# tejank10/AlphaGo.jl

Hardware: AMD Instinct MI355X
Metric: self-play positions/sec (9x9, tower=10, 400 readouts) (higher is better)
Workload: dtype f32

## Files before the change

### alphago.jl_amd/_lib.py

```python
import ctypes as C
import os

HERE = os.path.dirname(os.path.abspath(__file__))
LIB_PATH = os.path.join(HERE, "libagz.so")

OK, ILLEGAL_MOVE, ASSERT_DONE_NODE, HISTORY_INCOMPLETE, BAD_SHAPE, ASSERT_SOFTPICK = range(6)
BAD_ARGUMENT, HIP_ERROR, POOL_EXHAUSTED, RCCL_ERROR, NOT_READY = 6, 7, 8, 9, 10

L_VALUE_CONV, L_POLICY_CONV, L_VALUE_FC1, L_VALUE_FC2, L_POLICY_FC = -1, -2, -3, -4, -5
K_WEIGHT, K_BIAS, K_BN_BETA, K_BN_GAMMA, K_BN_MEAN, K_BN_VAR, K_BN_EPS = range(7)
F_CHILD_N, F_CHILD_W, F_CHILD_PRIOR = 0, 1, 2


class AgzError(RuntimeError):
    def __init__(self, status, message):
        super().__init__(f"agz status {status}: {message}")
        self.status = status


class IllegalMove(AgzError):
    """IllegalMove, src/AlphaGo.jl:8"""


class Config(C.Structure):
    _fields_ = [
        ("board_size", C.c_int32), ("tower_height", C.c_int32), ("games", C.c_int32),
        ("num_readouts", C.c_int32), ("parallel_readouts", C.c_int32), ("two_player_mode", C.c_int32),
        ("komi", C.c_float), ("reserved0", C.c_float),
        ("c_puct", C.c_double), ("dirichlet_noise_weight", C.c_double), ("resign_threshold", C.c_double),
        ("resign_disable_fraction", C.c_double),
        ("seed", C.c_uint64), ("game_id_base", C.c_uint64), ("game_id_stride", C.c_uint64),
        ("max_nodes_per_game", C.c_int32), ("device", C.c_int32), ("external_network", C.c_int32),
        ("pool_policy", C.c_int32), ("record_capacity_games", C.c_int32), ("arena_mode", C.c_int32),
    ]


class Stats(C.Structure):
    _fields_ = [(n, C.c_int64) for n in (
        "steps", "positions", "games_started", "games_finished", "evals", "duplicate_evals",
        "terminal_visits", "root_visits", "nodes_in_use", "pool_exhausted", "resigned_games", "live_games",
        "records_dropped", "pool_short_searches", "peak_nodes_per_game", "stalled_games", "node_capacity",
        "abandoned_games")]

    def as_dict(self):
        return {n: getattr(self, n) for n, _ in self._fields_}


class GameHeader(C.Structure):
    _fields_ = [("game_id", C.c_uint64), ("num_moves", C.c_int32), ("result", C.c_int32),
                ("was_resign", C.c_int32), ("resign_disabled", C.c_int32), ("final_score", C.c_float),
                ("short_searches", C.c_int32)]


class PositionInfo(C.Structure):
    _fields_ = [("n", C.c_int32), ("to_play", C.c_int32), ("ko", C.c_int32), ("caps_black", C.c_int32),
                ("caps_white", C.c_int32), ("last_move", C.c_int32), ("prev_move", C.c_int32),
                ("history_len", C.c_int32), ("komi", C.c_float)]


class NodeInfo(C.Structure):
    _fields_ = [("N", C.c_float), ("W", C.c_float), ("Q", C.c_float), ("parent", C.c_int32),
                ("fmove", C.c_int32), ("is_expanded", C.c_int32), ("losses_applied", C.c_int32),
                ("done", C.c_int32), ("pos", PositionInfo)]


class Analysis(C.Structure):
    _fields_ = [("move", C.c_int32), ("status", C.c_int32), ("N", C.c_float), ("W", C.c_float), ("Q", C.c_float),
                ("nodes_used", C.c_int32)]


class Line(C.Structure):
    _fields_ = [("move", C.c_int32), ("pv_len", C.c_int32), ("N", C.c_float), ("W", C.c_float), ("prior", C.c_float),
                ("end_W", C.c_float)]


_lib = None


def _share_hip_runtime_with_torch():
    import importlib.util
    import sys
    if "torch" in sys.modules or os.environ.get("AGZ_SYSTEM_HIP") == "1":
        return
    try:
        spec = importlib.util.find_spec("torch")
        path = os.path.join(os.path.dirname(spec.origin), "lib", "libamdhip64.so") if spec and spec.origin else None
        if path and os.path.exists(path):
            C.CDLL(path, mode=C.RTLD_GLOBAL)
    except Exception:
        pass


def load():
    global _lib
    if _lib is not None:
        return _lib
    _share_hip_runtime_with_torch()
    if not os.path.exists(LIB_PATH):
        raise ImportError(
            f"{LIB_PATH} is missing: build it with `python -c 'import __graft_entry__ as g; g.build()'` "
            "(hipcc --offload-arch=gfx950).  There is no CPU fallback.")
    L = C.CDLL(LIB_PATH)
    E = C.c_void_p
    P = C.POINTER
    i32, i64, u32, u64, f32, f64 = C.c_int32, C.c_int64, C.c_uint32, C.c_uint64, C.c_float, C.c_double
    i8p, i16p, i32p, f32p, f64p = P(C.c_int8), P(C.c_int16), P(i32), P(f32), P(f64)
    sig = {
        "agz_version": (i32, []),
        "agz_config_default": (None, [P(Config)]),
        "agz_engine_create": (i32, [P(Config), P(E)]),
        "agz_engine_destroy": (None, [E]),
        "agz_last_error": (C.c_char_p, [E]),
        "agz_engine_sync": (i32, [E]),
        "agz_net_set_weights": (i32, [E, i32, i32, f32p, i64]),
        "agz_net_param_count": (i64, [E, i32, i32]),
        "agz_net_get_weights": (i32, [E, i32, i32, f32p, i64]),
        "agz_net_init_synthetic": (i32, [E, u64]),
        "agz_net_forward": (i32, [E, i8p, i8p, i32p, i8p, i32, f32p, f32p]),
        "agz_net_forward_features": (i32, [E, f32p, i32, f32p, f32p]),
        "agz_net_forward_features_sym": (i32, [E, f32p, i32p, i32, f32p, f32p]),
        "agz_features": (i32, [E, i8p, i8p, i32p, i8p, i32, f32p]),
        "agz_net_time_forward": (i32, [E, i32, i32, f32p]),
        "agz_net_time_conv": (i32, [E, i32, i32, f32p]),
        "agz_net_set_winograd": (i32, [E, i32]),
        "agz_net_set_tower_persistent": (i32, [E, i32]),
        "agz_net_set_tower_streams": (i32, [E, i32]),
        "agz_net_set_precision": (i32, [E, i32]),
        "agz_profile_conv_enable": (i32, [E, i32]),
        "agz_profile_conv_read": (i32, [E, f64p, f64p, P(i64)]),
        "agz_profile_search_enable": (i32, [E, i32]),
        "agz_profile_search_read": (i32, [E, f64p, P(i64)]),
        "agz_go_play": (i32, [E, i8p, i8p, i32p, i32p, i32, i8p, i32p, i32p, i32p]),
        "agz_go_legal": (i32, [E, i8p, i8p, i32p, i32, i8p]),
        "agz_go_score": (i32, [E, i8p, f32p, i32, f32p]),
        "agz_selfplay_start": (i32, [E, i64]),
        "agz_selfplay_step": (i32, [E, i32]),
        "agz_selfplay_set_symmetry": (i32, [E, i32]),
        "agz_selfplay_set_hold": (i32, [E, i32]),
        "agz_selfplay_release": (i32, [E]),
        "agz_selfplay_set_starts": (i32, [E, i8p, P(PositionInfo), i8p, i64]),
        "agz_selfplay_starts_count": (i64, [E]),
        "agz_selfplay_set_playout_cap": (i32, [E, i32, C.c_double]),
        "agz_selfplay_playout_cap_counts": (i32, [E, P(i64)]),
        "agz_replay_set_targets_only": (i32, [E, i32]),
        "agz_replay_set_value_target": (i32, [E, C.c_double, C.c_double]),
        "agz_records_value_targets": (i32, [E, i64, C.c_double, C.c_double, f32p]),
        "agz_value_targets": (i32, [f32p, i32, i32, C.c_double, C.c_double, f32p]),
        "agz_selfplay_set_forced_playouts": (i32, [E, C.c_double, i32]),
        "agz_selfplay_forced_counts": (i32, [E, P(i64)]),
        "agz_tree_pruned_pi": (i32, [E, i32, i32, C.c_double, f32p]),
        "agz_selfplay_set_gumbel": (i32, [E, i32, C.c_double, C.c_double]),
        "agz_selfplay_gumbel_counts": (i32, [E, P(i64)]),
        "agz_tree_gumbel_pi": (i32, [E, i32, i32, C.c_double, C.c_double, f32p]),
        "agz_analyze_start": (i32, [E, i8p, P(PositionInfo), i8p, i64, u64]),
        "agz_review_start": (i32, [E, P(C.c_int16), P(i64), i8p, P(PositionInfo), i8p, i64, u64]),
        "agz_replay_reanalyze_start": (i32, [E, i64, i64, u64]),
        "agz_replay_reanalyze_commit": (i32, [E, P(i64)]),
        "agz_analyze_progress": (i32, [E, P(i64)]),
        "agz_analyze_results": (i32, [E, P(Analysis), f32p, f32p, f32p]),
        "agz_analyze_set_lines": (i32, [E, i32, i32, i32]),
        "agz_analyze_lines": (i32, [E, P(Line), i16p, f32p]),
        "agz_tree_lines": (i32, [E, i32, i32, i32, i32, i32, P(Line), i16p, f32p]),
        "agz_engine_stats": (i32, [E, P(Stats)]),
        "agz_selfplay_select": (i32, [E, i32p]),
        "agz_selfplay_leaf_features": (i32, [E, f32p]),
        "agz_selfplay_incorporate": (i32, [E, f32p, f32p]),
        "agz_records_count": (i64, [E]),
        "agz_records_header": (i32, [E, i64, P(GameHeader)]),
        "agz_records_game": (i32, [E, i64, i16p, f32p, f32p]),
        "agz_records_packed_size": (i32, [E, P(i64)]),
        "agz_records_export_packed": (i32, [E, C.c_void_p, i64, i32]),
        "agz_records_clear": (i32, [E]),
        "agz_slot_status": (i32, [E, i32p, i32p, i32p]),
        "agz_slot_abandon": (i32, [E, i32]),
        "agz_arena_counts": (i32, [E, i32p]),
        "agz_net_select": (i32, [E, i32]),
        "agz_records_features": (i32, [E, i64, f32p]),
        "agz_replay_features": (i32, [E, i16p, i64, i32p, i32p, i32, C.c_void_p, i32]),
        "agz_replay_features_starts": (i32, [E, i16p, i64, i32p, i32p, i32p, i32, C.c_void_p, i32]),
        "agz_replay_ingest_packed": (i32, [E, C.c_void_p, i64, i32, P(i64)]),
        "agz_replay_ingest_gathered": (i32, [E, C.c_void_p, i32, i32, i64, P(i64), P(i64)]),
        "agz_replay_count": (i64, [E]),
        "agz_replay_positions": (i64, [E]),
        "agz_replay_header": (i32, [E, i64, P(GameHeader)]),
        "agz_replay_game": (i32, [E, i64, i16p, f32p, f32p]),
        "agz_replay_trim": (i32, [E, i64]),
        "agz_replay_clear": (i32, [E]),
        "agz_replay_batch": (i32, [E, P(i64), i32p, i32, C.c_void_p, C.c_void_p, C.c_void_p, i32]),
        "agz_replay_batch_sym": (i32, [E, P(i64), i32p, i32p, i32, C.c_void_p, C.c_void_p, C.c_void_p, i32]),
        "agz_replay_ingest_records": (i32, [E, i64, i64, P(i64)]),
        "agz_replay_set_window": (i32, [E, i64]),
        "agz_replay_live_positions": (i64, [E]),
        "agz_device_alloc": (i32, [E, i64, P(C.c_void_p)]),
        "agz_device_free": (i32, [E, C.c_void_p]),
        "agz_replay_sample": (i32, [E, i32, u64, i32, C.c_void_p, C.c_void_p, C.c_void_p, C.c_void_p, C.c_void_p]),
        "agz_train_step": (i32, [E, C.c_void_p, C.c_void_p, C.c_void_p, i32, i32, f32, f32, f32p]),
        "agz_train_reset": (i32, [E]),
        "agz_comm_unique_id": (i32, [P(C.c_uint8)]),
        "agz_comm_create": (i32, [E, i32, i32, P(C.c_uint8), P(E)]),
        "agz_comm_destroy": (None, [E]),
        "agz_allgather_records": (i32, [E, E, P(i64)]),
        "agz_broadcast_weights": (i32, [E, E, i32, P(i64)]),
        "agz_gather_plan": (i32, [P(i64), i32, P(i64), P(i64)]),
        "agz_abi_layout": (i32, [C.c_char_p, i32p, i32]),
        "agz_tree_init": (i32, [E, i32, i8p, P(PositionInfo), i8p]),
        "agz_tree_root": (i32, [E, i32, i32p]),
        "agz_tree_select_leaf": (i32, [E, i32, i32, i32p]),
        "agz_tree_maybe_add_child": (i32, [E, i32, i32, i32, i32p]),
        "agz_tree_add_virtual_loss": (i32, [E, i32, i32, i32]),
        "agz_tree_revert_virtual_loss": (i32, [E, i32, i32, i32]),
        "agz_tree_incorporate": (i32, [E, i32, i32, f32p, i32, f32, i32]),
        "agz_tree_inject_noise": (i32, [E, i32, i32]),
        "agz_tree_search": (i32, [E, i32, i32, i32p]),
        "agz_tree_search_select": (i32, [E, i32, i32, i32p]),
        "agz_tree_leaf_features": (i32, [E, i32, f32p]),
        "agz_tree_leaf_positions": (i32, [E, i32, i32p, i8p, i8p, i32p, i8p, P(PositionInfo)]),
        "agz_tree_search_incorporate": (i32, [E, i32, f32p, f32p]),
        "agz_tree_pick_move": (i32, [E, i32, i32p]),
        "agz_tree_play_move": (i32, [E, i32, i32, i32p]),
        "agz_tree_should_resign": (i32, [E, i32, i32p]),
        "agz_tree_is_done": (i32, [E, i32, i32, i32p]),
        "agz_tree_node_info": (i32, [E, i32, i32, P(NodeInfo)]),
        "agz_tree_node_floats": (i32, [E, i32, i32, i32, f32p]),
        "agz_tree_node_scores": (i32, [E, i32, i32, f64p]),
        "agz_tree_node_set_floats": (i32, [E, i32, i32, i32, f32p]),
        "agz_tree_node_set_N": (i32, [E, i32, i32, f32]),
        "agz_tree_node_set_n": (i32, [E, i32, i32, i32]),
        "agz_tree_node_children": (i32, [E, i32, i32, i32p]),
        "agz_tree_node_board": (i32, [E, i32, i32, i8p]),
        "agz_tree_pending_vlosses": (i32, [E, i32, i32p]),
        "agz_tree_set_draw": (i32, [E, i32, u64, u32]),
        "agz_debug_draws": (i32, [E, u64, u64, u32, i32, f64, f64p]),
        "agz_debug_math": (i32, [E, i32, f64p, f64p, i32, f64p]),
        "agz_debug_counters": (i32, [E, C.POINTER(C.c_uint64), i32]),
        "agz_debug_set_stagger": (i32, [E, i32]),
        "agz_debug_live_record": (i32, [E, i32, i32, P(u64), i32p, i32p, f32p, f32p]),
        "agz_debug_mfma_sustained": (i32, [E, i32, C.POINTER(C.c_float)]),
        "agz_debug_pack_diff": (i32, [E, i32, P(i64)]),
        "agz_debug_mfma_sustained_data": (i32, [E, i32, i32, C.POINTER(C.c_float)]),
    }
    for name, (res, args) in sig.items():
        fn = getattr(L, name)
        fn.restype = res
        fn.argtypes = args
    L._agz_signatures = sig
    _lib = L
    return L


def default_config(**kw):
    c = Config()
    load().agz_config_default(C.byref(c))
    for k, v in kw.items():
        if not hasattr(c, k):
            raise TypeError(f"unknown agz_config field {k!r}")
        setattr(c, k, v)
    return c
```

### alphago.jl_amd/csrc/agz_capi.hip

```cpp
#include <cstddef>
#include <cstring>
#include <string>
#include <vector>

#include "../../include/agz_value_target.h"
#include "agz_engine.h"
#include "agz_search.h"

struct agz_engine {
  agz::Engine* impl;
  std::string err;
};

namespace {
std::string g_create_error;

template <class F>
agz_status guard(agz_engine* e, F&& f) {
  if (!e || !e->impl) return AGZ_BAD_ARGUMENT;
  try {
    f(*e->impl);
    return AGZ_OK;
  } catch (const agz::Error& x) {
    e->err = x.what();
    return x.status;
  } catch (const std::exception& x) {
    e->err = x.what();
    return AGZ_BAD_ARGUMENT;
  }
}

template <class F>
agz_status guard_status(agz_engine* e, F&& f) {
  if (!e || !e->impl) return AGZ_BAD_ARGUMENT;
  try {
    const int st = f(*e->impl);
    if (st != AGZ_OK) e->err = "reference-level condition " + std::to_string(st);
    return st;
  } catch (const agz::Error& x) {
    e->err = x.what();
    return x.status;
  } catch (const std::exception& x) {
    e->err = x.what();
    return AGZ_BAD_ARGUMENT;
  }
}

agz::TreeArgs targs(int op, int g, int node = 0, int a = 0, int up_to = -1) {
  agz::TreeArgs T;
  std::memset(&T, 0, sizeof(T));
  T.op = op; T.g = g; T.node = node; T.a = a; T.up_to = up_to;
  return T;
}
}

extern "C" {

int32_t agz_version(void) { return AGZ_VERSION; }

void agz_config_default(agz_config* c) {
  std::memset(c, 0, sizeof(*c));
  c->board_size = 19;
  c->tower_height = 19;
  c->games = 1;
  c->num_readouts = 800;
  c->parallel_readouts = 8;
  c->two_player_mode = 0;
  c->arena_mode = 0;
  c->komi = 7.5f;
  c->c_puct = 0.96;
  c->dirichlet_noise_weight = 0.25;
  c->resign_threshold = -0.9;
  c->resign_disable_fraction = 0.05;
  c->seed = 0;
  c->game_id_base = 0;
  c->game_id_stride = 1;
}

agz_status agz_engine_create(const agz_config* cfg, agz_engine** out) {
  if (!cfg || !out) return AGZ_BAD_ARGUMENT;
  *out = nullptr;
  try {
    agz_engine* e = new agz_engine{nullptr, {}};
    e->impl = new agz::Engine(*cfg);
    *out = e;
    return AGZ_OK;
  } catch (const agz::Error& x) {
    g_create_error = x.what();
    return x.status;
  } catch (const std::exception& x) {
    g_create_error = x.what();
    return AGZ_BAD_ARGUMENT;
  }
}

void agz_engine_destroy(agz_engine* e) {
  if (!e) return;
  delete e->impl;
  delete e;
}

const char* agz_last_error(const agz_engine* e) { return e ? e->err.c_str() : g_create_error.c_str(); }

agz_status agz_engine_sync(agz_engine* e) { return guard(e, [&](agz::Engine& E) { E.sync(); }); }

agz_status agz_net_set_weights(agz_engine* e, int32_t layer, int32_t kind, const float* data, int64_t count) {
  return guard(e, [&](agz::Engine& E) { E.net().set(layer, kind, data, count); });
}
int64_t agz_net_param_count(const agz_engine* e, int32_t layer, int32_t kind) {
  if (!e || !e->impl) return -1;
  return e->impl->net().param_count(layer, kind);
}
agz_status agz_net_get_weights(agz_engine* e, int32_t layer, int32_t kind, float* out, int64_t count) {
  return guard(e, [&](agz::Engine& E) { E.net().get(layer, kind, out, count); });
}
agz_status agz_net_select(agz_engine* e, int32_t which) {
  return guard(e, [&](agz::Engine& E) { E.net_select(which); });
}
agz_status agz_arena_counts(agz_engine* e, int32_t* counts_out) {
  return guard(e, [&](agz::Engine& E) {
    AGZ_REQUIRE(counts_out, AGZ_BAD_ARGUMENT, "null pointer");
    E.arena_counts(counts_out);
  });
}
agz_status agz_net_init_synthetic(agz_engine* e, uint64_t seed) {
  return guard(e, [&](agz::Engine& E) { E.net().init_synthetic(seed); });
}
agz_status agz_net_forward(agz_engine* e, const int8_t* boards, const int8_t* deltas, const int32_t* ndeltas,
                           const int8_t* to_play, int32_t B, float* pi_out, float* v_out) {
  return guard(e, [&](agz::Engine& E) { E.net_forward_positions(boards, deltas, ndeltas, to_play, B, pi_out, v_out); });
}
agz_status agz_net_forward_features(agz_engine* e, const float* feats, int32_t B, float* pi_out, float* v_out) {
  return guard(e, [&](agz::Engine& E) { E.net_forward_features(feats, B, pi_out, v_out); });
}
agz_status agz_net_forward_features_sym(agz_engine* e, const float* feats, const int32_t* sym, int32_t B, float* pi,
                                        float* v) {
  return guard(e, [&](agz::Engine& E) { E.net_forward_features_sym(feats, sym, B, pi, v); });
}
agz_status agz_features(agz_engine* e, const int8_t* boards, const int8_t* deltas, const int32_t* ndeltas,
                        const int8_t* to_play, int32_t B, float* out) {
  return guard(e, [&](agz::Engine& E) { E.features(boards, deltas, ndeltas, to_play, B, out); });
}
agz_status agz_net_time_forward(agz_engine* e, int32_t B, int32_t iters, float* ms_out) {
  return guard(e, [&](agz::Engine& E) { *ms_out = E.time_forward(B, iters); });
}
agz_status agz_net_time_conv(agz_engine* e, int32_t B, int32_t iters, float* ms_out) {
  return guard(e, [&](agz::Engine& E) { *ms_out = E.time_conv(B, iters); });
}

agz_status agz_net_set_winograd(agz_engine* e, int32_t on) {
  return guard(e, [&](agz::Engine& E) { AGZ_REQUIRE(on >= 0 && on <= 3, AGZ_BAD_ARGUMENT, "agz_net_set_winograd: 0, 1, 2 or 3"); E.net().set_winograd(on); });
}
agz_status agz_net_set_tower_persistent(agz_engine* e, int32_t on) {
  return guard(e, [&](agz::Engine& E) { E.net().set_tower_persistent(on != 0); });
}
agz_status agz_net_set_tower_streams(agz_engine* e, int32_t n) {
  return guard(e, [&](agz::Engine& E) {
    AGZ_REQUIRE(n >= 1 && n <= 4, AGZ_BAD_ARGUMENT, "agz_net_set_tower_streams: 1..4");
    E.net().set_tower_streams(n);
  });
}
agz_status agz_net_set_precision(agz_engine* e, int32_t precision) {
  return guard(e, [&](agz::Engine& E) {
    AGZ_REQUIRE(precision == AGZ_PRECISION_F32 || precision == AGZ_PRECISION_F16 || precision == AGZ_PRECISION_F32S,
                AGZ_BAD_ARGUMENT, "precision %d (0 = f32, 1 = f16 tower, 2 = f32 as split f16 operands)", precision);
    E.net().set_precision(precision);
  });
}
agz_status agz_profile_conv_enable(agz_engine* e, int32_t on) {
  return guard(e, [&](agz::Engine& E) { E.net().profile_enable(on != 0); });
}
agz_status agz_profile_conv_read(agz_engine* e, double* total_ms, double* total_flop, int64_t* launches) {
  return guard(e, [&](agz::Engine& E) { E.net().profile_read(total_ms, total_flop, launches); });
}
agz_status agz_profile_search_enable(agz_engine* e, int32_t on) {
  return guard(e, [&](agz::Engine& E) { E.profile_search_enable(on != 0); });
}
agz_status agz_profile_search_read(agz_engine* e, double* ms5, int64_t* steps) {
  return guard(e, [&](agz::Engine& E) {
    AGZ_REQUIRE(ms5, AGZ_BAD_ARGUMENT, "ms5 is NULL");
    E.profile_search_read(ms5, steps);
  });
}

agz_status agz_go_play(agz_engine* e, const int8_t* boards, const int8_t* to_play, const int32_t* ko,
                       const int32_t* moves, int32_t B, int8_t* boards_out, int32_t* ko_out,
                       int32_t* ncaptured_out, int32_t* status_out) {
  return guard(e, [&](agz::Engine& E) { E.go_play(boards, to_play, ko, moves, B, boards_out, ko_out, ncaptured_out, status_out); });
}
agz_status agz_go_legal(agz_engine* e, const int8_t* boards, const int8_t* to_play, const int32_t* ko, int32_t B,
                        int8_t* legal_out) {
  return guard(e, [&](agz::Engine& E) { E.go_legal(boards, to_play, ko, B, legal_out); });
}
agz_status agz_go_score(agz_engine* e, const int8_t* boards, const float* komi, int32_t B, float* score_out) {
  return guard(e, [&](agz::Engine& E) { E.go_score(boards, komi, B, score_out); });
}

agz_status agz_selfplay_start(agz_engine* e, int64_t total_games) {
  return guard(e, [&](agz::Engine& E) { E.start(total_games); });
}
agz_status agz_selfplay_step(agz_engine* e, int32_t nsteps) {
  return guard(e, [&](agz::Engine& E) { E.step(nsteps); });
}
agz_status agz_engine_stats(agz_engine* e, agz_stats* out) {
  return guard(e, [&](agz::Engine& E) { E.stats(out); });
}
agz_status agz_selfplay_select(agz_engine* e, int32_t* nleaves_out) {
  return guard(e, [&](agz::Engine& E) { *nleaves_out = E.select_external(); });
}
agz_status agz_selfplay_leaf_features(agz_engine* e, float* feats_out) {
  return guard(e, [&](agz::Engine& E) { E.leaf_features_external(feats_out); });
}
agz_status agz_selfplay_incorporate(agz_engine* e, const float* pi, const float* v) {
  return guard(e, [&](agz::Engine& E) { E.incorporate_external(pi, v); });
}

int64_t agz_records_count(agz_engine* e) {
  int64_t n = -1;
  guard(e, [&](agz::Engine& E) { n = E.records_count(); });
  return n;
}
agz_status agz_records_header(agz_engine* e, int64_t k, agz_game_header* out) {
  return guard(e, [&](agz::Engine& E) { E.record_header(k, out); });
}
agz_status agz_records_game(agz_engine* e, int64_t k, int16_t* moves, float* pis, float* qs) {
  return guard(e, [&](agz::Engine& E) { E.record_game(k, moves, pis, qs); });
}
agz_status agz_records_packed_size(agz_engine* e, int64_t* nbytes_out) {
  return guard(e, [&](agz::Engine& E) { *nbytes_out = E.records_packed_size(); });
}
agz_status agz_records_export_packed(agz_engine* e, void* dst, int64_t capacity, int32_t is_device) {
  return guard(e, [&](agz::Engine& E) { E.records_export_packed(dst, capacity, is_device != 0); });
}
agz_status agz_records_clear(agz_engine* e) { return guard(e, [&](agz::Engine& E) { E.records_clear(); }); }
agz_status agz_slot_status(agz_engine* e, int32_t* status_out, int32_t* nodes_out, int32_t* moves_out) {
  return guard(e, [&](agz::Engine& E) { E.slot_status(status_out, nodes_out, moves_out); });
}
agz_status agz_slot_abandon(agz_engine* e, int32_t slot) {
  return guard(e, [&](agz::Engine& E) { E.slot_abandon(slot); });
}
agz_status agz_records_features(agz_engine* e, int64_t k, float* out) {
  return guard(e, [&](agz::Engine& E) { E.record_features(k, out); });
}
agz_status agz_records_value_targets(agz_engine* e, int64_t k, double alpha, double lambda, float* out) {
  return guard(e, [&](agz::Engine& E) { E.record_value_targets(k, alpha, lambda, out); });
}
agz_status agz_value_targets(const float* qs, int32_t T, int32_t result, double alpha, double lambda, float* out) {
  if (T < 0 || (T > 0 && (!qs || !out)) || !agz_value_target_params_ok(alpha, lambda)) {
    g_create_error = "value targets: T >= 0 entries of qs and out, alpha and lambda both 0..1";
    return AGZ_BAD_ARGUMENT;
  }
  for (int32_t t = 0; t < T; ++t) out[t] = agz_value_target(qs, T, t, result, alpha, lambda);
  return AGZ_OK;
}
agz_status agz_replay_ingest_packed(agz_engine* e, const void* packed, int64_t nbytes, int32_t is_device,
                                    int64_t* added_out) {
  return guard(e, [&](agz::Engine& E) {
    const int64_t n = E.replay_ingest(packed, nbytes, is_device != 0);
    if (added_out) *added_out = n;
  });
}
agz_status agz_replay_ingest_gathered(agz_engine* e, const void* buf, int32_t is_device, int32_t world,
                                      int64_t chunk_stride, const int64_t* counts, int64_t* added_out) {
  return guard(e, [&](agz::Engine& E) {
    AGZ_REQUIRE(buf && counts && world >= 1 && chunk_stride >= 0 && chunk_stride % 8 == 0, AGZ_BAD_ARGUMENT, "bad gather buffer");
    std::vector<int64_t> coff((size_t)world), cbytes((size_t)world), cnrec((size_t)world);
    for (int r = 0; r < world; ++r) {
      AGZ_REQUIRE(counts[2 * r] >= 0 && counts[2 * r + 1] >= 0 && counts[2 * r + 1] <= chunk_stride && counts[2 * r + 1] % 8 == 0,
                  AGZ_BAD_ARGUMENT, "chunk %d: %lld records in %lld bytes", r, (long long)counts[2 * r], (long long)counts[2 * r + 1]);
      coff[r] = (int64_t)r * chunk_stride;
      cnrec[r] = counts[2 * r];
      cbytes[r] = counts[2 * r + 1];
    }
    const int64_t n = E.replay_ingest_gathered(buf, is_device != 0, (size_t)world * (size_t)chunk_stride, coff, cbytes, cnrec);
    if (added_out) *added_out = n;
  });
}
int64_t agz_replay_count(agz_engine* e) { return (e && e->impl) ? e->impl->replay_count() : -1; }
int64_t agz_selfplay_starts_count(agz_engine* e) { return (e && e->impl) ? e->impl->starts_count() : -1; }
int64_t agz_replay_positions(agz_engine* e) { return (e && e->impl) ? e->impl->replay_positions() : -1; }
agz_status agz_replay_header(agz_engine* e, int64_t k, agz_game_header* out) {
  return guard(e, [&](agz::Engine& E) {
    AGZ_REQUIRE(out != nullptr, AGZ_BAD_ARGUMENT, "null pointer");
    E.replay_header(k, out);
  });
}
agz_status agz_replay_game(agz_engine* e, int64_t k, int16_t* moves, float* pis, float* qs) {
  return guard(e, [&](agz::Engine& E) { E.replay_game(k, moves, pis, qs); });
}
agz_status agz_replay_trim(agz_engine* e, int64_t max_positions) {
  return guard(e, [&](agz::Engine& E) { E.replay_trim(max_positions); });
}
agz_status agz_replay_clear(agz_engine* e) { return guard(e, [&](agz::Engine& E) { E.replay_clear(); }); }
agz_status agz_replay_batch(agz_engine* e, const int64_t* game, const int32_t* ply, int32_t B, float* feats,
                            float* pi, float* z, int32_t out_is_device) {
  return guard(e, [&](agz::Engine& E) { E.replay_batch(game, ply, B, feats, pi, z, out_is_device != 0); });
}

agz_status agz_replay_ingest_records(agz_engine* e, int64_t first, int64_t count, int64_t* added_out) {
  return guard(e, [&](agz::Engine& E) {
    const int64_t n = E.replay_ingest_records(first, count);
    if (added_out) *added_out = n;
  });
}
agz_status agz_replay_set_window(agz_engine* e, int64_t max_entries) {
  return guard(e, [&](agz::Engine& E) { E.replay_set_window(max_entries); });
}
int64_t agz_replay_live_positions(agz_engine* e) { return (e && e->impl) ? e->impl->replay_live_positions() : -1; }
agz_status agz_replay_sample(agz_engine* e, int32_t B, uint64_t call, int32_t sym_mode, float* feats, float* pi, float* z,
                             int64_t* game_out, int32_t* ply_out) {
  return guard(e, [&](agz::Engine& E) { E.replay_sample(B, call, sym_mode, feats, pi, z, game_out, ply_out); });
}
agz_status agz_selfplay_set_hold(agz_engine* e, int32_t on) {
  return guard(e, [&](agz::Engine& E) { E.set_hold(on != 0); });
}
agz_status agz_selfplay_release(agz_engine* e) { return guard(e, [&](agz::Engine& E) { E.release(); }); }
agz_status agz_selfplay_set_starts(agz_engine* e, const int8_t* boards, const agz_position_info* info,
                                   const int8_t* history, int64_t S) {
  return guard(e, [&](agz::Engine& E) { E.set_starts(boards, info, history, S); });
}
agz_status agz_selfplay_set_playout_cap(agz_engine* e, int32_t fast_readouts, double full_prob) {
  return guard(e, [&](agz::Engine& E) { E.set_playout_cap(fast_readouts, full_prob); });
}
agz_status agz_selfplay_playout_cap_counts(agz_engine* e, int64_t out[2]) {
  return guard(e, [&](agz::Engine& E) {
    AGZ_REQUIRE(out, AGZ_BAD_ARGUMENT, "null pointer");
    E.playout_cap_counts(out);
  });
}
agz_status agz_selfplay_set_forced_playouts(agz_engine* e, double k, int32_t prune) {
  return guard(e, [&](agz::Engine& E) { E.set_forced_playouts(k, prune); });
}
agz_status agz_selfplay_forced_counts(agz_engine* e, int64_t out[2]) {
  return guard(e, [&](agz::Engine& E) {
    AGZ_REQUIRE(out, AGZ_BAD_ARGUMENT, "null pointer");
    E.forced_counts(out);
  });
}
agz_status agz_tree_pruned_pi(agz_engine* e, int32_t g, int32_t node, double k, float* out) {
  return guard(e, [&](agz::Engine& E) { E.tree_pruned_pi(g, node, k, out); });
}
agz_status agz_selfplay_set_gumbel(agz_engine* e, int32_t m, double c_visit, double c_scale) {
  return guard(e, [&](agz::Engine& E) { E.set_gumbel(m, c_visit, c_scale); });
}
agz_status agz_selfplay_gumbel_counts(agz_engine* e, int64_t out[2]) {
  return guard(e, [&](agz::Engine& E) {
    AGZ_REQUIRE(out, AGZ_BAD_ARGUMENT, "null pointer");
    E.gumbel_counts(out);
  });
}
agz_status agz_tree_gumbel_pi(agz_engine* e, int32_t g, int32_t node, double c_visit, double c_scale, float* out) {
  return guard(e, [&](agz::Engine& E) { E.tree_gumbel_pi(g, node, c_visit, c_scale, out); });
}
agz_status agz_replay_set_targets_only(agz_engine* e, int32_t on) {
  return guard(e, [&](agz::Engine& E) { E.replay_set_targets_only(on != 0); });
}
agz_status agz_replay_set_value_target(agz_engine* e, double alpha, double lambda) {
  return guard(e, [&](agz::Engine& E) { E.replay_set_value_target(alpha, lambda); });
}
agz_status agz_device_alloc(agz_engine* e, int64_t bytes, void** out) {
  return guard(e, [&](agz::Engine& E) {
    AGZ_REQUIRE(out && bytes > 0, AGZ_BAD_ARGUMENT, "bad allocation request");
    *out = nullptr;
    AGZ_HIP(hipSetDevice(E.config().device));
    AGZ_HIP(hipMalloc(out, (size_t)bytes));
  });
}
agz_status agz_device_free(agz_engine* e, void* p) {
  return guard(e, [&](agz::Engine& E) {
    E.sync();
    if (p) AGZ_HIP(hipFree(p));
  });
}

agz_status agz_replay_batch_sym(agz_engine* e, const int64_t* game, const int32_t* ply, const int32_t* sym, int32_t B,
                                float* feats, float* pi, float* z, int32_t out_is_device) {
  return guard(e, [&](agz::Engine& E) {
    AGZ_REQUIRE(sym, AGZ_BAD_ARGUMENT, "sym is NULL");
    E.replay_batch(game, ply, B, feats, pi, z, out_is_device != 0, sym);
  });
}
agz_status agz_selfplay_set_symmetry(agz_engine* e, int32_t mode) {
  return guard(e, [&](agz::Engine& E) { E.set_symmetry(mode); });
}

agz_status agz_analyze_start(agz_engine* e, const int8_t* boards, const agz_position_info* info, const int8_t* history,
                             int64_t B, uint64_t game_id_base) {
  return guard(e, [&](agz::Engine& E) { E.analyze_start(boards, info, history, B, game_id_base); });
}
agz_status agz_review_start(agz_engine* e, const int16_t* moves, const int64_t* game_offset, const int8_t* boards,
                            const agz_position_info* info, const int8_t* history, int64_t G, uint64_t game_id_base) {
  return guard(e, [&](agz::Engine& E) { E.review_start(moves, game_offset, boards, info, history, G, game_id_base); });
}
agz_status agz_replay_reanalyze_start(agz_engine* e, int64_t first, int64_t count, uint64_t game_id_base) {
  return guard(e, [&](agz::Engine& E) { E.replay_reanalyze_start(first, count, game_id_base); });
}
agz_status agz_replay_reanalyze_commit(agz_engine* e, int64_t counts_out[3]) {
  return guard(e, [&](agz::Engine& E) { E.replay_reanalyze_commit(counts_out); });
}
agz_status agz_analyze_progress(agz_engine* e, int64_t* done_out) {
  return guard(e, [&](agz::Engine& E) {
    const int64_t d = E.analyze_progress();
    if (done_out) *done_out = d;
  });
}
agz_status agz_analyze_results(agz_engine* e, agz_analysis* out, float* child_N, float* child_W, float* prior) {
  return guard(e, [&](agz::Engine& E) { E.analyze_results(out, child_N, child_W, prior); });
}

agz_status agz_analyze_set_lines(agz_engine* e, int32_t K, int32_t D, int32_t min_visits) {
  return guard(e, [&](agz::Engine& E) { E.analyze_set_lines(K, D, min_visits); });
}
agz_status agz_analyze_lines(agz_engine* e, agz_line* lines, int16_t* pv, float* pv_N) {
  return guard(e, [&](agz::Engine& E) { E.analyze_lines(lines, pv, pv_N); });
}
agz_status agz_tree_lines(agz_engine* e, int32_t g, int32_t node, int32_t K, int32_t D, int32_t min_visits,
                          agz_line* lines, int16_t* pv, float* pv_N) {
  return guard(e, [&](agz::Engine& E) { E.tree_lines(g, node, K, D, min_visits, lines, pv, pv_N); });
}

agz_status agz_train_step(agz_engine* e, const float* feats, const float* pi, const float* z, int32_t B,
                          int32_t inputs_are_device, float eta, float rho, float* losses_out) {
  return guard(e, [&](agz::Engine& E) { E.train_step(feats, pi, z, B, inputs_are_device != 0, eta, rho, losses_out); });
}
agz_status agz_train_reset(agz_engine* e) { return guard(e, [&](agz::Engine& E) { E.train_reset(); }); }

agz_status agz_comm_unique_id(uint8_t* id_out) {
  if (!id_out) return AGZ_BAD_ARGUMENT;
  try {
    agz::comm_unique_id(id_out);
    return AGZ_OK;
  } catch (const agz::Error& x) {
    g_create_error = x.what();
    return x.status;
  } catch (const std::exception& x) {
    g_create_error = x.what();
    return AGZ_RCCL_ERROR;
  }
}
agz_status agz_comm_create(agz_engine* e, int32_t rank, int32_t world, const uint8_t* id, agz_comm** out) {
  if (!out) return AGZ_BAD_ARGUMENT;
  *out = nullptr;
  return guard(e, [&](agz::Engine& E) { *out = reinterpret_cast<agz_comm*>(agz::comm_create(E, rank, world, id)); });
}
void agz_comm_destroy(agz_comm* c) { agz::comm_destroy(reinterpret_cast<agz::Comm*>(c)); }
agz_status agz_allgather_records(agz_engine* e, agz_comm* comm, int64_t* added_out) {
  return guard(e, [&](agz::Engine& E) {
    const int64_t n = agz::comm_allgather_records(E, reinterpret_cast<agz::Comm*>(comm));
    if (added_out) *added_out = n;
  });
}
agz_status agz_gather_plan(const int64_t* counts, int32_t world, int64_t* chunk_stride_out, int64_t* total_records_out) {
  if (!chunk_stride_out) return AGZ_BAD_ARGUMENT;
  try {
    *chunk_stride_out = agz::gather_plan(counts, world, total_records_out);
    return AGZ_OK;
  } catch (const agz::Error& x) {
    g_create_error = x.what();
    return x.status;
  }
}
agz_status agz_broadcast_weights(agz_engine* e, agz_comm* comm, int32_t root, int64_t* nfloats_out) {
  return guard(e, [&](agz::Engine& E) {
    const int64_t n = agz::comm_broadcast_weights(E, reinterpret_cast<agz::Comm*>(comm), root);
    if (nfloats_out) *nfloats_out = n;
  });
}

int32_t agz_abi_layout(const char* name, int32_t* out, int32_t cap) {
  if (!name || !out) return -1;
  std::vector<int32_t> v;
#define AGZ_SZ(T) v.push_back((int32_t)sizeof(T))
#define AGZ_OFF(T, f) v.push_back((int32_t)offsetof(T, f))
  const std::string n(name);
  if (n == "agz_config") {
    AGZ_SZ(agz_config);
    AGZ_OFF(agz_config, board_size); AGZ_OFF(agz_config, tower_height); AGZ_OFF(agz_config, games);
    AGZ_OFF(agz_config, num_readouts); AGZ_OFF(agz_config, parallel_readouts); AGZ_OFF(agz_config, two_player_mode);
    AGZ_OFF(agz_config, komi); AGZ_OFF(agz_config, reserved0); AGZ_OFF(agz_config, c_puct);
    AGZ_OFF(agz_config, dirichlet_noise_weight); AGZ_OFF(agz_config, resign_threshold);
    AGZ_OFF(agz_config, resign_disable_fraction); AGZ_OFF(agz_config, seed); AGZ_OFF(agz_config, game_id_base);
    AGZ_OFF(agz_config, game_id_stride); AGZ_OFF(agz_config, max_nodes_per_game); AGZ_OFF(agz_config, device);
    AGZ_OFF(agz_config, external_network); AGZ_OFF(agz_config, pool_policy);
    AGZ_OFF(agz_config, record_capacity_games); AGZ_OFF(agz_config, arena_mode);
  } else if (n == "agz_stats") {
    AGZ_SZ(agz_stats);
    AGZ_OFF(agz_stats, steps); AGZ_OFF(agz_stats, positions); AGZ_OFF(agz_stats, games_started);
    AGZ_OFF(agz_stats, games_finished); AGZ_OFF(agz_stats, evals); AGZ_OFF(agz_stats, duplicate_evals);
    AGZ_OFF(agz_stats, terminal_visits); AGZ_OFF(agz_stats, root_visits); AGZ_OFF(agz_stats, nodes_in_use);
    AGZ_OFF(agz_stats, pool_exhausted); AGZ_OFF(agz_stats, resigned_games); AGZ_OFF(agz_stats, live_games);
    AGZ_OFF(agz_stats, records_dropped); AGZ_OFF(agz_stats, pool_short_searches);
    AGZ_OFF(agz_stats, peak_nodes_per_game); AGZ_OFF(agz_stats, stalled_games); AGZ_OFF(agz_stats, node_capacity);
    AGZ_OFF(agz_stats, abandoned_games);
  } else if (n == "agz_game_header") {
    AGZ_SZ(agz_game_header);
    AGZ_OFF(agz_game_header, game_id); AGZ_OFF(agz_game_header, num_moves); AGZ_OFF(agz_game_header, result);
    AGZ_OFF(agz_game_header, was_resign); AGZ_OFF(agz_game_header, resign_disabled);
    AGZ_OFF(agz_game_header, final_score); AGZ_OFF(agz_game_header, short_searches);
  } else if (n == "agz_position_info") {
    AGZ_SZ(agz_position_info);
    AGZ_OFF(agz_position_info, n); AGZ_OFF(agz_position_info, to_play); AGZ_OFF(agz_position_info, ko);
    AGZ_OFF(agz_position_info, caps_black); AGZ_OFF(agz_position_info, caps_white);
    AGZ_OFF(agz_position_info, last_move); AGZ_OFF(agz_position_info, prev_move);
    AGZ_OFF(agz_position_info, history_len); AGZ_OFF(agz_position_info, komi);
  } else if (n == "agz_node_info") {
    AGZ_SZ(agz_node_info);
    AGZ_OFF(agz_node_info, N); AGZ_OFF(agz_node_info, W); AGZ_OFF(agz_node_info, Q); AGZ_OFF(agz_node_info, parent);
    AGZ_OFF(agz_node_info, fmove); AGZ_OFF(agz_node_info, is_expanded); AGZ_OFF(agz_node_info, losses_applied);
    AGZ_OFF(agz_node_info, done); AGZ_OFF(agz_node_info, pos);
  } else if (n == "agz_analysis") {
    AGZ_SZ(agz_analysis);
    AGZ_OFF(agz_analysis, move); AGZ_OFF(agz_analysis, status); AGZ_OFF(agz_analysis, N); AGZ_OFF(agz_analysis, W);
    AGZ_OFF(agz_analysis, Q); AGZ_OFF(agz_analysis, nodes_used);
  } else if (n == "agz_line") {
    AGZ_SZ(agz_line);
    AGZ_OFF(agz_line, move); AGZ_OFF(agz_line, pv_len); AGZ_OFF(agz_line, N); AGZ_OFF(agz_line, W);
    AGZ_OFF(agz_line, prior); AGZ_OFF(agz_line, end_W);
  } else {
    return -1;
  }
#undef AGZ_SZ
#undef AGZ_OFF
  if ((int32_t)v.size() > cap) return -1;
  for (size_t i = 0; i < v.size(); ++i) out[i] = v[i];
  return (int32_t)v.size() - 1;
}

agz_status agz_replay_features(agz_engine* e, const int16_t* moves, int64_t nmoves, const int32_t* game_offset,
                               const int32_t* ply, int32_t B, float* out, int32_t out_is_device) {
  return guard(e, [&](agz::Engine& E) {
    AGZ_REQUIRE(B == 0 || (game_offset && ply && out && (moves || nmoves == 0)), AGZ_BAD_ARGUMENT, "null pointer");
    E.replay_batch_features(moves, nmoves, game_offset, ply, B, out, out_is_device != 0);
  });
}
agz_status agz_replay_features_starts(agz_engine* e, const int16_t* moves, int64_t nmoves, const int32_t* game_offset,
                                      const int32_t* ply, const int32_t* start, int32_t B, float* out,
                                      int32_t out_is_device) {
  return guard(e, [&](agz::Engine& E) {
    AGZ_REQUIRE(B == 0 || (game_offset && ply && out && (moves || nmoves == 0)), AGZ_BAD_ARGUMENT, "null pointer");
    E.replay_batch_features(moves, nmoves, game_offset, ply, B, out, out_is_device != 0, start);
  });
}

agz_status agz_tree_init(agz_engine* e, int32_t g, const int8_t* board, const agz_position_info* info,
                         const int8_t* history) {
  return guard_status(e, [&](agz::Engine& E) {
    AGZ_REQUIRE(board && info, AGZ_BAD_ARGUMENT, "agz_tree_init: null board/info");
    agz::TreeArgs T = targs(agz::TOP_INIT, g);
    T.info = *info;
    T.board = board;
    T.history = history;
    return E.tree_op(T, nullptr);
  });
}
agz_status agz_tree_root(agz_engine* e, int32_t g, int32_t* node_out) {
  return guard(e, [&](agz::Engine& E) {
    agz::GameState s;
    E.game_state(g, &s);
    *node_out = s.root;
  });
}
agz_status agz_tree_select_leaf(agz_engine* e, int32_t g, int32_t from_node, int32_t* leaf_out) {
  return guard_status(e, [&](agz::Engine& E) {
    agz::TreeArgs T = targs(agz::TOP_SELECT, g, from_node);
    return E.tree_op(T, leaf_out);
  });
}
agz_status agz_tree_maybe_add_child(agz_engine* e, int32_t g, int32_t node, int32_t a, int32_t* child_out) {
  return guard_status(e, [&](agz::Engine& E) {
    agz::TreeArgs T = targs(agz::TOP_ADD_CHILD, g, node, a);
    return E.tree_op(T, child_out);
  });
}
agz_status agz_tree_add_virtual_loss(agz_engine* e, int32_t g, int32_t node, int32_t up_to) {
  return guard_status(e, [&](agz::Engine& E) {
    agz::TreeArgs T = targs(agz::TOP_VLOSS_ADD, g, node, 0, up_to);
    return E.tree_op(T, nullptr);
  });
}
agz_status agz_tree_revert_virtual_loss(agz_engine* e, int32_t g, int32_t node, int32_t up_to) {
  return guard_status(e, [&](agz::Engine& E) {
    agz::TreeArgs T = targs(agz::TOP_VLOSS_REVERT, g, node, 0, up_to);
    return E.tree_op(T, nullptr);
  });
}
agz_status agz_tree_incorporate(agz_engine* e, int32_t g, int32_t node, const float* probs, int32_t nprobs,
                                float value, int32_t up_to) {
  return guard_status(e, [&](agz::Engine& E) {
    if (nprobs != E.view().A) return (int)AGZ_BAD_SHAPE;
    agz::TreeArgs T = targs(agz::TOP_INCORPORATE, g, node, 0, up_to);
    T.probs = probs;
    T.value = value;
    return E.tree_op(T, nullptr);
  });
}
agz_status agz_tree_inject_noise(agz_engine* e, int32_t g, int32_t node) {
  return guard_status(e, [&](agz::Engine& E) {
    agz::TreeArgs T = targs(agz::TOP_NOISE, g, node);
    return E.tree_op(T, nullptr);
  });
}
agz_status agz_tree_search_select(agz_engine* e, int32_t g, int32_t par, int32_t* nleaves_out) {
  return guard_status(e, [&](agz::Engine& E) { return E.tree_search_select(g, par, nleaves_out); });
}
agz_status agz_tree_leaf_features(agz_engine* e, int32_t g, float* feats_out) {
  return guard(e, [&](agz::Engine& E) { E.tree_leaf_features(g, feats_out); });
}
agz_status agz_tree_leaf_positions(agz_engine* e, int32_t g, int32_t* nodes_out, int8_t* boards_out, int8_t* deltas_out,
                                   int32_t* ndeltas_out, int8_t* to_play_out, agz_position_info* info_out) {
  return guard(e, [&](agz::Engine& E) {
    E.tree_leaf_positions(g, nodes_out, boards_out, deltas_out, ndeltas_out, to_play_out, info_out);
  });
}
agz_status agz_tree_search_incorporate(agz_engine* e, int32_t g, const float* pi, const float* v) {
  return guard_status(e, [&](agz::Engine& E) { return E.tree_search_incorporate(g, pi, v); });
}
agz_status agz_tree_search(agz_engine* e, int32_t g, int32_t par, int32_t* nleaves_out) {
  return guard_status(e, [&](agz::Engine& E) {
    const int st = E.tree_search_select(g, par, nleaves_out);
    if (st != AGZ_OK) return st;
    return E.tree_search_incorporate(g, nullptr, nullptr);
  });
}
agz_status agz_tree_pick_move(agz_engine* e, int32_t g, int32_t* a_out) {
  return guard_status(e, [&](agz::Engine& E) {
    agz::TreeArgs T = targs(agz::TOP_PICK, g);
    return E.tree_op(T, a_out);
  });
}
agz_status agz_tree_play_move(agz_engine* e, int32_t g, int32_t a, int32_t* ok_out) {
  return guard_status(e, [&](agz::Engine& E) {
    agz::TreeArgs T = targs(agz::TOP_PLAY, g, 0, a);
    return E.tree_op(T, ok_out);
  });
}
agz_status agz_tree_should_resign(agz_engine* e, int32_t g, int32_t* out) {
  return guard_status(e, [&](agz::Engine& E) {
    agz::TreeArgs T = targs(agz::TOP_RESIGN, g);
    return E.tree_op(T, out);
  });
}
agz_status agz_tree_is_done(agz_engine* e, int32_t g, int32_t node, int32_t* out) {
  return guard(e, [&](agz::Engine& E) {
    agz::NodeMeta m;
    E.node_meta(g, node, &m);
    *out = (m.flags & agz::NF_DONE) || m.n >= E.view().max_game_length;
  });
}
agz_status agz_tree_node_info(agz_engine* e, int32_t g, int32_t node, agz_node_info* out) {
  return guard(e, [&](agz::Engine& E) {
    agz::NodeMeta m;
    agz::GameState s;
    E.node_meta(g, node, &m);
    E.game_state(g, &s);
    std::memset(out, 0, sizeof(*out));
    out->N = E.node_stat(g, node, 0);
    out->W = E.node_stat(g, node, 1);
    out->Q = out->W / (1.0f + out->N);
    out->parent = m.parent;
    out->fmove = m.fmove;
    out->is_expanded = (m.flags & agz::NF_EXPANDED) != 0;
    out->losses_applied = m.losses;
    out->done = (m.flags & agz::NF_DONE) != 0;
    out->pos.n = m.n;
    out->pos.to_play = m.to_play;
    out->pos.ko = m.ko;
    out->pos.caps_black = m.caps_b;
    out->pos.caps_white = m.caps_w;
    out->pos.last_move = m.last_move;
    out->pos.prev_move = -1;
    out->pos.history_len = s.hist_len;
    out->pos.komi = s.komi;
  });
}
agz_status agz_tree_node_floats(agz_engine* e, int32_t g, int32_t node, int32_t field, float* out) {
  return guard(e, [&](agz::Engine& E) { E.node_row_get(g, node, field, out); });
}
agz_status agz_tree_node_scores(agz_engine* e, int32_t g, int32_t node, double* out) {
  return guard_status(e, [&](agz::Engine& E) {
    agz::TreeArgs T = targs(agz::TOP_SCORES, g, node);
    T.dout = out;
    return E.tree_op(T, nullptr);
  });
}
agz_status agz_tree_node_set_floats(agz_engine* e, int32_t g, int32_t node, int32_t field, const float* in) {
  return guard(e, [&](agz::Engine& E) { E.node_row_set(g, node, field, in); });
}
agz_status agz_tree_node_set_N(agz_engine* e, int32_t g, int32_t node, float value) {
  return guard(e, [&](agz::Engine& E) { E.node_set_N(g, node, value); });
}
agz_status agz_tree_node_set_n(agz_engine* e, int32_t g, int32_t node, int32_t n) {
  return guard(e, [&](agz::Engine& E) {
    agz::NodeMeta m;
    E.node_meta(g, node, &m);
    m.n = n;
    E.node_meta_set(g, node, m);
  });
}
agz_status agz_tree_node_children(agz_engine* e, int32_t g, int32_t node, int32_t* out) {
  return guard(e, [&](agz::Engine& E) { E.node_children(g, node, out); });
}
agz_status agz_tree_node_board(agz_engine* e, int32_t g, int32_t node, int8_t* out) {
  return guard(e, [&](agz::Engine& E) { E.node_board(g, node, out); });
}
agz_status agz_tree_pending_vlosses(agz_engine* e, int32_t g, int32_t* out) {
  return guard_status(e, [&](agz::Engine& E) {
    agz::TreeArgs T = targs(agz::TOP_PENDING, g);
    return E.tree_op(T, out);
  });
}
agz_status agz_tree_set_draw(agz_engine* e, int32_t g, uint64_t game_id, uint32_t sel) {
  return guard(e, [&](agz::Engine& E) {
    agz::GameState s;
    E.game_state(g, &s);
    s.game_id = game_id;
    s.sel = (int32_t)sel;
    E.game_patch(g, s);
  });
}

agz_status agz_debug_draws(agz_engine* e, uint64_t seed, uint64_t game, uint32_t move, int32_t n, double alpha,
                           double* gamma_out) {
  return guard(e, [&](agz::Engine& E) { E.debug_draws(seed, game, move, n, alpha, gamma_out); });
}
agz_status agz_debug_math(agz_engine* e, int32_t op, const double* x, const double* y, int32_t n, double* out) {
  return guard(e, [&](agz::Engine& E) { E.debug_math(op, x, y, n, out); });
}
int32_t agz_debug_counters(agz_engine* e, uint64_t* out, int32_t cap) {
  int32_t n = -1;
  (void)guard(e, [&](agz::Engine& E) { n = E.debug_counters(out, cap); });
  return n;
}
agz_status agz_debug_live_record(agz_engine* e, int32_t g, int32_t k, uint64_t* game_id_out, int32_t* num_moves_out,
                                 int32_t* move_out, float* pi_out, float* q_out) {
  return guard(e, [&](agz::Engine& E) { E.debug_live_record(g, k, game_id_out, num_moves_out, move_out, pi_out, q_out); });
}
agz_status agz_debug_set_stagger(agz_engine* e, int32_t moves) {
  return guard(e, [&](agz::Engine& E) { E.debug_set_stagger(moves); });
}
agz_status agz_debug_mfma_sustained(agz_engine* e, int32_t millis, float* tflops_out) {
  return guard(e, [&](agz::Engine& E) { *tflops_out = E.net().mfma_sustained_tflops(millis); });
}
agz_status agz_debug_mfma_sustained_data(agz_engine* e, int32_t millis, int32_t mode, float* tflops_out) {
  return guard(e, [&](agz::Engine& E) { *tflops_out = E.net().mfma_sustained_tflops(millis, mode); });
}
agz_status agz_debug_pack_diff(agz_engine* e, int32_t which, int64_t* mismatches_out) {
  return guard(e, [&](agz::Engine& E) { *mismatches_out = (int64_t)E.net().debug_pack_diff(which); });
}

}
```

### alphago.jl_amd/csrc/agz_glds.h

```cpp
#pragma once

namespace agz {

__device__ __forceinline__ void glds16(const float* g, unsigned lds_byte_addr) {
  unsigned keep;
  lds_byte_addr = __builtin_amdgcn_readfirstlane(lds_byte_addr);
  asm volatile(
      "s_mov_b32 %0, m0\n\ts_mov_b32 m0, %2\n\ts_nop 0\n\tglobal_load_lds_dwordx4 %1, off\n\ts_mov_b32 m0, %0"
      : "=&s"(keep)
      : "v"(g), "s"(lds_byte_addr)
      : "memory");
}

__device__ __forceinline__ void glds16s(const float* gbase_uniform, unsigned lane_byte_off, unsigned lds_byte_addr) {
  unsigned keep;
  lds_byte_addr = __builtin_amdgcn_readfirstlane(lds_byte_addr);
  asm volatile("s_mov_b32 %0, m0\n\ts_mov_b32 m0, %3\n\ts_nop 0\n\tglobal_load_lds_dwordx4 %1, %2\n\ts_mov_b32 m0, %0"
               : "=&s"(keep) : "v"(lane_byte_off), "s"(gbase_uniform), "s"(lds_byte_addr) : "memory");
}

__device__ __forceinline__ void glds16_l2(const float* g, unsigned lds_byte_addr) {
  unsigned keep;
  lds_byte_addr = __builtin_amdgcn_readfirstlane(lds_byte_addr);
  asm volatile(
      "s_mov_b32 %0, m0\n\ts_mov_b32 m0, %2\n\ts_nop 0\n\tglobal_load_lds_dwordx4 %1, off sc1\n\ts_mov_b32 m0, %0"
      : "=&s"(keep)
      : "v"(g), "s"(lds_byte_addr)
      : "memory");
}
__device__ __forceinline__ void glds16s_l2(const float* gbase_uniform, unsigned lane_byte_off, unsigned lds_byte_addr) {
  unsigned keep;
  lds_byte_addr = __builtin_amdgcn_readfirstlane(lds_byte_addr);
  asm volatile("s_mov_b32 %0, m0\n\ts_mov_b32 m0, %3\n\ts_nop 0\n\tglobal_load_lds_dwordx4 %1, %2 sc1\n\ts_mov_b32 m0, %0"
               : "=&s"(keep) : "v"(lane_byte_off), "s"(gbase_uniform), "s"(lds_byte_addr) : "memory");
}


}
```

### alphago.jl_amd/csrc/agz_nn.h

```cpp
#pragma once
#include <algorithm>
#include <cstdint>
#include <functional>
#include <memory>
#include <type_traits>
#include <vector>

#include "agz_common.h"

namespace agz {

constexpr int kC = 256;
constexpr int kCinStem = 17;
constexpr int kCinStemPad = 32;
constexpr int kWinoStages = 64, kWinoStemStages = 8;

struct ConvHost {
  int k = 3, cin = 0, cout = 0;
  std::vector<float> w, b, beta, gamma, mean, var;
  float eps = 1e-5f;
};
struct DenseHost {
  int in = 0, out = 0;
  std::vector<float> w, b;
};

struct ImageFamily {
  const char* name;
  size_t (*bytes)(int ns);
  void (*host_pack)(const ConvHost& c, void* out, int ns);
  void (*device_pack)(const float* d_w, long wstride, int cin, int layers, void* d_out, int ns, hipStream_t s);
};
extern const ImageFamily kDirectImage;
extern const ImageFamily kWinoImage, kWinoSplitImage;
extern const ImageFamily kWino4Image, kWino5Image;
extern const ImageFamily kConv16Image;

bool wino4_applies(int N);
bool wino_fusable(int N);

enum class TowerForm { Direct, F16, Wino3, Wino3Persistent, Wino5, Wino4 };

class Net {
 public:
  Net(int N, int tower, hipStream_t stream);
  ~Net();
  int N() const { return N_; }
  int P() const { return P_; }
  int A() const { return A_; }
  int tower() const { return tower_; }

  int64_t param_count(int layer, int kind) const;
  void set(int layer, int kind, const float* data, int64_t count);
  void get(int layer, int kind, float* out, int64_t count) const;
  void init_synthetic(uint64_t seed);

  static void weight_keys(int tower, std::vector<std::pair<int, int>>& keys);
  float* flux_device() { return d_flux_.p; }
  size_t flux_count() const { return flux_n_; }
  size_t flux_offset(int layer, int kind) const;
  void device_master_written() { host_stale_ = true; ++param_version_; }
  long debug_pack_diff(int which);

  void reserve(int bcap);
  void forward(const float* d_x32, const int* d_count, int bcap, float* d_pi, float* d_v);
  void launch_tower_conv_once(const int* d_count, int bcap);

  void set_winograd(int mode) { winograd_ = mode; }
  bool winograd() const { return winograd_ != 0; }
  void set_tower_streams(int n) { tower_streams_ = n < 1 ? 1 : n > kMaxTowerStreams ? kMaxTowerStreams : n; }
  int tower_streams() const { return tower_streams_; }
  void set_tower_persistent(bool on) { tower_persistent_ = on; }
  void check_async_error();
  bool tower_persistent() const { return tower_persistent_; }
  void set_precision(int p) { precision_ = p; }
  int precision() const { return precision_; }
  TowerForm tower_form() const {
    if (tower_ == 0) return TowerForm::Direct;
    if (precision_ == 1) return TowerForm::F16;
    if (winograd_ == 0) return TowerForm::Direct;
    if (precision_ == 0 && winograd_ != 2 && wino4_applies(N_)) return TowerForm::Wino4;
    if (precision_ == 0 && winograd_ == 3 && wino_fusable(N_)) return TowerForm::Wino5;
    return tower_persistent_ && wino_fusable(N_) ? TowerForm::Wino3Persistent : TowerForm::Wino3;
  }

  float mfma_sustained_tflops(int millis, int mode = 0);
  void profile_enable(bool on);
  void profile_read(double* total_ms, double* total_flop, int64_t* launches);

  ConvHost* conv(int layer);
  const ConvHost* conv(int layer) const;
  DenseHost* dense(int layer);
  const DenseHost* dense(int layer) const;
  void sync_host() const;
  uint64_t param_version() const { return param_version_; }

  double flops_per_eval() const;
  double conv_flops_per_launch(int B) const { return 2.0 * B * P_ * 9.0 * kC * kC; }

 private:
  void pack();
  enum ImageId { kDirectStem, kDirectTower, kWinoStem, kWinoTower, kSplitStem, kSplitTower, kWino4Tower, kWino5Tower, kF16Tower, kImages };
  struct BuiltImage {
    const ImageFamily* family;
    bool stem;
    int which;
    bool (*needed)(const Net&);
    DevBuf<uint32_t> buf;
    uint64_t version = ~0ull;
  };
  static bool always(const Net&) { return true; }
  static bool with_tower(const Net& n) { return n.tower_ > 0; }
  static bool split_selected(const Net& n) { return n.tower_ > 0 && n.precision_ == 2; }
  template <TowerForm F> static bool form_is(const Net& n) { return n.tower_form() == F; }
  BuiltImage images_[kImages] = {{&kDirectImage, true, 0, always},
                                 {&kDirectImage, false, 0, with_tower},
                                 {&kWinoImage, true, 1, with_tower},
                                 {&kWinoImage, false, 1, with_tower},
                                 {&kWinoSplitImage, true, 4, split_selected},
                                 {&kWinoSplitImage, false, 4, split_selected},
                                 {&kWino4Image, false, 2, form_is<TowerForm::Wino4>},
                                 {&kWino5Image, false, 6, form_is<TowerForm::Wino5>},
                                 {&kConv16Image, false, 3, form_is<TowerForm::F16>}};
  uint64_t affines_version_ = ~0ull;
  int image_stages(const BuiltImage& im) const { return im.stem ? kWinoStemStages : kWinoStages; }
  template <class T>
  const T* image(ImageId id, int l = 0) const {
    const BuiltImage& im = images_[id];
    return reinterpret_cast<const T*>(im.buf.p + im.family->bytes(image_stages(im)) / 4 * l);
  }
  void stem(TowerForm form, const float* d_x32, const int* d_count, int bcap);
  void direct_tower(const int* d_count, int bcap);
  void f16_tower(const int* d_count, int bcap);
  void wino_tower(TowerForm form, const int* d_count, int bcap);
  void persistent_tower(const int* d_count, int bcap);
  struct LayerIO { const float *vin, *res; float *y, *vout; };
  LayerIO layer_io(int l, bool dense) const;
  void wino_layer(TowerForm form, int l, const LayerIO& io, const int* d_count, int bcap, hipStream_t st, int part = 0,
                  int parts = 1);
  template <class Layer> void run_chains(int chains, const Layer& layer);
  template <class Launch> void timed(int layers, const Launch& launch);

  int N_, P_, A_, tower_;
  hipStream_t stream_;
  ConvHost stem_, vconv_, pconv_;
  std::vector<ConvHost> tconv_;
  DenseHost vfc1_, vfc2_, pfc_;
  struct FluxSlot { int layer, kind; size_t off, n; };
  std::vector<FluxSlot> slots_;
  size_t flux_n_ = 0;
  DevBuf<float> d_flux_;
  mutable bool host_stale_ = false;
  uint64_t param_version_ = 0;
  void upload_slot(const FluxSlot& s);
  void upload_host_all();
  const float* host_slot(const FluxSlot& s) const;

  DevBuf<float> d_scale_, d_shift_;
  DevBuf<float> d_head_;
  const float *d_vfc1w_ = nullptr, *d_vfc1b_ = nullptr, *d_vfc2w_ = nullptr, *d_vfc2b_ = nullptr, *d_pfcw_ = nullptr,
              *d_pfcb_ = nullptr;
  int bcap_ = 0;
  DevBuf<float> d_a_, d_b_, d_t_, d_vh_, d_ph_;
  int winograd_ = 1;
  static constexpr int kMaxTowerStreams = 4;
  int tower_streams_ = 2;
  hipStream_t streamx_[kMaxTowerStreams - 1] = {nullptr, nullptr, nullptr};
  hipEvent_t ev_fork_ = nullptr, ev_join_[kMaxTowerStreams - 1] = {nullptr, nullptr, nullptr};
  DevBuf<float> d_scale_s_;
  DevBuf<float> d_vimg_, d_vimg2_;
  int precision_ = 0;
  DevBuf<uint16_t> d_ha_, d_hb_, d_ht_;
  bool tower_persistent_ = false;
  DevBuf<int> d_tower_sched_;
  DevBuf<char> d_tower_layers_;
  std::vector<char> tower_layers_host_;
  int32_t* tower_err_ = nullptr;
  std::vector<int> prof_mult_;
  bool prof_on_ = false;
  std::vector<hipEvent_t> prof_ev_;
  std::vector<int> prof_fwd_of_;
  int32_t* prof_counts_ = nullptr;
  int prof_n_ = 0, prof_fwd_ = 0;
  static constexpr int kProfMax = 4096;
};

class Trainer {
 public:
  Trainer(Net& net, hipStream_t s);
  ~Trainer();
  void step(const float* feats, const float* pi, const float* z, int B, bool is_device, float eta, float rho,
            float* losses_out);
  void reset();

 private:
  struct Param;
  void upload();
  void publish(long M);
  uint64_t uploaded_version_ = ~0ull;
  Net& net_;
  hipStream_t stream_;
  std::vector<std::unique_ptr<Param>> params_;
  bool have_vel_ = false;
  DevBuf<float> d_x32_, d_u_, d_o_, d_ga_, d_gb_, d_gc_, d_stats_, d_ones_, d_zero_, d_wd_, d_small_, d_in_, d_part_, d_wpart_;
  DevBuf<double> d_sums_;
  DevBuf<int> d_cnt_;
  DevBuf<unsigned char> d_opta_, d_optw_;
  int n_optw_ = 0;
};

void launch_conv3x3_direct_taps(const float* x, const float* wt, const float* ones, const float* zeros, const float* shift,
                                float* y, float* part, const int* d_count, int bcap, int N, int cin_pad, hipStream_t s);
int conv3x3_direct_blocks(int bcap, int N);
void launch_conv3x3_direct(const float* x, const float* wt, const float* scale, const float* shift, const float* res,
                           float* y, const int* d_count, int bcap, int N, int relu, int cin_pad, hipStream_t s);

size_t wino_v_floats(int bcap, int T);
long wino_blocks(int bcap, int T);
inline void wino_block_range(int blocks, int part, int parts, bool pairs, int& tb0, int& tb1) {
  AGZ_REQUIRE(parts >= 1 && part >= 0 && part < parts, AGZ_BAD_ARGUMENT, "tile-block range %d of %d", part, parts);
  int per = (blocks + parts - 1) / parts;
  if (pairs) per = (per + 1) & ~1;
  tb0 = std::min(blocks, part * per);
  tb1 = part + 1 == parts ? blocks : std::min(blocks, tb0 + per);
}
inline void wino_check_32bit(long blocks, int rows, int bcap, int N) {
  AGZ_REQUIRE((blocks + 1) * rows < (1L << 31) && (long)bcap * N * N * kC * 4 < (1L << 32), AGZ_BAD_ARGUMENT,
              "batch of %d positions at %dx%d: tile index / activation byte offset exceeds 32 bits", bcap, N, N);
}
void launch_wino_in(const float* x, float* vimg, const int* d_count, int bcap, int N, bool split, hipStream_t s,
                    int ns = kWinoStages, bool fixup = false);
void launch_wino_gemm(const float* vimg, const float* uimg, const float* scale, const float* shift, const float* res,
                      float* y, float* vnext, const int* d_count, int bcap, int N, int relu, bool split, hipStream_t s,
                      int ns = kWinoStages, int part = 0, int parts = 1);
bool wino_fusable(int N);
struct WinoTowerLayer {
  const float *v, *u, *scale, *shift, *res;
  float *y, *vnext;
  int mode, relu;
};
size_t wino_tower_sched_ints(int layers, int bcap, int N);
bool wino_tower_supported(hipStream_t s);
void launch_wino_tower(const void* d_layers, int layers, int* d_sched, const int* d_count, int bcap, int N, bool split, hipStream_t s);
constexpr int kWinoTowerErrWord = 8;
float wino_split_descale();

template <class Launch>
void dispatch_mode(const void* y, const void* vnext, const void* res, Launch&& launch) {
  switch ((y ? 1 : 0) | (vnext ? 2 : 0) | (res ? 4 : 0)) {
    case 1: launch(std::integral_constant<int, 1>{}); break;
    case 2: launch(std::integral_constant<int, 2>{}); break;
    case 3: launch(std::integral_constant<int, 3>{}); break;
    case 5: launch(std::integral_constant<int, 5>{}); break;
    case 6: launch(std::integral_constant<int, 6>{}); break;
    default: launch(std::integral_constant<int, 7>{}); break;
  }
}

void launch_wino5_gemm(const float* vimg, const float* uimg, const float* scale, const float* shift, const float* res,
                       float* y, float* vnext, const int* d_count, int bcap, int N, int relu, hipStream_t s, int part = 0,
                       int parts = 1);

constexpr int kWino4Stages = 96;
bool wino4_applies(int N);
bool wino4_whole_boards(int N);
size_t wino4_v_floats(int bcap, int N);
void launch_wino4_in(const float* x, float* vimg, const int* d_count, int bcap, int N, hipStream_t s, bool fixup, int part = 0,
                     int parts = 1);
void launch_wino4_gemm(const float* vimg, const float* uimg, const float* scale, const float* shift, const float* res,
                       float* y, float* vnext, const int* d_count, int bcap, int N, int relu, hipStream_t s, int part = 0,
                       int parts = 1, bool y_for_fixup_only = false);
bool wino4_paired(int N);
void wino4_validate(int bcap, int N);

void launch_conv16_dma(const uint16_t* x, const uint16_t* wi, const float* scale, const float* shift, const void* res,
                       int res_f32, void* y, int out_f32, const int* d_count, int bcap, int N, int relu, hipStream_t s);
void launch_f32_to_f16(const float* x, uint16_t* y, const int* d_count, int bcap, int N, hipStream_t s);

void launch_features_from_deltas(const int8_t* d_boards, const int8_t* d_deltas, const int32_t* d_ndeltas,
                                 const int8_t* d_to_play, int B, int N, float* d_x32, float* d_whcn,
                                 hipStream_t stream);
void launch_whcn_to_x32(const float* d_whcn, int B, int N, float* d_x32, hipStream_t stream);

}
```

### alphago.jl_amd/csrc/agz_nn.hip

```cpp
#include "agz_nn.h"
#include "agz_pack.h"

#include <cmath>
#include <algorithm>
#include <cstring>

#include "../../include/agz_draws.h"

namespace agz {

typedef float f32x16 __attribute__((ext_vector_type(16)));


constexpr int BM = 128, BN = 128, BK = 32;
constexpr int LDS_STRIDE = BK + 4;

template <int CIN, bool TAPSPLIT = false>
__global__ __launch_bounds__(256, 2) void k_conv3x3_mfma(
    const float* __restrict__ x, const float* __restrict__ wt, const float* __restrict__ scale,
    const float* __restrict__ shift, const float* __restrict__ res, float* __restrict__ y,
    const int* __restrict__ d_count, int N, int relu, long ystride = 0) {
  constexpr int NCHUNK = 9 * CIN / BK;
  constexpr int CPT = CIN / BK;
  const int c_begin = TAPSPLIT ? (int)blockIdx.y * CPT : 0, c_end = TAPSPLIT ? c_begin + CPT : NCHUNK;
  if (TAPSPLIT) y += (long)blockIdx.y * ystride;
  __shared__ __attribute__((aligned(16))) float lds[2][2][BM * LDS_STRIDE];

  const int P = N * N;
  const long M = (long)(*d_count) * P;

  const int nblk = gridDim.x, bid = blockIdx.x;
  const int q = nblk >> 3, r = nblk & 7, xcd = bid & 7;
  const int swz = (xcd < r ? xcd * (q + 1) : r * (q + 1) + (xcd - r) * q) + (bid >> 3);
  const long m0 = (long)(swz >> 1) * BM;
  const int n0 = (swz & 1) * BN;
  if (m0 >= M) return;

  const int tid = threadIdx.x;
  const int lrow = tid >> 3, c4 = tid & 7;

#define AGZ_ROWSETUP(i)                                            \
  const long mrow##i = m0 + lrow + 32 * i;                         \
  const bool rvalid##i = mrow##i < M;                              \
  const int p##i = (int)(mrow##i % P);                             \
  const int ri##i = p##i % N, cj##i = p##i / N;                    \
  const float* wrow##i = wt + (long)(n0 + lrow + 32 * i) * (9 * CIN) + c4 * 4;
  AGZ_ROWSETUP(0) AGZ_ROWSETUP(1) AGZ_ROWSETUP(2) AGZ_ROWSETUP(3)
#undef AGZ_ROWSETUP

  float4 ra0, ra1, ra2, ra3, rb0, rb1, rb2, rb3;
#define AGZ_LOADROW(i, da, db, aoff, boff)                                                             \
  {                                                                                                     \
    const bool ok = rvalid##i && (unsigned)(ri##i + da) < (unsigned)N && (unsigned)(cj##i + db) < (unsigned)N; \
    ra##i = ok ? *reinterpret_cast<const float4*>(x + (mrow##i + da + N * db) * CIN + aoff)             \
               : make_float4(0.f, 0.f, 0.f, 0.f);                                                       \
    rb##i = *reinterpret_cast<const float4*>(wrow##i + boff);                                           \
  }
#define AGZ_LOAD_CHUNK(c)                                         \
  {                                                               \
    const int tap_ = (c) / CPT, ci0_ = ((c) % CPT) * BK;          \
    const int da_ = tap_ % 3 - 1, db_ = tap_ / 3 - 1;             \
    const int aoff_ = ci0_ + c4 * 4, boff_ = (c) * BK;            \
    AGZ_LOADROW(0, da_, db_, aoff_, boff_)                        \
    AGZ_LOADROW(1, da_, db_, aoff_, boff_)                        \
    AGZ_LOADROW(2, da_, db_, aoff_, boff_)                        \
    AGZ_LOADROW(3, da_, db_, aoff_, boff_)                        \
  }
#define AGZ_STOREROW(buf, i)                                                                           \
  *reinterpret_cast<float4*>(&lds[buf][0][(lrow + 32 * i) * LDS_STRIDE + c4 * 4]) = ra##i;             \
  *reinterpret_cast<float4*>(&lds[buf][1][(lrow + 32 * i) * LDS_STRIDE + c4 * 4]) = rb##i;
#define AGZ_STORE_CHUNK(buf) { AGZ_STOREROW(buf, 0) AGZ_STOREROW(buf, 1) AGZ_STOREROW(buf, 2) AGZ_STOREROW(buf, 3) }

  const int lane = tid & 63, wave = tid >> 6;
  const int wr = wave >> 1, wc = wave & 1;
  const int l31 = lane & 31, hi = lane >> 5;

  f32x16 acc[2][2];
#pragma unroll
  for (int a = 0; a < 2; ++a)
#pragma unroll
    for (int b = 0; b < 2; ++b)
#pragma unroll
      for (int e = 0; e < 16; ++e) acc[a][b][e] = 0.f;

  AGZ_LOAD_CHUNK(c_begin)
  AGZ_STORE_CHUNK(0)
  __syncthreads();

  for (int c = c_begin; c < c_end; ++c) {
    const int buf = (c - c_begin) & 1;
    if (c + 1 < c_end) AGZ_LOAD_CHUNK(c + 1)
    const float* As = &lds[buf][0][(wr * 64 + l31) * LDS_STRIDE + hi * 4];
    const float* Bs = &lds[buf][1][(wc * 64 + l31) * LDS_STRIDE + hi * 4];
#pragma unroll
    for (int kk = 0; kk < BK / 8; ++kk) {
      const float4 a0 = *reinterpret_cast<const float4*>(As + kk * 8);
      const float4 a1 = *reinterpret_cast<const float4*>(As + 32 * LDS_STRIDE + kk * 8);
      const float4 b0 = *reinterpret_cast<const float4*>(Bs + kk * 8);
      const float4 b1 = *reinterpret_cast<const float4*>(Bs + 32 * LDS_STRIDE + kk * 8);
#define AGZ_MFMA4(f)                                                                          \
  acc[0][0] = __builtin_amdgcn_mfma_f32_32x32x2f32(a0.f, b0.f, acc[0][0], 0, 0, 0);             \
  acc[0][1] = __builtin_amdgcn_mfma_f32_32x32x2f32(a0.f, b1.f, acc[0][1], 0, 0, 0);             \
  acc[1][0] = __builtin_amdgcn_mfma_f32_32x32x2f32(a1.f, b0.f, acc[1][0], 0, 0, 0);             \
  acc[1][1] = __builtin_amdgcn_mfma_f32_32x32x2f32(a1.f, b1.f, acc[1][1], 0, 0, 0);
      AGZ_MFMA4(x) AGZ_MFMA4(y) AGZ_MFMA4(z) AGZ_MFMA4(w)
#undef AGZ_MFMA4
    }
    if (c + 1 < c_end) AGZ_STORE_CHUNK(buf ^ 1)
    __syncthreads();
  }

#undef AGZ_LOADROW
#undef AGZ_LOAD_CHUNK
#undef AGZ_STOREROW
#undef AGZ_STORE_CHUNK
#pragma unroll
  for (int tn = 0; tn < 2; ++tn) {
    const int n = n0 + wc * 64 + tn * 32 + l31;
    const float sc = scale[n], sh = shift[n];
#pragma unroll
    for (int tm = 0; tm < 2; ++tm) {
#pragma unroll
      for (int e = 0; e < 16; ++e) {
        const long m = m0 + wr * 64 + tm * 32 + (e & 3) + 8 * (e >> 2) + 4 * hi;
        if (m < M) {
          float v = acc[tm][tn][e] * sc + sh;
          if (res) v += res[m * kC + n];
          if (relu) v = fmaxf(v, 0.f);
          y[m * kC + n] = v;
        }
      }
    }
  }
}


__device__ __forceinline__ float wave_sum(float v) {
#pragma unroll
  for (int o = 32; o > 0; o >>= 1) v += __shfl_xor(v, o, 64);
  return v;
}

__global__ __launch_bounds__(256) void k_head_conv(const float* __restrict__ x, const float* __restrict__ hp,
                                                    float* __restrict__ vh, float* __restrict__ ph,
                                                    const int* __restrict__ d_count, int P) {
  const long M = (long)(*d_count) * P;
  const int lane = threadIdx.x & 63, wave = threadIdx.x >> 6;
  const float4 wv = *reinterpret_cast<const float4*>(hp + lane * 4);
  const float4 w0 = *reinterpret_cast<const float4*>(hp + 256 + lane * 4);
  const float4 w1 = *reinterpret_cast<const float4*>(hp + 512 + lane * 4);
  const float sv = hp[768], tv = hp[769], s0 = hp[770], t0 = hp[771], s1 = hp[772], t1 = hp[773];
  for (long m = (long)blockIdx.x * 4 + wave; m < M; m += (long)gridDim.x * 4) {
    const float4 xv = *reinterpret_cast<const float4*>(x + m * kC + lane * 4);
    float dv = xv.x * wv.x + xv.y * wv.y + xv.z * wv.z + xv.w * wv.w;
    float d0 = xv.x * w0.x + xv.y * w0.y + xv.z * w0.z + xv.w * w0.w;
    float d1 = xv.x * w1.x + xv.y * w1.y + xv.z * w1.z + xv.w * w1.w;
    dv = wave_sum(dv);
    d0 = wave_sum(d0);
    d1 = wave_sum(d1);
    if (lane == 0) {
      vh[m] = fmaxf(dv * sv + tv, 0.f);
      ph[m * 2 + 0] = fmaxf(d0 * s0 + t0, 0.f);
      ph[m * 2 + 1] = fmaxf(d1 * s1 + t1, 0.f);
    }
  }
}

__device__ float block_reduce(float v, bool is_max, float* red ) {
  const int lane = threadIdx.x & 63, wave = threadIdx.x >> 6;
#pragma unroll
  for (int o = 32; o > 0; o >>= 1) {
    const float t = __shfl_xor(v, o, 64);
    v = is_max ? fmaxf(v, t) : v + t;
  }
  __syncthreads();
  if (lane == 0) red[wave] = v;
  __syncthreads();
  float r = red[0];
#pragma unroll
  for (int w = 1; w < 4; ++w) r = is_max ? fmaxf(r, red[w]) : r + red[w];
  return r;
}

__global__ __launch_bounds__(256) void k_head_fc(
    const float* __restrict__ vh, const float* __restrict__ ph, const float* __restrict__ w1,
    const float* __restrict__ b1, const float* __restrict__ w2, const float* __restrict__ b2,
    const float* __restrict__ wp, const float* __restrict__ bp, float* __restrict__ pi,
    float* __restrict__ v, const int* __restrict__ d_count, int P, int A) {
  extern __shared__ __attribute__((aligned(16))) float sm[];
  float* vin = sm;
  float* pin = sm + P;
  float* logit = pin + 2 * P;
  float* red = logit + A;
  const int b = blockIdx.x;
  if (b >= *d_count) return;
  const int tid = threadIdx.x;
  for (int i = tid; i < P; i += 256) {
    vin[i] = vh[(long)b * P + i];
    pin[i] = ph[((long)b * P + i) * 2 + 0];
    pin[P + i] = ph[((long)b * P + i) * 2 + 1];
  }
  __syncthreads();
  float lmax = -INFINITY;
  for (int o = tid; o < A; o += 256) {
    float z = bp[o];
    for (int i = 0; i < 2 * P; ++i) z += wp[o + (long)A * i] * pin[i];
    logit[o] = z;
    lmax = fmaxf(lmax, z);
  }
  const float mx = block_reduce(lmax, true, red);
  float lsum = 0.f;
  for (int o = tid; o < A; o += 256) {
    const float e = expf(logit[o] - mx);
    logit[o] = e;
    lsum += e;
  }
  const float sum = block_reduce(lsum, false, red);
  for (int o = tid; o < A; o += 256) pi[(long)b * A + o] = logit[o] / sum;
  float h = b1[tid];
  for (int i = 0; i < P; ++i) h += w1[tid + 256 * i] * vin[i];
  h = fmaxf(h, 0.f);
  const float s = block_reduce(h * w2[tid], false, red);
  if (tid == 0) v[b] = tanhf(s + b2[0]);
}


__global__ __launch_bounds__(128) void k_feats_from_deltas(
    const int8_t* __restrict__ boards, const int8_t* __restrict__ deltas, const int32_t* __restrict__ ndeltas,
    const int8_t* __restrict__ to_play, int B, int N, float* __restrict__ x32, float* __restrict__ whcn) {
  const int b = blockIdx.x;
  if (b >= B) return;
  const int P = N * N;
  const int nd = ndeltas[b];
  const int tp = to_play[b];
  for (int p = threadIdx.x; p < P; p += blockDim.x) {
    int cur = boards[(long)b * P + p];
    float f[32];
#pragma unroll
    for (int k = 0; k < 8; ++k) {
      if (k >= 1 && k <= nd) cur -= deltas[((long)b * 7 + (k - 1)) * P + p];
      f[2 * k] = cur == tp ? 1.f : 0.f;
      f[2 * k + 1] = cur == -tp ? 1.f : 0.f;
    }
    f[16] = (float)tp;
#pragma unroll
    for (int c = 17; c < 32; ++c) f[c] = 0.f;
    if (x32) {
      float4* dst = reinterpret_cast<float4*>(x32 + ((long)b * P + p) * 32);
#pragma unroll
      for (int c = 0; c < 8; ++c) dst[c] = make_float4(f[4 * c], f[4 * c + 1], f[4 * c + 2], f[4 * c + 3]);
    }
    if (whcn) {
#pragma unroll
      for (int c = 0; c < 17; ++c) whcn[(long)P * (c + 17L * b) + p] = f[c];
    }
  }
}

__global__ __launch_bounds__(128) void k_whcn_to_x32(const float* __restrict__ whcn, int B, int P,
                                                      float* __restrict__ x32) {
  const int b = blockIdx.x;
  if (b >= B) return;
  for (int p = threadIdx.x; p < P; p += blockDim.x) {
    float* dst = x32 + ((long)b * P + p) * 32;
    for (int c = 0; c < 17; ++c) dst[c] = whcn[(long)P * (c + 17L * b) + p];
    for (int c = 17; c < 32; ++c) dst[c] = 0.f;
  }
}

void launch_features_from_deltas(const int8_t* d_boards, const int8_t* d_deltas, const int32_t* d_ndeltas,
                                 const int8_t* d_to_play, int B, int N, float* d_x32, float* d_whcn,
                                 hipStream_t stream) {
  if (B <= 0) return;
  hipLaunchKernelGGL(k_feats_from_deltas, dim3(B), dim3(128), 0, stream, d_boards, d_deltas, d_ndeltas,
                     d_to_play, B, N, d_x32, d_whcn);
  AGZ_HIP(hipGetLastError());
}

void launch_whcn_to_x32(const float* d_whcn, int B, int N, float* d_x32, hipStream_t stream) {
  if (B <= 0) return;
  hipLaunchKernelGGL(k_whcn_to_x32, dim3(B), dim3(128), 0, stream, d_whcn, B, N * N, d_x32);
  AGZ_HIP(hipGetLastError());
}


static void conv_init(ConvHost& c, int k, int cin, int cout) {
  c.k = k; c.cin = cin; c.cout = cout;
  c.w.assign((size_t)k * k * cin * cout, 0.f);
  c.b.assign(cout, 0.f);
  c.beta.assign(cout, 0.f);
  c.gamma.assign(cout, 1.f);
  c.mean.assign(cout, 0.f);
  c.var.assign(cout, 1.f);
  c.eps = 1e-5f;
}
static void dense_init(DenseHost& d, int in, int out) {
  d.in = in; d.out = out;
  d.w.assign((size_t)in * out, 0.f);
  d.b.assign(out, 0.f);
}

static std::vector<float>* conv_field(ConvHost* c, int kind);

Net::Net(int N, int tower, hipStream_t stream) : N_(N), P_(N * N), A_(N * N + 1), tower_(tower), stream_(stream) {
  conv_init(stem_, 3, kCinStem, kC);
  tconv_.resize(2 * tower);
  for (auto& c : tconv_) conv_init(c, 3, kC, kC);
  conv_init(vconv_, 1, kC, 1);
  conv_init(pconv_, 1, kC, 2);
  dense_init(vfc1_, P_, 256);
  dense_init(vfc2_, 256, 1);
  dense_init(pfc_, 2 * P_, A_);
  std::vector<std::pair<int, int>> keys;
  weight_keys(tower_, keys);
  for (auto& lk : keys) {
    const size_t n = (size_t)param_count(lk.first, lk.second);
    slots_.push_back({lk.first, lk.second, flux_n_, n});
    flux_n_ += n;
  }
  d_flux_.alloc(flux_n_);
  upload_host_all();
}

void Net::weight_keys(int tower, std::vector<std::pair<int, int>>& keys) {
  for (int l = 0; l <= 2 * tower; ++l)
    for (int k = 0; k < 7; ++k) keys.push_back({l, k});
  for (int l : {AGZ_L_VALUE_CONV, AGZ_L_POLICY_CONV})
    for (int k = 0; k < 7; ++k) keys.push_back({l, k});
  for (int l : {AGZ_L_VALUE_FC1, AGZ_L_VALUE_FC2, AGZ_L_POLICY_FC})
    for (int k = 0; k < 2; ++k) keys.push_back({l, k});
}

size_t Net::flux_offset(int layer, int kind) const {
  for (const auto& sl : slots_)
    if (sl.layer == layer && sl.kind == kind) return sl.off;
  AGZ_REQUIRE(false, AGZ_BAD_ARGUMENT, "no parameter (layer %d, kind %d)", layer, kind);
  return 0;
}

const float* Net::host_slot(const FluxSlot& sl) const {
  if (const ConvHost* c = conv(sl.layer))
    return sl.kind == AGZ_K_BN_EPS ? &c->eps : conv_field(const_cast<ConvHost*>(c), sl.kind)->data();
  const DenseHost* d = dense(sl.layer);
  return (sl.kind == AGZ_K_WEIGHT ? d->w : d->b).data();
}

void Net::upload_slot(const FluxSlot& sl) {
  upload(d_flux_.p + sl.off, host_slot(sl), (size_t)sl.n, stream_);
}
void Net::upload_host_all() {
  std::vector<float> flat(flux_n_);
  for (const auto& sl : slots_) std::memcpy(flat.data() + sl.off, host_slot(sl), sizeof(float) * sl.n);
  upload(d_flux_.p, flat.data(), (size_t)flux_n_, stream_);
  AGZ_HIP(hipStreamSynchronize(stream_));
  host_stale_ = false;
}

void Net::sync_host() const {
  if (!host_stale_) return;
  std::vector<float> flat(flux_n_);
  download(flat.data(), d_flux_.p, (size_t)flux_n_, stream_);
  AGZ_HIP(hipStreamSynchronize(stream_));
  for (const auto& sl : slots_) std::memcpy(const_cast<float*>(host_slot(sl)), flat.data() + sl.off, sizeof(float) * sl.n);
  host_stale_ = false;
}

ConvHost* Net::conv(int layer) {
  if (layer == 0) return &stem_;
  if (layer >= 1 && layer <= 2 * tower_) return &tconv_[layer - 1];
  if (layer == AGZ_L_VALUE_CONV) return &vconv_;
  if (layer == AGZ_L_POLICY_CONV) return &pconv_;
  return nullptr;
}
const ConvHost* Net::conv(int layer) const { return const_cast<Net*>(this)->conv(layer); }
DenseHost* Net::dense(int layer) {
  if (layer == AGZ_L_VALUE_FC1) return &vfc1_;
  if (layer == AGZ_L_VALUE_FC2) return &vfc2_;
  if (layer == AGZ_L_POLICY_FC) return &pfc_;
  return nullptr;
}
const DenseHost* Net::dense(int layer) const { return const_cast<Net*>(this)->dense(layer); }

static std::vector<float>* conv_field(ConvHost* c, int kind) {
  switch (kind) {
    case AGZ_K_WEIGHT: return &c->w;
    case AGZ_K_BIAS: return &c->b;
    case AGZ_K_BN_BETA: return &c->beta;
    case AGZ_K_BN_GAMMA: return &c->gamma;
    case AGZ_K_BN_MEAN: return &c->mean;
    case AGZ_K_BN_VAR: return &c->var;
    default: return nullptr;
  }
}

int64_t Net::param_count(int layer, int kind) const {
  if (const ConvHost* c = conv(layer)) {
    if (kind == AGZ_K_BN_EPS) return 1;
    auto* f = conv_field(const_cast<ConvHost*>(c), kind);
    return f ? (int64_t)f->size() : -1;
  }
  if (const DenseHost* d = dense(layer)) {
    if (kind == AGZ_K_WEIGHT) return (int64_t)d->w.size();
    if (kind == AGZ_K_BIAS) return (int64_t)d->b.size();
  }
  return -1;
}

void Net::set(int layer, int kind, const float* data, int64_t count) {
  AGZ_REQUIRE(data != nullptr, AGZ_BAD_ARGUMENT, "agz_net_set_weights: null data");
  const int64_t want = param_count(layer, kind);
  AGZ_REQUIRE(want >= 0, AGZ_BAD_ARGUMENT, "agz_net_set_weights: no parameter (layer %d, kind %d)", layer, kind);
  AGZ_REQUIRE(want == count, AGZ_BAD_SHAPE, "agz_net_set_weights: layer %d kind %d expects %lld floats, got %lld",
              layer, kind, (long long)want, (long long)count);
  sync_host();
  ++param_version_;
  if (ConvHost* c = conv(layer)) {
    if (kind == AGZ_K_BN_EPS) c->eps = data[0];
    else std::memcpy(conv_field(c, kind)->data(), data, sizeof(float) * (size_t)count);
  } else {
    DenseHost* d = dense(layer);
    std::memcpy((kind == AGZ_K_WEIGHT ? d->w : d->b).data(), data, sizeof(float) * (size_t)count);
  }
  for (const auto& sl : slots_)
    if (sl.layer == layer && sl.kind == kind) upload_slot(sl);
  AGZ_HIP(hipStreamSynchronize(stream_));
}

void Net::get(int layer, int kind, float* out, int64_t count) const {
  AGZ_REQUIRE(out != nullptr, AGZ_BAD_ARGUMENT, "agz_net_get_weights: null output");
  const int64_t want = param_count(layer, kind);
  AGZ_REQUIRE(want >= 0, AGZ_BAD_ARGUMENT, "agz_net_get_weights: no parameter (layer %d, kind %d)", layer, kind);
  AGZ_REQUIRE(want == count, AGZ_BAD_SHAPE, "agz_net_get_weights: layer %d kind %d holds %lld floats, asked %lld",
              layer, kind, (long long)want, (long long)count);
  sync_host();
  if (const ConvHost* c = conv(layer)) {
    if (kind == AGZ_K_BN_EPS) out[0] = c->eps;
    else std::memcpy(out, conv_field(const_cast<ConvHost*>(c), kind)->data(), sizeof(float) * (size_t)count);
  } else {
    const DenseHost* d = dense(layer);
    std::memcpy(out, (kind == AGZ_K_WEIGHT ? d->w : d->b).data(), sizeof(float) * (size_t)count);
  }
}

static void glorot(std::vector<float>& w, double fan_in, double fan_out, uint64_t seed, int layer) {
  const double limit = std::sqrt(6.0 / (fan_in + fan_out));
  const uint64_t key = (uint64_t)(int64_t)(layer + 4096);
  for (size_t i = 0; i < w.size(); ++i) {
    const double u = agz_u01(agz_draw_u64(seed, key, 0, AGZ_SITE_WEIGHTS, (uint64_t)i));
    w[i] = (float)((2.0 * u - 1.0) * limit);
  }
}

void Net::init_synthetic(uint64_t seed) {
  host_stale_ = false;
  ++param_version_;
  for (int l = 0; l <= 2 * tower_; ++l) {
    ConvHost* c = conv(l);
    const int cin = c->cin, cout = c->cout, k = c->k;
    conv_init(*c, k, cin, cout);
    glorot(c->w, 9.0 * cin, 9.0 * cout, seed, l);
  }
  conv_init(vconv_, 1, kC, 1);
  conv_init(pconv_, 1, kC, 2);
  glorot(vconv_.w, kC, 1, seed, AGZ_L_VALUE_CONV);
  glorot(pconv_.w, kC, 2, seed, AGZ_L_POLICY_CONV);
  dense_init(vfc1_, P_, 256);
  dense_init(vfc2_, 256, 1);
  dense_init(pfc_, 2 * P_, A_);
  glorot(vfc1_.w, vfc1_.in, vfc1_.out, seed, AGZ_L_VALUE_FC1);
  glorot(vfc2_.w, vfc2_.in, vfc2_.out, seed, AGZ_L_VALUE_FC2);
  glorot(pfc_.w, pfc_.in, pfc_.out, seed, AGZ_L_POLICY_FC);
  upload_host_all();
}

struct DirectImage : ImageDefaults {
  using word = float;
  static constexpr const char* name = "direct";
  static constexpr int grid_cap = 8192;
  __host__ __device__ static size_t words(int ns) { return (size_t)kC * 9 * 4 * ns; }
  __host__ __device__ static long units(int, int ns) { return (long)words(ns); }
  __host__ __device__ static void put(const float* w, int cin, long idx, int ns, float* out) {
    const int cin_pad = 4 * ns;
    const int ci = (int)(idx % cin_pad), tap = (int)((idx / cin_pad) % 9), o = (int)(idx / ((long)9 * cin_pad));
    out[idx] = ci < cin ? flux_tap(w, cin, tap % 3, tap / 3, ci, o) : 0.f;
  }
};
const ImageFamily kDirectImage = image_family<DirectImage>();

__host__ __device__ inline void bn_affine_one(float gamma, float var, float eps, float beta, float b, float mean, float* scale,
                                              float* shift) {
#pragma clang fp contract(off)
  const double s = (double)gamma / sqrt((double)var + (double)eps);
  *scale = (float)s;
  *shift = (float)((double)beta + s * ((double)b - (double)mean));
}
static void bn_affine(const ConvHost& c, float* scale, float* shift) {
  for (int o = 0; o < c.cout; ++o) bn_affine_one(c.gamma[o], c.var[o], c.eps, c.beta[o], c.b[o], c.mean[o], scale + o, shift + o);
}
__global__ __launch_bounds__(256) void k_bn_affine(const float* __restrict__ base, long stride, int layers, int cout,
                                                   float* __restrict__ scale, float* __restrict__ shift, float* __restrict__ scale2,
                                                   float mul) {
  const int n = layers * cout;
  for (int t = blockIdx.x * 256 + threadIdx.x; t < n; t += gridDim.x * 256) {
    const int l = t / cout, o = t % cout;
    const float* q = base + l * stride;
    float sc, sh;
    bn_affine_one(q[2 * cout + o], q[4 * cout + o], q[5 * cout], q[cout + o], q[o], q[3 * cout + o], &sc, &sh);
    scale[t] = sc;
    shift[t] = sh;
    if (scale2) scale2[t] = sc * mul;
  }
}
__global__ void k_pack_head(const float* __restrict__ vw, const float* __restrict__ pw, float* __restrict__ hp) {
  const int c = threadIdx.x;
  hp[c] = vw[c];
  hp[256 + c] = pw[c];
  hp[512 + c] = pw[kC + c];
  if (c < 8) hp[768 + c] = 0.f;
  __syncthreads();
  if (c == 0) {
    const float* q = vw + kC;
    bn_affine_one(q[2], q[4], q[5], q[1], q[0], q[3], hp + 768, hp + 769);
    const float* r = pw + 2 * kC;
    bn_affine_one(r[4], r[8], r[10], r[2], r[0], r[6], hp + 770, hp + 771);
    bn_affine_one(r[5], r[9], r[10], r[3], r[1], r[7], hp + 772, hp + 773);
  }
}

void Net::pack() {
  const int L = 1 + 2 * tower_;
  const float* F = d_flux_.p;
  auto tstride = [&] { return (long)(flux_offset(2, AGZ_K_WEIGHT) - flux_offset(1, AGZ_K_WEIGHT)); };
  bool launched = false;
  for (BuiltImage& im : images_) {
    if (im.version == param_version_ || !im.needed(*this)) continue;
    const int layers = im.stem ? 1 : 2 * tower_, ns = image_stages(im);
    const size_t bytes = im.family->bytes(ns);
    AGZ_REQUIRE(bytes % 4 == 0, AGZ_BAD_ARGUMENT, "%s image: %zu bytes per layer are not whole 32-bit words", im.family->name, bytes);
    im.buf.ensure(bytes / 4 * layers);
    im.family->device_pack(F + flux_offset(im.stem ? 0 : 1, AGZ_K_WEIGHT), im.stem ? 0 : tstride(), im.stem ? kCinStem : kC, layers,
                           im.buf.p, ns, stream_);
    im.version = param_version_;
    launched = true;
  }
  if (affines_version_ != param_version_) {
    d_scale_.ensure((size_t)L * kC);
    d_shift_.ensure((size_t)L * kC);
    d_scale_s_.ensure((size_t)L * kC);
    hipLaunchKernelGGL(k_bn_affine, dim3(1), dim3(256), 0, stream_, F + flux_offset(0, AGZ_K_BIAS), 0L, 1, kC, d_scale_.p, d_shift_.p,
                       d_scale_s_.p + (size_t)2 * tower_ * kC, wino_split_descale());
    if (tower_ > 0)
      hipLaunchKernelGGL(k_bn_affine, dim3(2 * tower_), dim3(256), 0, stream_, F + flux_offset(1, AGZ_K_BIAS), tstride(), 2 * tower_, kC,
                         d_scale_.p + kC, d_shift_.p + kC, d_scale_s_.p, wino_split_descale());
    d_head_.ensure(776);
    hipLaunchKernelGGL(k_pack_head, dim3(1), dim3(256), 0, stream_, F + flux_offset(AGZ_L_VALUE_CONV, AGZ_K_WEIGHT),
                       F + flux_offset(AGZ_L_POLICY_CONV, AGZ_K_WEIGHT), d_head_.p);
    d_vfc1w_ = F + flux_offset(AGZ_L_VALUE_FC1, AGZ_K_WEIGHT); d_vfc1b_ = F + flux_offset(AGZ_L_VALUE_FC1, AGZ_K_BIAS);
    d_vfc2w_ = F + flux_offset(AGZ_L_VALUE_FC2, AGZ_K_WEIGHT); d_vfc2b_ = F + flux_offset(AGZ_L_VALUE_FC2, AGZ_K_BIAS);
    d_pfcw_ = F + flux_offset(AGZ_L_POLICY_FC, AGZ_K_WEIGHT); d_pfcb_ = F + flux_offset(AGZ_L_POLICY_FC, AGZ_K_BIAS);
    affines_version_ = param_version_;
    launched = true;
  }
  if (launched) AGZ_HIP(hipGetLastError());
}

long Net::debug_pack_diff(int which) {
  pack();
  sync_host();
  if (which < 0 || which > 6) return -1;
  const int L = 1 + 2 * tower_;
  auto diff = [&](const auto* dev, const auto& host) {
    static_assert(sizeof(host[0]) == 4, "debug_pack_diff counts 32-bit words");
    auto got = host;
    download(got.data(), dev, got.size(), stream_);
    AGZ_HIP(hipStreamSynchronize(stream_));
    long bad = 0;
    for (size_t i = 0; i < got.size(); ++i) bad += std::memcmp(&got[i], &host[i], 4) != 0;
    return bad;
  };
  long bad = 0;
  for (const BuiltImage& im : images_) {
    if (im.which != which || !im.needed(*this)) continue;
    std::vector<uint32_t> img(im.family->bytes(image_stages(im)) / 4);
    for (int l = 0; l < (im.stem ? 1 : 2 * tower_); ++l) {
      im.family->host_pack(im.stem ? stem_ : tconv_[l], img.data(), image_stages(im));
      bad += diff(im.buf.p + img.size() * l, img);
    }
  }
  if (which == 4 && images_[kSplitTower].needed(*this)) {
    std::vector<float> sc((size_t)L * kC), tmp(kC);
    for (int l = 0; l <= 2 * tower_; ++l) {
      bn_affine(l < 2 * tower_ ? tconv_[l] : stem_, sc.data() + (size_t)l * kC, tmp.data());
      for (int o = 0; o < kC; ++o) sc[(size_t)l * kC + o] *= wino_split_descale();
    }
    bad += diff(d_scale_s_.p, sc);
  }
  if (which == 5) {
    std::vector<float> scale((size_t)L * kC), shift((size_t)L * kC);
    bn_affine(stem_, scale.data(), shift.data());
    for (int l = 0; l < 2 * tower_; ++l) bn_affine(tconv_[l], scale.data() + (size_t)(l + 1) * kC, shift.data() + (size_t)(l + 1) * kC);
    bad += diff(d_scale_.p, scale) + diff(d_shift_.p, shift);
    std::vector<float> hp(776, 0.f);
    for (int c = 0; c < kC; ++c) { hp[c] = vconv_.w[c]; hp[256 + c] = pconv_.w[c]; hp[512 + c] = pconv_.w[kC + c]; }
    float s[2], t[2];
    bn_affine(vconv_, s, t);
    hp[768] = s[0]; hp[769] = t[0];
    bn_affine(pconv_, s, t);
    hp[770] = s[0]; hp[771] = t[0]; hp[772] = s[1]; hp[773] = t[1];
    bad += diff(d_head_.p, hp);
  }
  return bad;
}

void Net::reserve(int bcap) {
  if (precision_ == 1 && tower_ > 0 && d_ha_.n < ((size_t)std::max(bcap, bcap_) * P_ + 256) * kC) {
    const size_t n = ((size_t)std::max(bcap, bcap_) * P_ + 256) * kC;
    d_ha_.alloc(n);
    d_hb_.alloc(n);
    d_ht_.alloc(n);
  }
  if (bcap <= bcap_) return;
  const size_t rows = (size_t)bcap * P_;
  d_a_.alloc(rows * kC);
  d_b_.alloc(rows * kC);
  d_t_.alloc(rows * kC);
  d_vh_.alloc(rows);
  d_ph_.alloc(rows * 2);
  if (tower_ > 0) {
    const size_t vf = std::max(wino_v_floats(bcap, (N_ + 2) / 3), wino4_applies(N_) ? wino4_v_floats(bcap, N_) : (size_t)0);
    d_vimg_.alloc(vf);
    d_vimg2_.alloc(vf);
  }
  bcap_ = bcap;
}

static inline int conv_grid(int bcap, int P) { return ceil_div((long)bcap * P, BM) * (kC / BN); }
int conv3x3_direct_blocks(int bcap, int N) { return conv_grid(bcap, N * N); }

void launch_conv3x3_direct(const float* x, const float* wt, const float* scale, const float* shift, const float* res,
                           float* y, const int* d_count, int bcap, int N, int relu, int cin_pad, hipStream_t s) {
  const int grid = conv_grid(bcap, N * N);
  if (cin_pad == kCinStemPad)
    hipLaunchKernelGGL((k_conv3x3_mfma<kCinStemPad>), dim3(grid), dim3(256), 0, s, x, wt, scale, shift, res, y, d_count, N, relu);
  else
    hipLaunchKernelGGL((k_conv3x3_mfma<kC>), dim3(grid), dim3(256), 0, s, x, wt, scale, shift, res, y, d_count, N, relu);
}

__global__ __launch_bounds__(256) void k_sum_taps(const float* __restrict__ part, long stride, const float* __restrict__ shift,
                                                   float* __restrict__ y, const int* __restrict__ d_count, int P) {
  const long n4 = (long)(*d_count) * P * (kC / 4);
  for (long i = (long)blockIdx.x * 256 + threadIdx.x; i < n4; i += (long)gridDim.x * 256) {
    float4 s = *reinterpret_cast<const float4*>(part + i * 4);
#pragma unroll
    for (int z = 1; z < 9; ++z) {
      const float4 v = *reinterpret_cast<const float4*>(part + z * stride + i * 4);
      s.x += v.x; s.y += v.y; s.z += v.z; s.w += v.w;
    }
    const float4 b = *reinterpret_cast<const float4*>(shift + (i * 4) % kC);
    *reinterpret_cast<float4*>(y + i * 4) = make_float4(s.x + b.x, s.y + b.y, s.z + b.z, s.w + b.w);
  }
}

void launch_conv3x3_direct_taps(const float* x, const float* wt, const float* ones, const float* zeros, const float* shift,
                                float* y, float* part, const int* d_count, int bcap, int N, int cin_pad, hipStream_t s) {
  const int grid = conv_grid(bcap, N * N);
  const long stride = (long)bcap * N * N * kC;
  if (cin_pad == kCinStemPad)
    hipLaunchKernelGGL((k_conv3x3_mfma<kCinStemPad, true>), dim3(grid, 9), dim3(256), 0, s, x, wt, ones, zeros,
                       (const float*)nullptr, part, d_count, N, 0, stride);
  else
    hipLaunchKernelGGL((k_conv3x3_mfma<kC, true>), dim3(grid, 9), dim3(256), 0, s, x, wt, ones, zeros, (const float*)nullptr,
                       part, d_count, N, 0, stride);
  const int g = (int)std::min<long>(((long)bcap * N * N * (kC / 4) + 255) / 256, 2048);
  hipLaunchKernelGGL(k_sum_taps, dim3(g), dim3(256), 0, s, (const float*)part, stride, shift, y, d_count, N * N);
}

template <class Launch> void Net::timed(int layers, const Launch& launch) {
  const bool p = prof_on_ && prof_n_ < kProfMax;
  if (p) (void)hipEventRecord(prof_ev_[2 * prof_n_], stream_);
  launch();
  if (p) {
    (void)hipEventRecord(prof_ev_[2 * prof_n_ + 1], stream_);
    prof_mult_[prof_n_] = layers;
    prof_fwd_of_[prof_n_++] = prof_fwd_;
  }
}

template <class Layer> void Net::run_chains(int chains, const Layer& layer) {
  const int nl = 2 * tower_;
  if (chains == 1) {
    for (int l = 0; l < nl; ++l) timed(1, [&] { layer(l, 0, stream_); });
    return;
  }
  if (!ev_fork_) AGZ_HIP(hipEventCreateWithFlags(&ev_fork_, hipEventDisableTiming));
  for (int i = 0; i + 1 < chains; ++i)
    if (!streamx_[i]) {
      AGZ_HIP(hipStreamCreateWithFlags(&streamx_[i], hipStreamNonBlocking));
      AGZ_HIP(hipEventCreateWithFlags(&ev_join_[i], hipEventDisableTiming));
    }
  auto join = [&] {
    for (int i = 0; i + 1 < chains; ++i) {
      (void)hipEventRecord(ev_join_[i], streamx_[i]);
      (void)hipStreamWaitEvent(stream_, ev_join_[i], 0);
    }
  };
  timed(nl, [&] {
    AGZ_HIP(hipEventRecord(ev_fork_, stream_));
    for (int i = 0; i + 1 < chains; ++i) AGZ_HIP(hipStreamWaitEvent(streamx_[i], ev_fork_, 0));
    try {
      for (int part = 0; part < chains; ++part)
        for (int l = 0; l < nl; ++l) layer(l, part, part == 0 ? stream_ : streamx_[part - 1]);
    } catch (...) {
      join();
      throw;
    }
    join();
  });
}

static int chain_count(int streams, long tiles, int rows) {
  return (int)std::max<long>(1, std::min<long>(streams, (tiles + rows - 1) / rows / 256));
}

void Net::check_async_error() {
  if (tower_err_ && *tower_err_) {
    const int err = *tower_err_;
    *tower_err_ = 0;
    AGZ_REQUIRE(false, AGZ_HIP_ERROR,
                "the persistent tower kernel of an earlier forward gave up (scheduler error word %d: 1 = more than 32 "
                "workgroups on one XCD, 2 = a tile block's producer never arrived); its outputs were garbage", err);
  }
}

void Net::stem(TowerForm form, const float* d_x32, const int* d_count, int bcap) {
  float* a = d_a_.p;
  if (winograd_ == 0 || tower_ == 0) {
    launch_conv3x3_direct(d_x32, image<float>(kDirectStem), d_scale_.p, d_shift_.p, nullptr, a, d_count, bcap, N_, 1, kCinStemPad, stream_);
  } else if (form == TowerForm::F16 || form == TowerForm::Wino4) {
    float* v = form == TowerForm::F16 ? d_vimg_.p : d_vimg2_.p;
    launch_wino_in(d_x32, v, d_count, bcap, N_, false, stream_, kWinoStemStages);
    launch_wino_gemm(v, image<float>(kWinoStem), d_scale_.p, d_shift_.p, nullptr, a, nullptr, d_count, bcap, N_, 1, false, stream_,
                     kWinoStemStages);
    if (form == TowerForm::Wino4) launch_wino4_in(a, d_vimg_.p, d_count, bcap, N_, stream_, false);
  } else {
    const bool split = precision_ == 2;
    launch_wino_in(d_x32, d_vimg2_.p, d_count, bcap, N_, split, stream_, kWinoStemStages);
    launch_wino_gemm(d_vimg2_.p, image<float>(split ? kSplitStem : kWinoStem), split ? d_scale_s_.p + (size_t)2 * tower_ * kC : d_scale_.p,
                     d_shift_.p, nullptr, a, d_vimg_.p, d_count, bcap, N_, 1, split, stream_, kWinoStemStages);
    if (!wino_fusable(N_)) launch_wino_in(a, d_vimg_.p, d_count, bcap, N_, split, stream_, kWinoStages, true);
  }
}

void Net::direct_tower(const int* d_count, int bcap) {
  const float* sc = d_scale_.p + kC;
  const float* sh = d_shift_.p + kC;
  float *a = d_a_.p, *b = d_b_.p, *t = d_t_.p;
  for (int blk = 0; blk < tower_; ++blk) {
    const int l1 = 2 * blk, l2 = 2 * blk + 1;
    timed(1, [&] {
      launch_conv3x3_direct(a, image<float>(kDirectTower, l1), sc + (size_t)l1 * kC, sh + (size_t)l1 * kC, nullptr, t, d_count, bcap,
                            N_, 1, kC, stream_);
    });
    timed(1, [&] {
      launch_conv3x3_direct(t, image<float>(kDirectTower, l2), sc + (size_t)l2 * kC, sh + (size_t)l2 * kC, a, b, d_count, bcap, N_, 1,
                            kC, stream_);
    });
    std::swap(a, b);
  }
}

void Net::f16_tower(const int* d_count, int bcap) {
  const float* sc = d_scale_.p + kC;
  const float* sh = d_shift_.p + kC;
  const float* a = d_a_.p;
  uint16_t *cur = d_hb_.p, *nxt = d_ha_.p;
  launch_f32_to_f16(a, cur, d_count, bcap, N_, stream_);
  for (int blk = 0; blk < tower_; ++blk) {
    const int l1 = 2 * blk, l2 = 2 * blk + 1;
    const bool first = blk == 0, last = blk + 1 == tower_;
    timed(1, [&] {
      launch_conv16_dma(cur, image<uint16_t>(kF16Tower, l1), sc + (size_t)l1 * kC, sh + (size_t)l1 * kC, nullptr, 0, d_ht_.p, 0,
                        d_count, bcap, N_, 1, stream_);
    });
    timed(1, [&] {
      launch_conv16_dma(d_ht_.p, image<uint16_t>(kF16Tower, l2), sc + (size_t)l2 * kC, sh + (size_t)l2 * kC,
                        first ? (const void*)a : (const void*)cur, first ? 1 : 0, last ? (void*)d_b_.p : (void*)nxt,
                        last ? 1 : 0, d_count, bcap, N_, 1, stream_);
    });
    std::swap(cur, nxt);
  }
}

Net::LayerIO Net::layer_io(int l, bool dense) const {
  if (l % 2 == 0) return {d_vimg_.p, nullptr, dense ? d_t_.p : nullptr, d_vimg2_.p};
  const bool odd = (l / 2) % 2;
  return {d_vimg2_.p, odd ? d_b_.p : d_a_.p, odd ? d_a_.p : d_b_.p, l + 1 == 2 * tower_ ? nullptr : d_vimg_.p};
}

void Net::wino_layer(TowerForm form, int l, const LayerIO& io, const int* d_count, int bcap, hipStream_t st, int part, int parts) {
  const float* sc = d_scale_.p + (size_t)(l + 1) * kC;
  const float* sh = d_shift_.p + (size_t)(l + 1) * kC;
  if (form == TowerForm::Wino4) {
    launch_wino4_gemm(io.vin, image<float>(kWino4Tower, l), sc, sh, io.res, io.y, io.vout, d_count, bcap, N_, 1, st,
                      part, parts, io.y && !io.res && wino4_paired(N_));
    if (io.vout && !wino4_whole_boards(N_)) launch_wino4_in(io.y, io.vout, d_count, bcap, N_, st, true, part, parts);
  } else if (form == TowerForm::Wino5) {
    launch_wino5_gemm(io.vin, image<float>(kWino5Tower, l), sc, sh, io.res, io.y, io.vout, d_count, bcap, N_, 1, st,
                      part, parts);
  } else {
    const bool split = precision_ == 2;
    const float* u = image<float>(split ? kSplitTower : kWinoTower, l);
    launch_wino_gemm(io.vin, u, split ? d_scale_s_.p + (size_t)l * kC : sc, sh, io.res, io.y, io.vout, d_count, bcap, N_, 1, split,
                     st, kWinoStages, part, parts);
    if (io.vout && !wino_fusable(N_)) launch_wino_in(io.y, io.vout, d_count, bcap, N_, split, st, kWinoStages, true);
  }
}

void Net::wino_tower(TowerForm form, const int* d_count, int bcap) {
  const bool f44 = form == TowerForm::Wino4;
  const bool dense = f44 ? !wino4_whole_boards(N_) : !wino_fusable(N_);
  const int T = f44 ? (N_ + 3) / 4 : (N_ + 2) / 3;
  const int chains = dense && !f44 ? 1 : chain_count(tower_streams_, (long)bcap * T * T, f44 ? 64 : 63);
  run_chains(chains, [&](int l, int part, hipStream_t st) {
    wino_layer(form, l, layer_io(l, dense), d_count, bcap, st, part, chains);
  });
}

void Net::persistent_tower(const int* d_count, int bcap) {
  const bool split = precision_ == 2;
  const ImageId u = split ? kSplitTower : kWinoTower;
  const float* sc = split ? d_scale_s_.p : d_scale_.p + kC;
  const float* sh = d_shift_.p + kC;
  const int nl = 2 * tower_;
  std::vector<WinoTowerLayer> tab(nl);
  for (int l = 0; l < nl; ++l) {
    const LayerIO io = layer_io(l, false);
    tab[l] = {io.vin, image<float>(u, l), sc + (size_t)l * kC, sh + (size_t)l * kC, io.res, io.y, io.vout,
              (io.y ? 1 : 0) | (io.vout ? 2 : 0), 1};
  }
  const size_t tbytes = sizeof(WinoTowerLayer) * tab.size();
  if (tower_layers_host_.size() != tbytes || std::memcmp(tower_layers_host_.data(), tab.data(), tbytes) != 0) {
    AGZ_HIP(hipStreamSynchronize(stream_));
    tower_layers_host_.assign((const char*)tab.data(), (const char*)tab.data() + tbytes);
    d_tower_layers_.ensure(tbytes);
    AGZ_HIP(hipMemcpy(d_tower_layers_.p, tower_layers_host_.data(), tbytes, hipMemcpyHostToDevice));
  }
  d_tower_sched_.ensure(wino_tower_sched_ints(nl, bcap, N_));
  if (!tower_err_) {
    AGZ_HIP(hipHostMalloc((void**)&tower_err_, sizeof(int32_t), hipHostMallocDefault));
    *tower_err_ = 0;
  }
  timed(nl, [&] { launch_wino_tower(d_tower_layers_.p, nl, d_tower_sched_.p, d_count, bcap, N_, split, stream_); });
  (void)hipMemcpyAsync(tower_err_, d_tower_sched_.p + kWinoTowerErrWord, sizeof(int32_t), hipMemcpyDeviceToHost, stream_);
}

void Net::forward(const float* d_x32, const int* d_count, int bcap, float* d_pi, float* d_v) {
  check_async_error();
  TowerForm form = tower_form();
  if (form == TowerForm::Wino4) wino4_validate(bcap, N_);
  pack();
  reserve(bcap);
  if (prof_on_ && prof_fwd_ < kProfMax)
    (void)hipMemcpyAsync(&prof_counts_[prof_fwd_], d_count, sizeof(int32_t), hipMemcpyDeviceToHost, stream_);
  stem(form, d_x32, d_count, bcap);
  if (form == TowerForm::Wino3Persistent && !wino_tower_supported(stream_)) form = TowerForm::Wino3;
  switch (form) {
    case TowerForm::Direct: direct_tower(d_count, bcap); break;
    case TowerForm::F16: f16_tower(d_count, bcap); break;
    case TowerForm::Wino3Persistent: persistent_tower(d_count, bcap); break;
    default: wino_tower(form, d_count, bcap); break;
  }
  const float* x = form == TowerForm::F16 || tower_ % 2 ? d_b_.p : d_a_.p;
  const int hgrid = std::min(ceil_div((long)bcap * P_, 4), 256 * 16);
  hipLaunchKernelGGL(k_head_conv, dim3(hgrid), dim3(256), 0, stream_, x, d_head_.p, d_vh_.p, d_ph_.p, d_count, P_);
  const size_t smem = sizeof(float) * (size_t)(3 * P_ + A_ + 4);
  hipLaunchKernelGGL(k_head_fc, dim3(bcap), dim3(256), smem, stream_, (const float*)d_vh_.p,
                     (const float*)d_ph_.p, d_vfc1w_, d_vfc1b_, d_vfc2w_, d_vfc2b_, d_pfcw_,
                     d_pfcb_, d_pi, d_v, d_count, P_, A_);
  if (prof_on_ && prof_fwd_ < kProfMax) prof_fwd_++;
  AGZ_HIP(hipGetLastError());
}

__global__ __launch_bounds__(256) void k_mfma_f32_sustained(int iters, float* out) {
  typedef float f32x16 __attribute__((ext_vector_type(16)));
  f32x16 acc[8];
#pragma unroll
  for (int i = 0; i < 8; ++i)
#pragma unroll
    for (int e = 0; e < 16; ++e) acc[i][e] = 0.f;
  const float a = 1.f + threadIdx.x * 1e-6f, b = 0.5f;
  for (int it = 0; it < iters; ++it) {
#pragma unroll
    for (int i = 0; i < 8; ++i) acc[i] = __builtin_amdgcn_mfma_f32_32x32x2f32(a, b, acc[i], 0, 0, 0);
  }
  float s = 0.f;
#pragma unroll
  for (int i = 0; i < 8; ++i) s += acc[i][0] + acc[i][15];
  if (s == 123.456f) out[0] = s;
}

template <bool F16, bool DENSE>
__global__ __launch_bounds__(256) void k_mfma_sustained_data(int iters, float* out) {
  typedef float f32x16 __attribute__((ext_vector_type(16)));
  typedef _Float16 h8 __attribute__((ext_vector_type(8)));
  f32x16 acc[8];
#pragma unroll
  for (int i = 0; i < 8; ++i)
#pragma unroll
    for (int e = 0; e < 16; ++e) acc[i][e] = 0.f;
  unsigned st = 0x9e3779b9u * (threadIdx.x + 256u * blockIdx.x + 1u);
  auto rnd = [&]() { st = st * 1664525u + 1013904223u; return (float)(int)(st >> 8) * (1.0f / 8388608.0f) - 1.0f; };
  float a32[16], b32[16];
  h8 a16[16], b16[16];
#pragma unroll
  for (int k = 0; k < 16; ++k) {
    a32[k] = rnd(); b32[k] = DENSE ? rnd() : fmaxf(rnd(), 0.f) * 2.f;
#pragma unroll
    for (int e = 0; e < 8; ++e) {
      a16[k][e] = (_Float16)(0.06f * rnd());
      b16[k][e] = (_Float16)(DENSE ? rnd() : fmaxf(rnd(), 0.f) * 2.f);
    }
  }
  for (int it = 0; it < iters; it += 16) {
#pragma unroll
    for (int u = 0; u < 16; ++u)
#pragma unroll
      for (int i = 0; i < 8; ++i) {
        if (F16) acc[i] = __builtin_amdgcn_mfma_f32_32x32x16_f16(a16[(i + u) & 15], b16[(3 * i + 5 * u) & 15], acc[i], 0, 0, 0);
        else acc[i] = __builtin_amdgcn_mfma_f32_32x32x2f32(a32[(i + u) & 15], b32[(3 * i + 5 * u) & 15], acc[i], 0, 0, 0);
      }
  }
  float s = 0.f;
#pragma unroll
  for (int i = 0; i < 8; ++i) s += acc[i][0] + acc[i][15];
  if (s == 123.456f) out[0] = s;
}

float Net::mfma_sustained_tflops(int millis, int mode) {
  AGZ_REQUIRE(millis >= 50 && millis <= 5000, AGZ_BAD_ARGUMENT, "mfma_sustained_tflops: %d ms (50..5000)", millis);
  AGZ_REQUIRE(mode >= 0 && mode <= 4, AGZ_BAD_ARGUMENT, "mfma_sustained_tflops: mode %d", mode);
  const bool f16 = mode == 2 || mode == 4;
  DevBuf<float> out;
  out.alloc(16);
  hipEvent_t e0, e1;
  AGZ_HIP(hipEventCreate(&e0));
  AGZ_HIP(hipEventCreate(&e1));
  const int iters = f16 ? 20000 : 10000, grid = 1024;
  const double flop = (double)grid * 4 * iters * 8.0 * (f16 ? 32768.0 : 4096.0);
  std::vector<double> tf;
  double spent = 0.0;
  while (spent < millis) {
    AGZ_HIP(hipEventRecord(e0, stream_));
    if (mode == 0) hipLaunchKernelGGL(k_mfma_f32_sustained, dim3(grid), dim3(256), 0, stream_, iters, out.p);
    else if (mode == 1) hipLaunchKernelGGL((k_mfma_sustained_data<false, false>), dim3(grid), dim3(256), 0, stream_, iters, out.p);
    else if (mode == 2) hipLaunchKernelGGL((k_mfma_sustained_data<true, false>), dim3(grid), dim3(256), 0, stream_, iters, out.p);
    else if (mode == 3) hipLaunchKernelGGL((k_mfma_sustained_data<false, true>), dim3(grid), dim3(256), 0, stream_, iters, out.p);
    else hipLaunchKernelGGL((k_mfma_sustained_data<true, true>), dim3(grid), dim3(256), 0, stream_, iters, out.p);
    AGZ_HIP(hipEventRecord(e1, stream_));
    AGZ_HIP(hipEventSynchronize(e1));
    float ms = 0.f;
    AGZ_HIP(hipEventElapsedTime(&ms, e0, e1));
    tf.push_back(flop / (ms * 1e-3) / 1e12);
    spent += ms;
  }
  (void)hipEventDestroy(e0);
  (void)hipEventDestroy(e1);
  std::vector<double> tail(tf.begin() + tf.size() / 2, tf.end());
  std::sort(tail.begin(), tail.end());
  return (float)tail[tail.size() / 2];
}

Net::~Net() {
  for (auto e : prof_ev_) (void)hipEventDestroy(e);
  if (prof_counts_) (void)hipHostFree(prof_counts_);
  if (tower_err_) (void)hipHostFree(tower_err_);
  if (ev_fork_) (void)hipEventDestroy(ev_fork_);
  for (auto e : ev_join_)
    if (e) (void)hipEventDestroy(e);
  for (auto st : streamx_)
    if (st) (void)hipStreamDestroy(st);
}

void Net::profile_enable(bool on) {
  if (on && prof_ev_.empty()) {
    prof_ev_.resize(2 * kProfMax);
    for (auto& e : prof_ev_) AGZ_HIP(hipEventCreate(&e));
    prof_fwd_of_.assign(kProfMax, 0);
    prof_mult_.assign(kProfMax, 1);
    AGZ_HIP(hipHostMalloc((void**)&prof_counts_, sizeof(int32_t) * kProfMax, hipHostMallocDefault));
  }
  prof_on_ = on;
  prof_n_ = 0;
  prof_fwd_ = 0;
}

void Net::profile_read(double* total_ms, double* total_flop, int64_t* launches) {
  AGZ_HIP(hipStreamSynchronize(stream_));
  double ms = 0.0, fl = 0.0;
  int64_t n = 0;
  for (int i = 0; i < prof_n_; ++i) {
    float t = 0.f;
    AGZ_HIP(hipEventElapsedTime(&t, prof_ev_[2 * i], prof_ev_[2 * i + 1]));
    ms += t;
    const int f = prof_fwd_of_[i];
    fl += prof_mult_[i] * conv_flops_per_launch(f < kProfMax ? prof_counts_[f] : 0);
    n += prof_mult_[i];
  }
  *total_ms = ms;
  *total_flop = fl;
  *launches = n;
}

void Net::launch_tower_conv_once(const int* d_count, int bcap) {
  pack();
  reserve(bcap);
  AGZ_REQUIRE(tower_ > 0, AGZ_BAD_ARGUMENT, "no tower conv in a tower_height=0 network");
  const TowerForm form = tower_form();
  if (form == TowerForm::F16)
    launch_conv16_dma(d_ha_.p, image<uint16_t>(kF16Tower), d_scale_.p + kC, d_shift_.p + kC, nullptr, 0, d_ht_.p, 0, d_count, bcap, N_, 1,
                      stream_);
  else if (form == TowerForm::Direct)
    launch_conv3x3_direct(d_a_.p, image<float>(kDirectTower), d_scale_.p + kC, d_shift_.p + kC, nullptr, d_t_.p, d_count, bcap, N_, 1, kC,
                          stream_);
  else
    wino_layer(form, 0, {d_vimg_.p, d_a_.p, d_t_.p, d_vimg2_.p}, d_count, bcap, stream_);
  AGZ_HIP(hipGetLastError());
}

double Net::flops_per_eval() const {
  const double P = P_;
  return 2.0 * P * (9.0 * 17 * 256 + tower_ * 2.0 * 9 * 256 * 256) + 2.0 * P * 256 * 3 +
         2.0 * (2.0 * P * (P + 1) + P * 256 + 256);
}

}
```

### alphago.jl_amd/csrc/agz_wino.hip

```cpp
#include "agz_nn.h"
#include "agz_pack.h"
#include "agz_glds.h"

#include <algorithm>
#include <cmath>
#include <cstdio>
#include <cstdlib>
#include <cstring>
#include <type_traits>

namespace agz {

typedef float f32x16 __attribute__((ext_vector_type(16)));

constexpr int WT = 64;
constexpr int WC = 64;
constexpr int WK = 4;
constexpr int WNS = kC / WK;
static_assert(WNS == kWinoStages && kCinStemPad == kWinoStemStages * WK, "stage counts of agz_nn.h");
constexpr int WXI = 25;
constexpr int WPL = 13;
constexpr int A_STAGE = WPL * WT * 8;
constexpr int B_STAGE = WPL * WC * 8;
constexpr int STAGE = A_STAGE + B_STAGE;

__host__ __device__ __forceinline__ int wino_v_off(int xi, int row, int h) {
  return (xi >> 1) * (WT * 8) + (xi & 1) * (WT * 4) + row * 4 + 2 * ((h + (row >> 4)) & 1);
}

typedef _Float16 h8 __attribute__((ext_vector_type(8)));
typedef _Float16 h4 __attribute__((ext_vector_type(4)));
constexpr float kSplitV = 8.f, kSplitU = 1024.f;
__host__ __device__ __forceinline__ void split_half(float x, _Float16& hi, _Float16& lo) {
  hi = (_Float16)x;
  lo = (_Float16)(x - (float)hi);
}
__host__ __device__ __forceinline__ int wino_vs_off(int xi, int row) { return (xi >> 1) * (WT * 8) + (xi & 1) * (WT * 4) + row * 4; }

__host__ __device__ inline int wino_rows_per_block(int T) {
  const int tt = T * T;
  const int whole = (WT / tt) * tt;
  return (tt <= WT && whole * 10 >= WT * 9) ? whole : WT;
}
__host__ __device__ inline bool wino_whole_boards(int T) { return wino_rows_per_block(T) % (T * T) == 0 && T * T <= WT; }

__host__ __device__ __forceinline__ bool wino_tile_fused(int T, int row, int ti, int tj) {
  const int lo = (ti > 0 ? T : 0) + (tj > 0 ? 1 : 0), hi = (ti < T - 1 ? T : 0) + (tj < T - 1 ? 1 : 0);
  return row - lo >= 0 && row + hi < WT;
}


__device__ __forceinline__ void bt5(float x0, float x1, float x2, float x3, float x4, float* r) {
  r[3] = x3 - x1;
  r[0] = __builtin_fmaf(2.f, x0 - x2, r[3]);
  r[4] = __builtin_fmaf(-2.f, r[3], x4 - x2);
  r[1] = __builtin_fmaf(2.f, x1, x2 - x3);
  r[2] = __builtin_fmaf(-2.f, x1, __builtin_fmaf(3.f, x2, -x3));
}

template <int TPB, bool NT, bool SPLIT = false, int NS = WNS, bool FIXUP = false>
__global__ __launch_bounds__(256) void k_wino_in(const float* __restrict__ x, float* __restrict__ vimg,
                                                  const int* __restrict__ d_count, int N, int T) {
  static_assert(TPB == 32, "the copy-out below moves 32-row chunks");
  constexpr int LPT = 256 / TPB;
  constexpr int SP = LPT / 2;
  constexpr int CH = TPB * 4;
  constexpr int IMG = 26 * CH + 8;
  __shared__ __attribute__((aligned(16))) float img[SP * IMG];
  const int P = N * N, TT = T * T;
  const int RPB = wino_rows_per_block(T);
  const long Mt = (long)(*d_count) * TT;
  constexpr int PARTS = WT / TPB;
  const int tb = blockIdx.x / PARTS, part = blockIdx.x % PARTS;
  if ((long)tb * RPB + part * TPB >= Mt) return;
  const int hs = threadIdx.x % LPT, h = hs & 1, sl = hs >> 1;
  const int tl = threadIdx.x / LPT;
  const int row = part * TPB + tl;
  const long tile = (long)tb * RPB + row;
  bool live = row < RPB && tile < Mt;
  const int b = live ? (int)(tile / TT) : 0, t = live ? (int)(tile % TT) : 0;
  const int ti = t / T, tj = t % T;
  if (FIXUP && live && wino_tile_fused(T, row, ti, tj)) live = false;
  int off[25];
#pragma unroll
  for (int u = 0; u < 5; ++u)
#pragma unroll
    for (int v = 0; v < 5; ++v) {
      const int pi = 3 * ti - 1 + u, pj = 3 * tj - 1 + v;
      const bool ok = live && pi >= 0 && pi < N && pj >= 0 && pj < N;
      off[u * 5 + v] = ok ? (b * P + pi + N * pj) * (NS * WK) : -1;
    }
  float* mine = img + sl * IMG + tl * 4 + (SPLIT ? 0 : 2 * ((h + (row >> 4)) & 1));
  if (SPLIT) { mine[25 * CH + h] = 0.f; mine[25 * CH + 2 + h] = 0.f; }
  else *reinterpret_cast<float2*>(mine + 25 * CH) = make_float2(0.f, 0.f);
  float* gdst = vimg + (long)tb * NS * A_STAGE + part * CH;
  const int cq = threadIdx.x / TPB, cl = threadIdx.x % TPB;
  bool copy_row = true;
  if (FIXUP) {
    const int crow = part * TPB + cl;
    const long ctile = (long)tb * RPB + crow;
    const int ct = (int)(ctile % TT);
    copy_row = !(crow < RPB && ctile < Mt && wino_tile_fused(T, crow, ct / T, ct % T));
  }
  for (int sg = 0; sg < NS / SP; ++sg) {
    const int st = sg * SP + sl;
    float2 d[25];
#pragma unroll
    for (int q = 0; q < 25; ++q)
      d[q] = off[q] >= 0 ? *reinterpret_cast<const float2*>(x + off[q] + st * WK + 2 * h) : make_float2(0.f, 0.f);
    float tx[25], ty[25];
#pragma unroll
    for (int v = 0; v < 5; ++v) {
      float r[5];
      bt5(d[0 * 5 + v].x, d[1 * 5 + v].x, d[2 * 5 + v].x, d[3 * 5 + v].x, d[4 * 5 + v].x, r);
#pragma unroll
      for (int i = 0; i < 5; ++i) tx[i * 5 + v] = r[i];
      bt5(d[0 * 5 + v].y, d[1 * 5 + v].y, d[2 * 5 + v].y, d[3 * 5 + v].y, d[4 * 5 + v].y, r);
#pragma unroll
      for (int i = 0; i < 5; ++i) ty[i * 5 + v] = r[i];
    }
    if (sg) __syncthreads();
#pragma unroll
    for (int i = 0; i < 5; ++i) {
      float rx[5], ry[5];
      bt5(tx[i * 5 + 0], tx[i * 5 + 1], tx[i * 5 + 2], tx[i * 5 + 3], tx[i * 5 + 4], rx);
      bt5(ty[i * 5 + 0], ty[i * 5 + 1], ty[i * 5 + 2], ty[i * 5 + 3], ty[i * 5 + 4], ry);
#pragma unroll
      for (int j = 0; j < 5; ++j) {
        if (SPLIT) {
          _Float16 xh, xl, yh, yl;
          split_half(kSplitV * rx[j], xh, xl);
          split_half(kSplitV * ry[j], yh, yl);
          typedef _Float16 h2 __attribute__((ext_vector_type(2)));
          *reinterpret_cast<h2*>(mine + (i * 5 + j) * CH + h) = (h2){xh, yh};
          *reinterpret_cast<h2*>(mine + (i * 5 + j) * CH + 2 + h) = (h2){xl, yl};
        } else {
          *reinterpret_cast<float2*>(mine + (i * 5 + j) * CH) = make_float2(rx[j], ry[j]);
        }
      }
    }
    __syncthreads();
#pragma unroll
    for (int r = 0; r < 13; ++r) {
      const int c = r * 8 + cq, s4 = c / 26, xi = c % 26;
      typedef float f32x4 __attribute__((ext_vector_type(4)));
      const f32x4 v = *reinterpret_cast<const f32x4*>(img + s4 * IMG + xi * CH + cl * 4);
      f32x4* gp = reinterpret_cast<f32x4*>(gdst + (long)(sg * SP + s4) * A_STAGE + (xi >> 1) * (WT * 8) + (xi & 1) * (WT * 4) + cl * 4);
      if (FIXUP && !copy_row) continue;
      if (NT) __builtin_nontemporal_store(v, gp);
      else *gp = v;
    }
  }
}

constexpr int IMG_FLOATS = WT * 9 * WC;

template <bool SPLIT, int NS, bool COH>
__device__ __forceinline__ void wino_wg(
    float* __restrict__ lds, int* __restrict__ ptab, const float* __restrict__ vimg, const float* __restrict__ uimg,
    const float* __restrict__ scale, const float* __restrict__ shift, const float* __restrict__ res, float* __restrict__ y,
    float* __restrict__ vnext, const long Mt, const int N, const int T, const int relu, const int tb, const int cb, const int MODE,
    const int tid) {
  const int P = N * N, TT = T * T;
  const int RPB = wino_rows_per_block(T);
  const int lane = tid & 63;
  const int wave = __builtin_amdgcn_readfirstlane(tid >> 6);
  const int wm = wave & 1, wn = wave >> 1;
  const int l31 = lane & 31, hi = lane >> 5;
  const float* asrc = vimg + (long)tb * NS * A_STAGE;
  const float* bsrc = uimg + (long)cb * NS * B_STAGE;
  const unsigned lds0 = (unsigned)(size_t)(__attribute__((address_space(3))) float*)&lds[0];

  auto dma = [&](int st, int buf, int j) {
    const int c = 13 * wave + j;
    if (j == 12 && (wave & 1)) return;
    const float* g = wave < 2 ? asrc + (long)st * A_STAGE + c * 256 : bsrc + (long)st * B_STAGE + (c - 26) * 256;
    if constexpr (COH) glds16s_l2(g, (unsigned)lane * 16u, lds0 + (unsigned)(buf * STAGE + c * 256) * 4u);
    else glds16s(g, (unsigned)lane * 16u, lds0 + (unsigned)(buf * STAGE + c * 256) * 4u);
  };

#pragma unroll
  for (int j = 0; j < 13; ++j) dma(0, 0, j);

  for (int idx = tid; idx < WT * 9; idx += 256) {
    const int row = idx & (WT - 1), k = idx >> 6;
    const long tile = (long)tb * RPB + row;
    int off = -1;
    if (row < RPB && tile < Mt) {
      const unsigned tile32 = (unsigned)tile, b = tile32 / (unsigned)TT, t = tile32 - b * (unsigned)TT;
      const unsigned ti = t / (unsigned)T, k3 = (unsigned)k / 3u;
      const int pi = (int)(3 * ti + k3), pj = (int)(3 * (t - ti * T) + ((unsigned)k - 3 * k3));
      if (pi < N && pj < N) off = ((int)b * P + pi + N * pj) * kC + cb * WC;
    }
    ptab[idx] = off;
  }
#pragma unroll
  for (int j = 0; j < 13; ++j) dma(1, 1, j);

  f32x16 acc[WXI];

  const int arow = wm * 32 + l31, brow = wn * 32 + l31;
  const int aoff[2] = {wino_v_off(0, arow, hi), wino_v_off(1, arow, hi)};
  constexpr int LA = 4, RING = LA + 1;
  typedef float f32x4 __attribute__((ext_vector_type(4)));
  typedef typename std::conditional<SPLIT, f32x4, float2>::type a_t;
  a_t ra[RING];
  float2 rb[RING];
  const int asoff[2] = {wino_vs_off(0, arow), wino_vs_off(1, arow)};
  const int bsoff[2] = {A_STAGE + wino_v_off(0, brow, hi), A_STAGE + wino_v_off(1, brow, hi)};
  auto load = [&](const float* L, int xi, a_t& a, float2& b) {
    if constexpr (SPLIT) {
      a = *reinterpret_cast<const f32x4*>(L + asoff[xi & 1] + (xi >> 1) * (WT * 8));
      b = *reinterpret_cast<const float2*>(L + bsoff[xi & 1] + (xi >> 1) * (WC * 8));
    } else {
      a = *reinterpret_cast<const float2*>(L + aoff[xi & 1] + (xi >> 1) * (WT * 8));
      b = *reinterpret_cast<const float2*>(L + bsoff[xi & 1] + (xi >> 1) * (WC * 8));
    }
  };

  auto in_agpr = [](int k) { return k % 5 < 3; };
  const f32x16 zero16 = {0.f, 0.f, 0.f, 0.f, 0.f, 0.f, 0.f, 0.f, 0.f, 0.f, 0.f, 0.f, 0.f, 0.f, 0.f, 0.f};
  auto mma0 = [&](int k, const a_t& a, const float2& b) {
    if constexpr (SPLIT) {
      const h8 ah = __builtin_bit_cast(h8, a);
      const f32x4 bb = {b.x, b.y, b.x, b.y};
      const h8 bh = __builtin_bit_cast(h8, bb);
      if (in_agpr(k)) acc[k] = __builtin_amdgcn_mfma_f32_32x32x16_f16(ah, bh, zero16, 0, 0, 0);
      else asm volatile("s_nop 1\n\tv_mfma_f32_32x32x16_f16 %0, %1, %2, 0" : "=&v"(acc[k]) : "v"(ah), "v"(bh));
    } else if (in_agpr(k)) {
      acc[k] = __builtin_amdgcn_mfma_f32_32x32x2f32(a.x, b.x, zero16, 0, 0, 0);
      acc[k] = __builtin_amdgcn_mfma_f32_32x32x2f32(a.y, b.y, acc[k], 0, 0, 0);
    } else {
      asm volatile("s_nop 1\n\tv_mfma_f32_32x32x2_f32 %0, %1, %2, 0\n\tv_mfma_f32_32x32x2_f32 %0, %3, %4, %0"
                   : "=&v"(acc[k])
                   : "v"(a.x), "v"(b.x), "v"(a.y), "v"(b.y));
    }
  };
  auto mma = [&](int k, const a_t& a, const float2& b) {
    if constexpr (SPLIT) {
      const h8 ah = __builtin_bit_cast(h8, a);
      const f32x4 bb = {b.x, b.y, b.x, b.y};
      const h8 bh = __builtin_bit_cast(h8, bb);
      if (in_agpr(k)) acc[k] = __builtin_amdgcn_mfma_f32_32x32x16_f16(ah, bh, acc[k], 0, 0, 0);
      else asm volatile("s_nop 1\n\tv_mfma_f32_32x32x16_f16 %0, %1, %2, %0" : "+v"(acc[k]) : "v"(ah), "v"(bh));
    } else if (in_agpr(k)) {
      acc[k] = __builtin_amdgcn_mfma_f32_32x32x2f32(a.x, b.x, acc[k], 0, 0, 0);
      acc[k] = __builtin_amdgcn_mfma_f32_32x32x2f32(a.y, b.y, acc[k], 0, 0, 0);
    } else {
      asm volatile("s_nop 1\n\tv_mfma_f32_32x32x2_f32 %0, %1, %2, %0\n\tv_mfma_f32_32x32x2_f32 %0, %3, %4, %0"
                   : "+v"(acc[k])
                   : "v"(a.x), "v"(b.x), "v"(a.y), "v"(b.y));
    }
  };

  constexpr int PW = 13;
  auto wait_stage = [&]() {
    if (wave & 1) asm volatile("s_waitcnt vmcnt(12)" ::: "memory");
    else asm volatile("s_waitcnt vmcnt(13)" ::: "memory");
  };
  wait_stage();
  __syncthreads();
#pragma unroll
  for (int k = 0; k < LA; ++k) load(lds, k, ra[k], rb[k]);

  auto rdma = [&](int n) {
    const int i = wave + 4 * n;
    const int Xp = 4 * i + (lane >> 4), u = lane & 15;
    const int off = ptab[Xp];
    const unsigned boff = off >= 0 ? 4u * (unsigned)(off + 4 * (u ^ (Xp & 15))) : 0u;
    if constexpr (COH) glds16s_l2(res, boff, lds0 + (unsigned)(i * 256) * 4u);
    else glds16s(res, boff, lds0 + (unsigned)(i * 256) * 4u);
  };
  int buf = 0;
  auto stage = [&](int st, auto more_c, auto next_c, auto first_c) {
    constexpr bool more = decltype(more_c)::value, next = decltype(next_c)::value, first = decltype(first_c)::value;
    const int nbuf = buf == 2 ? 0 : buf + 1;
    const int dbuf = buf == 0 ? 2 : buf - 1;
    const float* L = lds + buf * STAGE;
    const float* Ln = lds + nbuf * STAGE;
#pragma unroll
    for (int k = 0; k < WXI; ++k) {
      const int t = k + LA;
      if (t == WXI && next) {
        if (more) wait_stage();
        else asm volatile("s_waitcnt vmcnt(0)" ::: "memory");
        __syncthreads();
      }
      if (t < WXI) load(L, t, ra[t % RING], rb[t % RING]);
      else if (next) load(Ln, t - WXI, ra[t % RING], rb[t % RING]);
      constexpr int D0 = SPLIT ? 0 : 6;
      if (more && k >= D0 && k < D0 + PW) {
        __builtin_amdgcn_sched_barrier(0);
        dma(st + 2, dbuf, k - D0);
        __builtin_amdgcn_sched_barrier(0);
      }
      if (first) mma0(k, ra[k % RING], rb[k % RING]);
      else mma(k, ra[k % RING], rb[k % RING]);
    }
    buf = nbuf;
  };
  static_assert(NS >= 4, "stage 0 is peeled off the loop");
  stage(0, std::true_type{}, std::true_type{}, std::true_type{});
  for (int st = 1; st < NS - 2; ++st) stage(st, std::true_type{}, std::true_type{}, std::false_type{});
  stage(NS - 2, std::false_type{}, std::true_type{}, std::false_type{});
  stage(NS - 1, std::false_type{}, std::false_type{}, std::false_type{});

  static_assert(WXI == 25, "the pad below lists the accumulators of transform columns 3 and 4");
  asm volatile("s_nop 15\n\ts_nop 15"
               : "+v"(acc[3]), "+v"(acc[4]), "+v"(acc[8]), "+v"(acc[9]), "+v"(acc[13]), "+v"(acc[14]), "+v"(acc[18]),
                 "+v"(acc[19]), "+v"(acc[23]), "+v"(acc[24]));

  __syncthreads();
  float* img = lds;
  static_assert(IMG_FLOATS + WC <= 3 * STAGE, "tile image (+ the block of zeros phase 2 reads for off-board points) exceeds the stage buffers");
  if (tid < WC) img[IMG_FLOATS + tid] = 0.f;
  const bool pass1b = (MODE & 1) != 0;
  if (res) {
    static_assert(WT * 9 / 4 == 4 * 36, "36 residual pieces per wave");
#pragma unroll
    for (int n = 0; n < 36; ++n) rdma(n);
  }
  {
    const int col = wn * 32 + l31;
    const float sc = scale[cb * WC + col], sh = shift[cb * WC + col];
    const float relu_lo = relu ? 0.f : -3.0e38f;
    f32x16 o[9];
    {
      f32x16 tmp[3][5];
#pragma unroll
      for (int jj = 0; jj < 5; ++jj) {
        const int j = (jj + 3) % 5;
        const f32x16 m0 = acc[0 * 5 + j], m1 = acc[1 * 5 + j], m2 = acc[2 * 5 + j], m3 = acc[3 * 5 + j], m4 = acc[4 * 5 + j];
        tmp[0][j] = ((m0 + m1) + m2) + m3;
        tmp[1][j] = (m1 - m2) + 2.f * m3;
        tmp[2][j] = ((m1 + m2) + 4.f * m3) + m4;
        __builtin_amdgcn_sched_barrier(0);
      }
#pragma unroll
      for (int i = 0; i < 3; ++i) {
        o[i * 3 + 0] = ((tmp[i][0] + tmp[i][1]) + tmp[i][2]) + tmp[i][3];
        o[i * 3 + 1] = (tmp[i][1] - tmp[i][2]) + 2.f * tmp[i][3];
        o[i * 3 + 2] = ((tmp[i][1] + tmp[i][2]) + 4.f * tmp[i][3]) + tmp[i][4];
      }
    }
    if (res) {
      asm volatile("s_waitcnt vmcnt(0)" ::: "memory");
      __syncthreads();
    }
    auto rows = [&](auto with_res) {
#pragma unroll
      for (int e0 = 0; e0 < 16; e0 += 4) {
        typedef __attribute__((address_space(3))) float lds_f;
        unsigned pa[4][3];
        float rr[4][9];
#pragma unroll
        for (int ee = 0; ee < 4; ++ee) {
          const int e = e0 + ee, row = wm * 32 + (e & 3) + 8 * (e >> 2) + 4 * hi;
          pa[ee][0] = lds0 + 4u * (unsigned)(row * WC + 4 * ((col >> 2) ^ (row & 15)) + (col & 3));
          pa[ee][1] = pa[ee][0] + 4u * 4 * (WT * WC);
          pa[ee][2] = pa[ee][0] + 4u * 8 * (WT * WC);
          asm volatile("" : "+v"(pa[ee][1]), "+v"(pa[ee][2]));
#pragma unroll
          for (int k = 0; k < 9; ++k)
            rr[ee][k] = decltype(with_res)::value ? *((lds_f*)(size_t)pa[ee][k >> 2] + (k & 3) * (WT * WC)) : 0.f;
        }
#pragma unroll
        for (int ee = 0; ee < 4; ++ee)
#pragma unroll
          for (int k = 0; k < 9; ++k) {
            float v = o[k][e0 + ee] * sc + sh + rr[ee][k];
            v = fmaxf(v, relu_lo);
            *((lds_f*)(size_t)pa[ee][k >> 2] + (k & 3) * (WT * WC)) = v;
          }
      }
    };
    if (res) rows(std::true_type{});
    else rows(std::false_type{});
  }
  __syncthreads();
  typedef float f32x4 __attribute__((ext_vector_type(4)));
  if (pass1b) {
    constexpr int PER = WT * 9 * (WC / 4) / 256;
    const int cg4 = 4 * ((tid ^ (tid >> 4)) & 15);
    f32x4* ip0 = reinterpret_cast<f32x4*>(img) + tid;
    const int* pt0 = ptab + (tid >> 4);
    int offs[PER];
#pragma unroll
    for (int i = 0; i < PER; ++i) offs[i] = pt0[16 * i];
#pragma unroll
    for (int i0 = 0; i0 < PER; i0 += 12) {
      f32x4 v[12];
#pragma unroll
      for (int j = 0; j < 12; ++j) v[j] = ip0[256 * (i0 + j)];
#pragma unroll
      for (int j = 0; j < 12; ++j)
        if ((MODE & 1) && offs[i0 + j] >= 0) *reinterpret_cast<f32x4*>(y + offs[i0 + j] + cg4) = v[j];
    }
  }
  if (!(MODE & 2)) return;

  {
    const int row = lane;
    const long tile = (long)tb * RPB + row;
    const bool live = row < RPB && tile < Mt;
    const int t = live ? (int)(tile % TT) : 0;
    const int ti = t / T, tj = t % T;
    const bool emit = wino_whole_boards(T) || (live && wino_tile_fused(T, row, ti, tj));
    unsigned adr[25];
#pragma unroll
    for (int u = 0; u < 5; ++u)
#pragma unroll
      for (int v = 0; v < 5; ++v) {
        const int du = u == 0 ? -1 : (u == 4 ? 1 : 0), ku = u == 0 ? 2 : (u == 4 ? 0 : u - 1);
        const int dv = v == 0 ? -1 : (v == 4 ? 1 : 0), kv = v == 0 ? 2 : (v == 4 ? 0 : v - 1);
        const int pi = 3 * ti - 1 + u, pj = 3 * tj - 1 + v;
        const bool ok = live && emit && pi >= 0 && pi < N && pj >= 0 && pj < N;
        const int Xq = (ku * 3 + kv) * WT + row + du * T + dv;
        const int pb = ok ? Xq * WC : IMG_FLOATS, xm = ok ? (Xq & 15) : 0;
        adr[u * 5 + v] = lds0 + 4u * (unsigned)(pb + 4 * (wave ^ xm) + (SPLIT ? 0 : 2 * ((row >> 4) & 1)));
      }
    typedef float f32x2 __attribute__((ext_vector_type(2)));
    static_assert(WC / WK == 16, "four stages per wave");
#pragma unroll 1
    for (int it = 0; it < 4; ++it) {
      const int sl = wave + 4 * it;
      const unsigned xo = (unsigned)it << 6;
      f32x4 d[25];
#pragma unroll
      for (int q = 0; q < 25; ++q) {
        const unsigned a0 = adr[q] ^ xo;
        if constexpr (SPLIT) {
          d[q] = *(const __attribute__((address_space(3))) f32x4*)(size_t)a0;
        } else {
          const f32x2 a = *(const __attribute__((address_space(3))) f32x2*)(size_t)a0;
          const f32x2 b = *(const __attribute__((address_space(3))) f32x2*)(size_t)(a0 ^ 8u);
          d[q] = (f32x4){a[0], a[1], b[0], b[1]};
        }
      }
      float* g = vnext + ((long)tb * WNS + (cb * (WC / WK) + sl)) * A_STAGE + row * 4;
      auto bt5p = [](f32x2 x0, f32x2 x1, f32x2 x2, f32x2 x3, f32x2 x4, f32x2* r) {
        const f32x2 two = {2.f, 2.f}, mtwo = {-2.f, -2.f}, three = {3.f, 3.f};
        r[3] = x3 - x1;
        r[0] = __builtin_elementwise_fma(two, x0 - x2, r[3]);
        r[4] = __builtin_elementwise_fma(mtwo, r[3], x4 - x2);
        r[1] = __builtin_elementwise_fma(two, x1, x2 - x3);
        r[2] = __builtin_elementwise_fma(mtwo, x1, __builtin_elementwise_fma(three, x2, -x3));
      };
      f32x2 vv[25][2];
#pragma unroll
      for (int h = 0; h < 2; ++h) {
        f32x2 tx[25];
#pragma unroll
        for (int v = 0; v < 5; ++v) {
          f32x2 r[5], c[5];
#pragma unroll
          for (int u = 0; u < 5; ++u) c[u] = (f32x2){d[u * 5 + v][2 * h], d[u * 5 + v][2 * h + 1]};
          bt5p(c[0], c[1], c[2], c[3], c[4], r);
#pragma unroll
          for (int i = 0; i < 5; ++i) tx[i * 5 + v] = r[i];
        }
#pragma unroll
        for (int i = 0; i < 5; ++i) {
          f32x2 r[5];
          bt5p(tx[i * 5 + 0], tx[i * 5 + 1], tx[i * 5 + 2], tx[i * 5 + 3], tx[i * 5 + 4], r);
#pragma unroll
          for (int j = 0; j < 5; ++j) vv[i * 5 + j][h] = r[j];
        }
      }
#pragma unroll
      for (int xi = 0; xi < WXI; ++xi) {
        const f32x2 p0 = vv[xi][0], p1 = vv[xi][1];
        f32x4 v4;
        if constexpr (SPLIT) {
          _Float16 ah[4], al[4];
          split_half(kSplitV * p0[0], ah[0], al[0]);
          split_half(kSplitV * p0[1], ah[1], al[1]);
          split_half(kSplitV * p1[0], ah[2], al[2]);
          split_half(kSplitV * p1[1], ah[3], al[3]);
          const h8 pk = {ah[0], ah[1], ah[2], ah[3], al[0], al[1], al[2], al[3]};
          v4 = __builtin_bit_cast(f32x4, pk);
        } else {
          v4 = (f32x4){p0[0], p0[1], p1[0], p1[1]};
        }
        f32x4* gp = reinterpret_cast<f32x4*>(g + (xi >> 1) * (WT * 8) + (xi & 1) * (WT * 4));
        if (emit) __builtin_nontemporal_store(v4, gp);
      }
    }
  }
}

template <int MODE, bool SPLIT = false, int NS = WNS>
__global__ __launch_bounds__(256, 1) void k_wino_gemm4(
    const float* __restrict__ vimg, const float* __restrict__ uimg, const float* __restrict__ scale,
    const float* __restrict__ shift, const float* __restrict__ res, float* __restrict__ y,
    float* __restrict__ vnext, const int* __restrict__ d_count, int N, int T, int relu, int tb0, int tb1) {
  __shared__ __attribute__((aligned(256))) float lds[3 * STAGE];
  __shared__ int ptab[WT * 9];
  const long Mt = (long)(*d_count) * (T * T);
  const int bid = blockIdx.x;
  const int xcd = bid & 7, jb = bid >> 3;
  const int cb = jb & 3;
  const int tb = tb0 + xcd + 8 * (jb >> 2);
  if (tb >= tb1 || (long)tb * wino_rows_per_block(T) >= Mt) return;
  wino_wg<SPLIT, NS, false>(lds, ptab, vimg, uimg, scale, shift, res, y, vnext, Mt, N, T, relu, tb, cb, MODE, (int)threadIdx.x);
}

typedef WinoTowerLayer TowerLayer;
static_assert(kWinoTowerErrWord == 8, "");
constexpr int kTowerErr = kWinoTowerErrWord, kTowerDone = 64;
constexpr int kTowerSpinLimit = 1 << 22;

template <bool SPLIT>
__global__ __launch_bounds__(256, 1) void k_wino_tower(const TowerLayer* __restrict__ layers, int nl, int* __restrict__ sched,
                                                       int blocks_cap, const int* __restrict__ d_count, int N, int T, int order) {
  __shared__ __attribute__((aligned(256))) float lds[3 * STAGE];
  __shared__ int ptab[WT * 9];
  __shared__ int s_bc;
  const int tid = threadIdx.x;
  unsigned xcc;
  asm volatile("s_getreg_b32 %0, hwreg(HW_REG_XCC_ID)" : "=s"(xcc));
  const int xcd = (int)(xcc & 7u);
  if (tid == 0) s_bc = atomicAdd(&sched[xcd], 1);
  __syncthreads();
  const int slot = s_bc;
  if (slot >= 32) {
    if (tid == 0) atomicOr(&sched[kTowerErr], 1);
    return;
  }
  const int quad = slot >> 2, cb = slot & 3;
  const int RPB = wino_rows_per_block(T);
  const long Mt = (long)(*d_count) * (T * T);
  const int blocks = (int)((Mt + RPB - 1) / RPB);
  const int nbx = blocks > xcd ? (blocks - xcd + 7) >> 3 : 0;
  const int total = nl * nbx;
  int* done = sched + kTowerDone;
  const int nitems = order == 0 ? (total > quad ? (total - quad + 7) >> 3 : 0) : (nbx > quad ? ((nbx - quad + 7) >> 3) * nl : 0);
  for (int k = 0; k < nitems; ++k) {
    int l, tb;
    if (order == 0) {
      const int item = quad + 8 * k;
      l = item / nbx;
      tb = xcd + 8 * (item - l * nbx);
    } else {
      const int j = k / nl;
      l = k - j * nl;
      tb = xcd + 8 * (quad + 8 * j);
    }
    if (tid == 0) s_bc = 0;
    if (l > 0 && tid == 0) {
      const int* flag = done + (size_t)(l - 1) * blocks_cap + tb;
      int spins = 0;
      while (__hip_atomic_load(flag, __ATOMIC_RELAXED, __HIP_MEMORY_SCOPE_AGENT) < 4) {
        __builtin_amdgcn_s_sleep(8);
        if (++spins > kTowerSpinLimit || ((spins & 1023) == 0 && __hip_atomic_load(&sched[kTowerErr], __ATOMIC_RELAXED, __HIP_MEMORY_SCOPE_AGENT))) {
          atomicOr(&sched[kTowerErr], 2);
          s_bc = 1;
          break;
        }
      }
    }
    __syncthreads();
    if (s_bc) return;
    const TowerLayer L = layers[l];
    int t = tid;
    asm volatile("" : "+v"(t));
    wino_wg<SPLIT, WNS, true>(lds, ptab, L.v, L.u, L.scale, L.shift, L.res, L.y, L.vnext, Mt, N, T, L.relu, tb, cb, L.mode, t);
    asm volatile("s_waitcnt vmcnt(0)" ::: "memory");
    __syncthreads();
    if (tid == 0) {
      int* flag = done + (size_t)l * blocks_cap + tb;
      if (__hip_atomic_fetch_add(flag, 1, __ATOMIC_RELAXED, __HIP_MEMORY_SCOPE_AGENT) != 3) {
        int spins = 0;
        while (__hip_atomic_load(flag, __ATOMIC_RELAXED, __HIP_MEMORY_SCOPE_AGENT) < 4 && ++spins < kTowerSpinLimit) __builtin_amdgcn_s_sleep(2);
      }
    }
  }
}

__global__ void k_xcd_census(int* out) {
  __shared__ float hog[150 * 1024 / 4];
  unsigned xcc;
  asm volatile("s_getreg_b32 %0, hwreg(HW_REG_XCC_ID)" : "=s"(xcc));
  if (threadIdx.x == 0) {
    hog[0] = 1.f;
    atomicAdd(&out[xcc & 7u], 1);
    const long long t0 = wall_clock64();
    while ((long long)wall_clock64() - t0 < 10000) __builtin_amdgcn_s_sleep(32);
    if (hog[0] == 2.f) out[8] = 1;
  }
}


template <bool SPLIT>
struct WinoImage : ImageDefaults {
  using word = float;
  static constexpr const char* name = SPLIT ? "split F(3x3,3x3)" : "F(3x3,3x3)";
  static constexpr bool zeroed = true;
  __host__ __device__ static size_t words(int ns) { return (size_t)(kC / WC) * ns * B_STAGE; }
  __host__ __device__ static long units(int cin, int) { return (long)kC * cin; }
  __host__ __device__ static void put(const float* w, int cin, long unit, int ns, float* out) {
#pragma clang fp contract(off)
    const int o = (int)(unit / cin), ci = (int)(unit % cin);
    const int cb = o / WC, ol = o % WC, st = ci / WK, cl = ci % WK;
    winograd_u<5>(w, cin, o, ci, [&](int i, int j, double u) {
      const int xi = i * 5 + j;
      if (SPLIT) {
        _Float16* o16 = reinterpret_cast<_Float16*>(out);
        _Float16 hi, lo;
        split_half((float)(u * (double)kSplitU), hi, lo);
        const size_t base = ((size_t)cb * ns + st) * B_STAGE;
        o16[2 * (base + wino_v_off(xi, ol, 0)) + cl] = hi;
        o16[2 * (base + wino_v_off(xi, ol, 1)) + cl] = lo;
      } else {
        out[((size_t)cb * ns + st) * B_STAGE + wino_v_off(xi, ol, cl >> 1) + (cl & 1)] = (float)u;
      }
    });
  }
};
const ImageFamily kWinoImage = image_family<WinoImage<false>>(), kWinoSplitImage = image_family<WinoImage<true>>();
float wino_split_descale() { return 1.f / (kSplitV * kSplitU); }

long wino_blocks(int bcap, int T) {
  const long rpb = wino_rows_per_block(T);
  return ((long)bcap * T * T + rpb - 1) / rpb;
}
size_t wino_v_floats(int bcap, int T) { return (size_t)wino_blocks(bcap, T) * WNS * A_STAGE; }
bool wino_fusable(int N) { return wino_whole_boards((N + 2) / 3); }

void launch_wino_in(const float* x, float* vimg, const int* d_count, int bcap, int N, bool split, hipStream_t s, int ns,
                    bool fixup) {
  const int T = (N + 2) / 3;
  const int blocks = (int)wino_blocks(bcap, T);
  AGZ_REQUIRE(!fixup || (ns == kWinoStages && !wino_whole_boards(T)), AGZ_BAD_ARGUMENT, "fix-up transform: dense tile blocks, tower layers");
#define WIN_LAUNCH(SPLIT_, NS_, FIXUP_) \
  hipLaunchKernelGGL((k_wino_in<32, true, SPLIT_, NS_, FIXUP_>), dim3(2 * blocks), dim3(256), 0, s, x, vimg, d_count, N, T)
  constexpr int S = kWinoStemStages;
  switch ((fixup ? 4 : ns == S ? 2 : 0) | (split ? 1 : 0)) {
    case 5: WIN_LAUNCH(true, WNS, true); break;
    case 4: WIN_LAUNCH(false, WNS, true); break;
    case 3: WIN_LAUNCH(true, S, false); break;
    case 2: WIN_LAUNCH(false, S, false); break;
    case 1: WIN_LAUNCH(true, WNS, false); break;
    default: WIN_LAUNCH(false, WNS, false); break;
  }
#undef WIN_LAUNCH
}

void launch_wino_gemm(const float* vimg, const float* uimg, const float* scale, const float* shift, const float* res,
                      float* y, float* vnext, const int* d_count, int bcap, int N, int relu, bool split, hipStream_t s, int ns, int part,
                      int parts) {
  const int T = (N + 2) / 3;
  const int all_blocks = (int)wino_blocks(bcap, T);
  int tb0, tb1;
  wino_block_range(all_blocks, part, parts, false, tb0, tb1);
  AGZ_REQUIRE(parts == 1 || wino_whole_boards(T), AGZ_BAD_ARGUMENT, "F(3x3,3x3): %d layer chains need whole-board tile blocks", parts);
  if (tb1 <= tb0) return;
  const int blocks = tb1 - tb0;
  const int per_xcd = 4 * ((blocks + 7) / 8);
  const dim3 grid(8 * per_xcd), block(256);
  wino_check_32bit(all_blocks, WT, bcap, N);
  const bool stem = ns == kWinoStemStages;
  const int mode = vnext ? (y || stem ? 3 : 2) : 1;
#define WG_LAUNCH(MODE_, SPLIT_, NS_)                                                                                     \
  hipLaunchKernelGGL((k_wino_gemm4<MODE_, SPLIT_, NS_>), grid, block, 0, s, vimg, uimg, scale, shift, res, y, vnext, d_count, \
                     N, T, relu, tb0, tb1)
  constexpr int S = kWinoStemStages;
  switch (mode | (split ? 4 : 0) | (stem ? 8 : 0)) {
    case 15: WG_LAUNCH(3, true, S); break;
    case 13: WG_LAUNCH(1, true, S); break;
    case 11: WG_LAUNCH(3, false, S); break;
    case 9: WG_LAUNCH(1, false, S); break;
    case 7: WG_LAUNCH(3, true, WNS); break;
    case 6: WG_LAUNCH(2, true, WNS); break;
    case 5: WG_LAUNCH(1, true, WNS); break;
    case 3: WG_LAUNCH(3, false, WNS); break;
    case 2: WG_LAUNCH(2, false, WNS); break;
    default: WG_LAUNCH(1, false, WNS); break;
  }
#undef WG_LAUNCH
}

size_t wino_tower_sched_ints(int layers, int bcap, int N) {
  const int T = (N + 2) / 3;
  return (size_t)kTowerDone + (size_t)layers * wino_blocks(bcap, T);
}

bool wino_tower_supported(hipStream_t s) {
  static int cached[64];
  int dev = 0;
  if (hipGetDevice(&dev) != hipSuccess || dev < 0 || dev >= 64) return false;
  if (cached[dev]) return cached[dev] == 1;
  hipDeviceProp_t prop;
  bool ok = hipGetDeviceProperties(&prop, dev) == hipSuccess && prop.multiProcessorCount == 256;
  if (ok) {
    int* d = nullptr;
    int h[9] = {0};
    ok = hipMalloc((void**)&d, sizeof(h)) == hipSuccess;
    if (ok) {
      (void)hipMemsetAsync(d, 0, sizeof(h), s);
      hipLaunchKernelGGL(k_xcd_census, dim3(256), dim3(64), 0, s, d);
      ok = hipMemcpyAsync(h, d, sizeof(h), hipMemcpyDeviceToHost, s) == hipSuccess && hipStreamSynchronize(s) == hipSuccess;
      (void)hipFree(d);
      for (int x = 0; ok && x < 8; ++x) ok = h[x] == 32;
    }
  }
  cached[dev] = ok ? 1 : 2;
  return ok;
}

void launch_wino_tower(const void* d_layers, int layers, int* d_sched, const int* d_count, int bcap, int N, bool split, hipStream_t s) {
  const int T = (N + 2) / 3;
  AGZ_REQUIRE(wino_whole_boards(T), AGZ_BAD_ARGUMENT, "the persistent tower kernel needs whole-board tile blocks");
  wino_check_32bit(wino_blocks(bcap, T), WT, bcap, N);
  const int blocks_cap = (int)wino_blocks(bcap, T);
  (void)hipMemsetAsync(d_sched, 0, sizeof(int) * wino_tower_sched_ints(layers, bcap, N), s);
  constexpr int order = 0;
  if (split)
    hipLaunchKernelGGL((k_wino_tower<true>), dim3(256), dim3(256), 0, s, (const TowerLayer*)d_layers, layers, d_sched, blocks_cap, d_count, N, T, order);
  else
    hipLaunchKernelGGL((k_wino_tower<false>), dim3(256), dim3(256), 0, s, (const TowerLayer*)d_layers, layers, d_sched, blocks_cap, d_count, N, T, order);
}

}
```

### include/agz_debug.h

```cpp
#ifndef AGZ_DEBUG_H
#define AGZ_DEBUG_H

#include "agz.h"

#ifdef __cplusplus
extern "C" {
#endif

agz_status agz_debug_draws(agz_engine* e, uint64_t seed, uint64_t game, uint32_t move, int32_t n,
                           double alpha, double* gamma_out);
agz_status agz_debug_math(agz_engine* e, int32_t op, const double* x, const double* y, int32_t n,
                          double* out);
int32_t agz_debug_counters(agz_engine* e, uint64_t* out, int32_t cap);
agz_status agz_debug_set_stagger(agz_engine* e, int32_t moves);

agz_status agz_debug_live_record(agz_engine* e, int32_t g, int32_t k, uint64_t* game_id_out, int32_t* num_moves_out,
                                 int32_t* move_out, float* pi_out, float* q_out);

agz_status agz_debug_mfma_sustained(agz_engine* e, int32_t millis, float* tflops_out);
agz_status agz_debug_mfma_sustained_data(agz_engine* e, int32_t millis, int32_t mode, float* tflops_out);
agz_status agz_debug_pack_diff(agz_engine* e, int32_t which, int64_t* mismatches_out);

#ifdef __cplusplus
}
#endif

#endif
```

Before: 453.9.

## Precompute Winograd workgroup gather table and batch head FC over four boards

Adds a per-board-size table of tile offsets and tile coordinates that is built once on the device. Winograd GEMM and tower workgroups now DMA it into LDS instead of recomputing the per-row address arithmetic (divisions and modulo) each call. The head FC kernel also processes four boards per block so each policy and value weight load is reused four times. The costs are extra LDS for the table and more registers and serial block reductions in the head kernel.

```diff
diff --git a/alphago.jl_amd/_lib.py b/alphago.jl_amd/_lib.py
--- a/alphago.jl_amd/_lib.py
+++ b/alphago.jl_amd/_lib.py
@@ -237,6 +237,7 @@
         "agz_debug_live_record": (i32, [E, i32, i32, P(u64), i32p, i32p, f32p, f32p]),
         "agz_debug_mfma_sustained": (i32, [E, i32, C.POINTER(C.c_float)]),
         "agz_debug_pack_diff": (i32, [E, i32, P(i64)]),
+        "agz_debug_wino_wg_table": (i32, [i32, i32p, i32]),
         "agz_debug_mfma_sustained_data": (i32, [E, i32, i32, C.POINTER(C.c_float)]),
     }
     for name, (res, args) in sig.items():
diff --git a/alphago.jl_amd/csrc/agz_capi.hip b/alphago.jl_amd/csrc/agz_capi.hip
--- a/alphago.jl_amd/csrc/agz_capi.hip
+++ b/alphago.jl_amd/csrc/agz_capi.hip
@@ -744,6 +744,14 @@
 agz_status agz_debug_mfma_sustained_data(agz_engine* e, int32_t millis, int32_t mode, float* tflops_out) {
   return guard(e, [&](agz::Engine& E) { *tflops_out = E.net().mfma_sustained_tflops(millis, mode); });
 }
+agz_status agz_debug_wino_wg_table(int32_t N, int32_t* out, int32_t capacity) {
+  if (!out || N < 1 || !agz::wino_fusable(N) || capacity < agz::kWinoWgTableInts) {
+    g_create_error = "workgroup table: a board with whole-board tile blocks (N <= 12) and room for 641 ints";
+    return AGZ_BAD_ARGUMENT;
+  }
+  agz::wino_wg_table_host(N, out);
+  return AGZ_OK;
+}
 agz_status agz_debug_pack_diff(agz_engine* e, int32_t which, int64_t* mismatches_out) {
   return guard(e, [&](agz::Engine& E) { *mismatches_out = (int64_t)E.net().debug_pack_diff(which); });
 }
diff --git a/alphago.jl_amd/csrc/agz_glds.h b/alphago.jl_amd/csrc/agz_glds.h
--- a/alphago.jl_amd/csrc/agz_glds.h
+++ b/alphago.jl_amd/csrc/agz_glds.h
@@ -19,6 +19,13 @@
                : "=&s"(keep) : "v"(lane_byte_off), "s"(gbase_uniform), "s"(lds_byte_addr) : "memory");
 }
 
+__device__ __forceinline__ void glds4s(const int* gbase_uniform, unsigned lane_byte_off, unsigned lds_byte_addr) {
+  unsigned keep;
+  lds_byte_addr = __builtin_amdgcn_readfirstlane(lds_byte_addr);
+  asm volatile("s_mov_b32 %0, m0\n\ts_mov_b32 m0, %3\n\ts_nop 0\n\tglobal_load_lds_dword %1, %2\n\ts_mov_b32 m0, %0"
+               : "=&s"(keep) : "v"(lane_byte_off), "s"(gbase_uniform), "s"(lds_byte_addr) : "memory");
+}
+
 __device__ __forceinline__ void glds16_l2(const float* g, unsigned lds_byte_addr) {
   unsigned keep;
   lds_byte_addr = __builtin_amdgcn_readfirstlane(lds_byte_addr);
diff --git a/alphago.jl_amd/csrc/agz_nn.h b/alphago.jl_amd/csrc/agz_nn.h
--- a/alphago.jl_amd/csrc/agz_nn.h
+++ b/alphago.jl_amd/csrc/agz_nn.h
@@ -169,6 +169,8 @@
   hipEvent_t ev_fork_ = nullptr, ev_join_[kMaxTowerStreams - 1] = {nullptr, nullptr, nullptr};
   DevBuf<float> d_scale_s_;
   DevBuf<float> d_vimg_, d_vimg2_;
+  DevBuf<int> d_wg_table_;
+  const int* wg_table() const { return d_wg_table_.p; }
   int precision_ = 0;
   DevBuf<uint16_t> d_ha_, d_hb_, d_ht_;
   bool tower_persistent_ = false;
@@ -230,9 +232,12 @@
 }
 void launch_wino_in(const float* x, float* vimg, const int* d_count, int bcap, int N, bool split, hipStream_t s,
                     int ns = kWinoStages, bool fixup = false);
+constexpr int kWinoWgTableInts = 641;
+void wino_wg_table_host(int N, int* out);
+void launch_wino_wg_table(int N, int* d_out, hipStream_t s);
 void launch_wino_gemm(const float* vimg, const float* uimg, const float* scale, const float* shift, const float* res,
                       float* y, float* vnext, const int* d_count, int bcap, int N, int relu, bool split, hipStream_t s,
-                      int ns = kWinoStages, int part = 0, int parts = 1);
+                      int ns = kWinoStages, int part = 0, int parts = 1, const int* wg_table = nullptr);
 bool wino_fusable(int N);
 struct WinoTowerLayer {
   const float *v, *u, *scale, *shift, *res;
@@ -241,7 +246,8 @@
 };
 size_t wino_tower_sched_ints(int layers, int bcap, int N);
 bool wino_tower_supported(hipStream_t s);
-void launch_wino_tower(const void* d_layers, int layers, int* d_sched, const int* d_count, int bcap, int N, bool split, hipStream_t s);
+void launch_wino_tower(const void* d_layers, int layers, int* d_sched, const int* d_count, int bcap, int N, bool split, hipStream_t s,
+                       const int* wg_table = nullptr);
 constexpr int kWinoTowerErrWord = 8;
 float wino_split_descale();
 
diff --git a/alphago.jl_amd/csrc/agz_nn.hip b/alphago.jl_amd/csrc/agz_nn.hip
--- a/alphago.jl_amd/csrc/agz_nn.hip
+++ b/alphago.jl_amd/csrc/agz_nn.hip
@@ -182,46 +182,76 @@
   return r;
 }
 
+constexpr int kHeadFcG = 4;
 __global__ __launch_bounds__(256) void k_head_fc(
     const float* __restrict__ vh, const float* __restrict__ ph, const float* __restrict__ w1,
     const float* __restrict__ b1, const float* __restrict__ w2, const float* __restrict__ b2,
     const float* __restrict__ wp, const float* __restrict__ bp, float* __restrict__ pi,
     float* __restrict__ v, const int* __restrict__ d_count, int P, int A) {
+  constexpr int G = kHeadFcG;
   extern __shared__ __attribute__((aligned(16))) float sm[];
   float* vin = sm;
-  float* pin = sm + P;
-  float* logit = pin + 2 * P;
-  float* red = logit + A;
-  const int b = blockIdx.x;
-  if (b >= *d_count) return;
+  float* pin = vin + G * P;
+  float* logit = pin + G * 2 * P;
+  float* red = logit + G * A;
+  const int b0 = blockIdx.x * G, count = *d_count;
+  if (b0 >= count) return;
   const int tid = threadIdx.x;
-  for (int i = tid; i < P; i += 256) {
-    vin[i] = vh[(long)b * P + i];
-    pin[i] = ph[((long)b * P + i) * 2 + 0];
-    pin[P + i] = ph[((long)b * P + i) * 2 + 1];
+  for (int g = 0; g < G; ++g) {
+    const int b = b0 + g;
+    const bool on = b < count;
+    for (int i = tid; i < P; i += 256) {
+      vin[g * P + i] = on ? vh[(long)b * P + i] : 0.f;
+      pin[g * 2 * P + i] = on ? ph[((long)b * P + i) * 2 + 0] : 0.f;
+      pin[g * 2 * P + P + i] = on ? ph[((long)b * P + i) * 2 + 1] : 0.f;
+    }
   }
   __syncthreads();
-  float lmax = -INFINITY;
+  float lmax[G];
+#pragma unroll
+  for (int g = 0; g < G; ++g) lmax[g] = -INFINITY;
   for (int o = tid; o < A; o += 256) {
-    float z = bp[o];
-    for (int i = 0; i < 2 * P; ++i) z += wp[o + (long)A * i] * pin[i];
-    logit[o] = z;
-    lmax = fmaxf(lmax, z);
-  }
-  const float mx = block_reduce(lmax, true, red);
-  float lsum = 0.f;
-  for (int o = tid; o < A; o += 256) {
-    const float e = expf(logit[o] - mx);
-    logit[o] = e;
-    lsum += e;
-  }
-  const float sum = block_reduce(lsum, false, red);
-  for (int o = tid; o < A; o += 256) pi[(long)b * A + o] = logit[o] / sum;
-  float h = b1[tid];
-  for (int i = 0; i < P; ++i) h += w1[tid + 256 * i] * vin[i];
-  h = fmaxf(h, 0.f);
-  const float s = block_reduce(h * w2[tid], false, red);
-  if (tid == 0) v[b] = tanhf(s + b2[0]);
+    float z[G];
+#pragma unroll
+    for (int g = 0; g < G; ++g) z[g] = bp[o];
+    for (int i = 0; i < 2 * P; ++i) {
+      const float w = wp[o + (long)A * i];
+#pragma unroll
+      for (int g = 0; g < G; ++g) z[g] += w * pin[g * 2 * P + i];
+    }
+#pragma unroll
+    for (int g = 0; g < G; ++g) {
+      logit[g * A + o] = z[g];
+      lmax[g] = fmaxf(lmax[g], z[g]);
+    }
+  }
+  float h[G];
+#pragma unroll
+  for (int g = 0; g < G; ++g) h[g] = b1[tid];
+  for (int i = 0; i < P; ++i) {
+    const float w = w1[tid + 256 * i];
+#pragma unroll
+    for (int g = 0; g < G; ++g) h[g] += w * vin[g * P + i];
+  }
+  const float w2t = w2[tid];
+#pragma unroll
+  for (int g = 0; g < G; ++g) {
+    const int b = b0 + g;
+    const bool on = b < count;
+    float* lg = logit + g * A;
+    const float mx = block_reduce(lmax[g], true, red);
+    float lsum = 0.f;
+    for (int o = tid; o < A; o += 256) {
+      const float e = expf(lg[o] - mx);
+      lg[o] = e;
+      lsum += e;
+    }
+    const float sum = block_reduce(lsum, false, red);
+    if (on)
+      for (int o = tid; o < A; o += 256) pi[(long)b * A + o] = lg[o] / sum;
+    const float s = block_reduce(fmaxf(h[g], 0.f) * w2t, false, red);
+    if (on && tid == 0) v[b] = tanhf(s + b2[0]);
+  }
 }
 
 
@@ -541,6 +571,11 @@
     im.family->device_pack(F + flux_offset(im.stem ? 0 : 1, AGZ_K_WEIGHT), im.stem ? 0 : tstride(), im.stem ? kCinStem : kC, layers,
                            im.buf.p, ns, stream_);
     im.version = param_version_;
+    launched = true;
+  }
+  if (!d_wg_table_.p && tower_ > 0 && wino_fusable(N_)) {
+    d_wg_table_.ensure(kWinoWgTableInts);
+    launch_wino_wg_table(N_, d_wg_table_.p, stream_);
     launched = true;
   }
   if (affines_version_ != param_version_) {
@@ -740,13 +775,13 @@
     float* v = form == TowerForm::F16 ? d_vimg_.p : d_vimg2_.p;
     launch_wino_in(d_x32, v, d_count, bcap, N_, false, stream_, kWinoStemStages);
     launch_wino_gemm(v, image<float>(kWinoStem), d_scale_.p, d_shift_.p, nullptr, a, nullptr, d_count, bcap, N_, 1, false, stream_,
-                     kWinoStemStages);
+                     kWinoStemStages, 0, 1, wg_table());
     if (form == TowerForm::Wino4) launch_wino4_in(a, d_vimg_.p, d_count, bcap, N_, stream_, false);
   } else {
     const bool split = precision_ == 2;
     launch_wino_in(d_x32, d_vimg2_.p, d_count, bcap, N_, split, stream_, kWinoStemStages);
     launch_wino_gemm(d_vimg2_.p, image<float>(split ? kSplitStem : kWinoStem), split ? d_scale_s_.p + (size_t)2 * tower_ * kC : d_scale_.p,
-                     d_shift_.p, nullptr, a, d_vimg_.p, d_count, bcap, N_, 1, split, stream_, kWinoStemStages);
+                     d_shift_.p, nullptr, a, d_vimg_.p, d_count, bcap, N_, 1, split, stream_, kWinoStemStages, 0, 1, wg_table());
     if (!wino_fusable(N_)) launch_wino_in(a, d_vimg_.p, d_count, bcap, N_, split, stream_, kWinoStages, true);
   }
 }
@@ -811,7 +846,7 @@
     const bool split = precision_ == 2;
     const float* u = image<float>(split ? kSplitTower : kWinoTower, l);
     launch_wino_gemm(io.vin, u, split ? d_scale_s_.p + (size_t)l * kC : sc, sh, io.res, io.y, io.vout, d_count, bcap, N_, 1, split,
-                     st, kWinoStages, part, parts);
+                     st, kWinoStages, part, parts, wg_table());
     if (io.vout && !wino_fusable(N_)) launch_wino_in(io.y, io.vout, d_count, bcap, N_, split, st, kWinoStages, true);
   }
 }
@@ -850,7 +885,7 @@
     AGZ_HIP(hipHostMalloc((void**)&tower_err_, sizeof(int32_t), hipHostMallocDefault));
     *tower_err_ = 0;
   }
-  timed(nl, [&] { launch_wino_tower(d_tower_layers_.p, nl, d_tower_sched_.p, d_count, bcap, N_, split, stream_); });
+  timed(nl, [&] { launch_wino_tower(d_tower_layers_.p, nl, d_tower_sched_.p, d_count, bcap, N_, split, stream_, wg_table()); });
   (void)hipMemcpyAsync(tower_err_, d_tower_sched_.p + kWinoTowerErrWord, sizeof(int32_t), hipMemcpyDeviceToHost, stream_);
 }
 
@@ -873,8 +908,8 @@
   const float* x = form == TowerForm::F16 || tower_ % 2 ? d_b_.p : d_a_.p;
   const int hgrid = std::min(ceil_div((long)bcap * P_, 4), 256 * 16);
   hipLaunchKernelGGL(k_head_conv, dim3(hgrid), dim3(256), 0, stream_, x, d_head_.p, d_vh_.p, d_ph_.p, d_count, P_);
-  const size_t smem = sizeof(float) * (size_t)(3 * P_ + A_ + 4);
-  hipLaunchKernelGGL(k_head_fc, dim3(bcap), dim3(256), smem, stream_, (const float*)d_vh_.p,
+  const size_t smem = sizeof(float) * (size_t)(kHeadFcG * (3 * P_ + A_) + 4);
+  hipLaunchKernelGGL(k_head_fc, dim3(ceil_div(bcap, kHeadFcG)), dim3(256), smem, stream_, (const float*)d_vh_.p,
                      (const float*)d_ph_.p, d_vfc1w_, d_vfc1b_, d_vfc2w_, d_vfc2b_, d_pfcw_,
                      d_pfcb_, d_pi, d_v, d_count, P_, A_);
   if (prof_on_ && prof_fwd_ < kProfMax) prof_fwd_++;
diff --git a/alphago.jl_amd/csrc/agz_wino.hip b/alphago.jl_amd/csrc/agz_wino.hip
--- a/alphago.jl_amd/csrc/agz_wino.hip
+++ b/alphago.jl_amd/csrc/agz_wino.hip
@@ -43,6 +43,21 @@
   return (tt <= WT && whole * 10 >= WT * 9) ? whole : WT;
 }
 __host__ __device__ inline bool wino_whole_boards(int T) { return wino_rows_per_block(T) % (T * T) == 0 && T * T <= WT; }
+
+constexpr int kWgTabPoints = WT * 9, kWgTabTiles = kWgTabPoints + WT;
+static_assert(kWgTabTiles + 1 == kWinoWgTableInts, "table size of agz_nn.h");
+__host__ __device__ inline int wino_wg_table_entry(int N, int i) {
+  const int T = (N + 2) / 3, TT = T * T, P = N * N;
+  const int RPB = wino_rows_per_block(T);
+  if (i == kWgTabTiles) return (RPB / TT) * P * kC;
+  const int row = i & (WT - 1);
+  if (row >= RPB) return -1;
+  const int b = row / TT, t = row - b * TT, ti = t / T, tj = t - ti * T;
+  if (i >= kWgTabPoints) return ti | tj << 8;
+  const int k = i >> 6;
+  const int pi = 3 * ti + k / 3, pj = 3 * tj + k % 3;
+  return pi < N && pj < N ? (b * P + pi + N * pj) * kC : -1;
+}
 
 __host__ __device__ __forceinline__ bool wino_tile_fused(int T, int row, int ti, int tj) {
   const int lo = (ti > 0 ? T : 0) + (tj > 0 ? 1 : 0), hi = (ti < T - 1 ? T : 0) + (tj < T - 1 ? 1 : 0);
@@ -160,7 +175,7 @@
     float* __restrict__ lds, int* __restrict__ ptab, const float* __restrict__ vimg, const float* __restrict__ uimg,
     const float* __restrict__ scale, const float* __restrict__ shift, const float* __restrict__ res, float* __restrict__ y,
     float* __restrict__ vnext, const long Mt, const int N, const int T, const int relu, const int tb, const int cb, const int MODE,
-    const int tid) {
+    const int tid, const int* __restrict__ wtab, const int wstride) {
   const int P = N * N, TT = T * T;
   const int RPB = wino_rows_per_block(T);
   const int lane = tid & 63;
@@ -179,9 +194,19 @@
     else glds16s(g, (unsigned)lane * 16u, lds0 + (unsigned)(buf * STAGE + c * 256) * 4u);
   };
 
+  if (wtab) {
+    const unsigned pt0 = (unsigned)(size_t)(__attribute__((address_space(3))) int*)&ptab[0];
+#pragma unroll
+    for (int i = 0; i < 3; ++i) {
+      const int first = i == 2 && wave >= 2 ? 64 * wave : 64 * wave + 256 * i;
+      glds4s(wtab, 4u * (unsigned)(first + lane), pt0 + 4u * (unsigned)first);
+    }
+  }
+
 #pragma unroll
   for (int j = 0; j < 13; ++j) dma(0, 0, j);
 
+  if (!wtab)
   for (int idx = tid; idx < WT * 9; idx += 256) {
     const int row = idx & (WT - 1), k = idx >> 6;
     const long tile = (long)tb * RPB + row;
@@ -260,6 +285,16 @@
   };
   wait_stage();
   __syncthreads();
+  if (wtab) {
+    const long left = Mt - (long)tb * RPB;
+    const int rows = left < WT ? (int)left : WT;
+    const int base = tb * wstride + cb * WC;
+    const bool alive = lane < rows;
+    const int te0 = ptab[tid], te1 = ptab[tid + 256], te2 = tid < 128 ? ptab[tid + 512] : -1;
+    ptab[tid] = alive && te0 >= 0 ? base + te0 : -1;
+    ptab[tid + 256] = alive && te1 >= 0 ? base + te1 : -1;
+    if (tid < 128) ptab[tid + 512] = alive && te2 >= 0 ? (tid < 64 ? base + te2 : te2) : -1;
+  }
 #pragma unroll
   for (int k = 0; k < LA; ++k) load(lds, k, ra[k], rb[k]);
 
@@ -401,10 +436,18 @@
 
   {
     const int row = lane;
-    const long tile = (long)tb * RPB + row;
-    const bool live = row < RPB && tile < Mt;
-    const int t = live ? (int)(tile % TT) : 0;
-    const int ti = t / T, tj = t % T;
+    bool live;
+    int ti, tj;
+    if (wtab) {
+      const int tij = ptab[kWgTabPoints + row];
+      live = tij >= 0;
+      ti = live ? tij & 255 : 0, tj = live ? tij >> 8 : 0;
+    } else {
+      const long tile = (long)tb * RPB + row;
+      live = row < RPB && tile < Mt;
+      const int t = live ? (int)(tile % TT) : 0;
+      ti = t / T, tj = t % T;
+    }
     const bool emit = wino_whole_boards(T) || (live && wino_tile_fused(T, row, ti, tj));
     unsigned adr[25];
 #pragma unroll
@@ -493,16 +536,18 @@
 __global__ __launch_bounds__(256, 1) void k_wino_gemm4(
     const float* __restrict__ vimg, const float* __restrict__ uimg, const float* __restrict__ scale,
     const float* __restrict__ shift, const float* __restrict__ res, float* __restrict__ y,
-    float* __restrict__ vnext, const int* __restrict__ d_count, int N, int T, int relu, int tb0, int tb1) {
+    float* __restrict__ vnext, const int* __restrict__ d_count, int N, int T, int relu, int tb0, int tb1,
+    const int* __restrict__ wtab) {
   __shared__ __attribute__((aligned(256))) float lds[3 * STAGE];
-  __shared__ int ptab[WT * 9];
+  __shared__ int ptab[kWgTabTiles];
   const long Mt = (long)(*d_count) * (T * T);
+  const int wstride = wtab ? wtab[kWgTabTiles] : 0;
   const int bid = blockIdx.x;
   const int xcd = bid & 7, jb = bid >> 3;
   const int cb = jb & 3;
   const int tb = tb0 + xcd + 8 * (jb >> 2);
   if (tb >= tb1 || (long)tb * wino_rows_per_block(T) >= Mt) return;
-  wino_wg<SPLIT, NS, false>(lds, ptab, vimg, uimg, scale, shift, res, y, vnext, Mt, N, T, relu, tb, cb, MODE, (int)threadIdx.x);
+  wino_wg<SPLIT, NS, false>(lds, ptab, vimg, uimg, scale, shift, res, y, vnext, Mt, N, T, relu, tb, cb, MODE, (int)threadIdx.x, wtab, wstride);
 }
 
 typedef WinoTowerLayer TowerLayer;
@@ -512,9 +557,10 @@
 
 template <bool SPLIT>
 __global__ __launch_bounds__(256, 1) void k_wino_tower(const TowerLayer* __restrict__ layers, int nl, int* __restrict__ sched,
-                                                       int blocks_cap, const int* __restrict__ d_count, int N, int T, int order) {
+                                                       int blocks_cap, const int* __restrict__ d_count, int N, int T, int order,
+                                                       const int* __restrict__ wtab) {
   __shared__ __attribute__((aligned(256))) float lds[3 * STAGE];
-  __shared__ int ptab[WT * 9];
+  __shared__ int ptab[kWgTabTiles];
   __shared__ int s_bc;
   const int tid = threadIdx.x;
   unsigned xcc;
@@ -528,6 +574,7 @@
     return;
   }
   const int quad = slot >> 2, cb = slot & 3;
+  const int wstride = __builtin_amdgcn_readfirstlane(wtab ? wtab[kWgTabTiles] : 0);
   const int RPB = wino_rows_per_block(T);
   const long Mt = (long)(*d_count) * (T * T);
   const int blocks = (int)((Mt + RPB - 1) / RPB);
@@ -564,7 +611,7 @@
     const TowerLayer L = layers[l];
     int t = tid;
     asm volatile("" : "+v"(t));
-    wino_wg<SPLIT, WNS, true>(lds, ptab, L.v, L.u, L.scale, L.shift, L.res, L.y, L.vnext, Mt, N, T, L.relu, tb, cb, L.mode, t);
+    wino_wg<SPLIT, WNS, true>(lds, ptab, L.v, L.u, L.scale, L.shift, L.res, L.y, L.vnext, Mt, N, T, L.relu, tb, cb, L.mode, t, wtab, wstride);
     asm volatile("s_waitcnt vmcnt(0)" ::: "memory");
     __syncthreads();
     if (tid == 0) {
@@ -620,6 +667,18 @@
 const ImageFamily kWinoImage = image_family<WinoImage<false>>(), kWinoSplitImage = image_family<WinoImage<true>>();
 float wino_split_descale() { return 1.f / (kSplitV * kSplitU); }
 
+void wino_wg_table_host(int N, int* out) {
+  for (int i = 0; i < kWinoWgTableInts; ++i) out[i] = wino_wg_table_entry(N, i);
+}
+__global__ void k_wino_wg_table(int N, int* __restrict__ out) {
+  const int i = blockIdx.x * blockDim.x + threadIdx.x;
+  if (i < kWinoWgTableInts) out[i] = wino_wg_table_entry(N, i);
+}
+void launch_wino_wg_table(int N, int* d_out, hipStream_t s) {
+  AGZ_REQUIRE(wino_fusable(N), AGZ_BAD_ARGUMENT, "F(3x3,3x3) workgroup table: %dx%d has dense tile blocks", N, N);
+  hipLaunchKernelGGL(k_wino_wg_table, dim3((kWinoWgTableInts + 255) / 256), dim3(256), 0, s, N, d_out);
+}
+
 long wino_blocks(int bcap, int T) {
   const long rpb = wino_rows_per_block(T);
   return ((long)bcap * T * T + rpb - 1) / rpb;
@@ -648,7 +707,7 @@
 
 void launch_wino_gemm(const float* vimg, const float* uimg, const float* scale, const float* shift, const float* res,
                       float* y, float* vnext, const int* d_count, int bcap, int N, int relu, bool split, hipStream_t s, int ns, int part,
-                      int parts) {
+                      int parts, const int* wg_table) {
   const int T = (N + 2) / 3;
   const int all_blocks = (int)wino_blocks(bcap, T);
   int tb0, tb1;
@@ -661,9 +720,10 @@
   wino_check_32bit(all_blocks, WT, bcap, N);
   const bool stem = ns == kWinoStemStages;
   const int mode = vnext ? (y || stem ? 3 : 2) : 1;
+  AGZ_REQUIRE(!wg_table || wino_whole_boards(T), AGZ_BAD_ARGUMENT, "F(3x3,3x3): a workgroup table needs whole-board tile blocks");
 #define WG_LAUNCH(MODE_, SPLIT_, NS_)                                                                                     \
   hipLaunchKernelGGL((k_wino_gemm4<MODE_, SPLIT_, NS_>), grid, block, 0, s, vimg, uimg, scale, shift, res, y, vnext, d_count, \
-                     N, T, relu, tb0, tb1)
+                     N, T, relu, tb0, tb1, wg_table)
   constexpr int S = kWinoStemStages;
   switch (mode | (split ? 4 : 0) | (stem ? 8 : 0)) {
     case 15: WG_LAUNCH(3, true, S); break;
@@ -708,7 +768,8 @@
   return ok;
 }
 
-void launch_wino_tower(const void* d_layers, int layers, int* d_sched, const int* d_count, int bcap, int N, bool split, hipStream_t s) {
+void launch_wino_tower(const void* d_layers, int layers, int* d_sched, const int* d_count, int bcap, int N, bool split, hipStream_t s,
+                       const int* wg_table) {
   const int T = (N + 2) / 3;
   AGZ_REQUIRE(wino_whole_boards(T), AGZ_BAD_ARGUMENT, "the persistent tower kernel needs whole-board tile blocks");
   wino_check_32bit(wino_blocks(bcap, T), WT, bcap, N);
@@ -716,9 +777,9 @@
   (void)hipMemsetAsync(d_sched, 0, sizeof(int) * wino_tower_sched_ints(layers, bcap, N), s);
   constexpr int order = 0;
   if (split)
-    hipLaunchKernelGGL((k_wino_tower<true>), dim3(256), dim3(256), 0, s, (const TowerLayer*)d_layers, layers, d_sched, blocks_cap, d_count, N, T, order);
+    hipLaunchKernelGGL((k_wino_tower<true>), dim3(256), dim3(256), 0, s, (const TowerLayer*)d_layers, layers, d_sched, blocks_cap, d_count, N, T, order, wg_table);
   else
-    hipLaunchKernelGGL((k_wino_tower<false>), dim3(256), dim3(256), 0, s, (const TowerLayer*)d_layers, layers, d_sched, blocks_cap, d_count, N, T, order);
-}
-
-}
+    hipLaunchKernelGGL((k_wino_tower<false>), dim3(256), dim3(256), 0, s, (const TowerLayer*)d_layers, layers, d_sched, blocks_cap, d_count, N, T, order, wg_table);
+}
+
+}
diff --git a/include/agz_debug.h b/include/agz_debug.h
--- a/include/agz_debug.h
+++ b/include/agz_debug.h
@@ -20,6 +20,7 @@
 agz_status agz_debug_mfma_sustained(agz_engine* e, int32_t millis, float* tflops_out);
 agz_status agz_debug_mfma_sustained_data(agz_engine* e, int32_t millis, int32_t mode, float* tflops_out);
 agz_status agz_debug_pack_diff(agz_engine* e, int32_t which, int64_t* mismatches_out);
+agz_status agz_debug_wino_wg_table(int32_t N, int32_t* out, int32_t capacity);
 
 #ifdef __cplusplus
 }
```

Result: no change. 454.2 (median of 3 runs) (+0.1%).
